# jameshball/kidney-diffusion

Measured on AMD Instinct MI355X. Metric: denoising-steps/sec (64->256 SR UNet, bs16), higher is better.
Workload: dtype f32

## Files before the change

### include/kd_engine.h

```cpp
#ifndef KD_ENGINE_H
#define KD_ENGINE_H

#include <stddef.h>
#include <stdint.h>

#ifdef __cplusplus
extern "C" {
#endif

#define KD_MAX_LEVELS 8

const char* kd_last_error(void);
#define KD_ENGINE_ABI_VERSION 2
int kd_version(void);
const char* kd_build_id(void);

typedef struct kd_unet_config {
  int dim;
  int num_levels;
  int dim_mults[KD_MAX_LEVELS];
  int num_resnet_blocks[KD_MAX_LEVELS];
  int layer_attns[KD_MAX_LEVELS];
  int layer_cross_attns[KD_MAX_LEVELS];
  int cond_dim;
  int channels;
  int cond_images_channels;
  int lowres_cond;
  int memory_efficient;
  int init_conv_to_final_conv_residual;
  int cond_on_text;
  int text_tokens;
  int attn_heads;
  int attn_dim_head;
  int ff_mult_x2;
  int num_time_tokens;
  int sinu_dim;
  int resnet_groups;
  int attend_at_middle;
  int use_gca;
  int batch;
  int image_size;
  int conv_algo;
  int attn_qk_norm;
  int downsample_conv4;
  int mid_attn_plain;
  int wino_slice_mb;
  int wino43_min_cin;
  int gemm_bf16x3;
  int x3_linear;
  int wino4_max_images;
} kd_unet_config_t;

typedef struct kd_param {
  const char* name;
  const float* d_data;
  int64_t numel;
} kd_param_t;

typedef struct kd_unet kd_unet_t;

int kd_unet_create(const kd_unet_config_t* cfg, const kd_param_t* params, int n_params,
                   kd_unet_t** out);
int kd_unet_create_shared(const kd_unet_config_t* cfg, const kd_param_t* params, int n_params,
                          const kd_unet_t* share_with, kd_unet_t** out);
int kd_unet_create_self_cond(const kd_unet_config_t* cfg, const kd_param_t* params, int n_params,
                             const kd_unet_t* share_with, int self_cond, kd_unet_t** out);
typedef struct kd_unet_ext {
  int self_cond;
  int use_linear_attn[KD_MAX_LEVELS];
  int use_linear_cross_attn[KD_MAX_LEVELS];
  int cross_embed_downsample;
  int upsample_nearest;
} kd_unet_ext_t;
int kd_unet_create_ext(const kd_unet_config_t* cfg, const kd_param_t* params, int n_params, const kd_unet_t* share_with,
                       const kd_unet_ext_t* ext, kd_unet_t** out);
typedef struct kd_unet_ext2 {
  int combine_upsample_fmaps;
} kd_unet_ext2_t;
int kd_unet_create_ext2(const kd_unet_config_t* cfg, const kd_param_t* params, int n_params, const kd_unet_t* share_with,
                        const kd_unet_ext_t* ext, const kd_unet_ext2_t* ext2, kd_unet_t** out);
typedef struct kd_unet_ext3 {
  int layer_attns_depth[KD_MAX_LEVELS];
} kd_unet_ext3_t;
int kd_unet_create_ext3(const kd_unet_config_t* cfg, const kd_param_t* params, int n_params, const kd_unet_t* share_with,
                        const kd_unet_ext_t* ext, const kd_unet_ext2_t* ext2, const kd_unet_ext3_t* ext3, kd_unet_t** out);
void kd_unet_destroy(kd_unet_t* u);
int64_t kd_unet_hbm_bytes(const kd_unet_t* u);
int64_t kd_unet_weight_bytes(const kd_unet_t* u);
int64_t kd_unet_macs(const kd_unet_t* u);
int64_t kd_unet_mfma_macs(const kd_unet_t* u);
int64_t kd_unet_mfma_bf16_macs(const kd_unet_t* u);
int kd_unet_num_launches(const kd_unet_t* u);
int kd_unet_num_cond_launches(const kd_unet_t* u);
float kd_unet_cond_table_build_ms(kd_unet_t* u, int* rows, int* runs);
int64_t kd_unet_cond_table_refused_bytes(const kd_unet_t* u);

int kd_unet_text_cond(kd_unet_t* u, const float* d_text_embeds, const float* d_text_mask, int L, int drop,
                      float* d_text_tokens, float* d_text_hiddens, void* stream);

int kd_unet_profile(kd_unet_t* u, int iters, char* buf, size_t buflen, void* stream);

int kd_unet_forward(kd_unet_t* u, const float* d_x, const float* d_lowres,
                    const float* d_cond_images, const float* d_log_snr,
                    const float* d_lowres_log_snr, const float* d_text_tokens,
                    const float* d_text_hiddens, float* d_out, void* stream);
int kd_unet_forward_self_cond(kd_unet_t* u, const float* d_x, const float* d_self_cond, const float* d_lowres,
                              const float* d_cond_images, const float* d_log_snr, const float* d_lowres_log_snr,
                              const float* d_text_tokens, const float* d_text_hiddens, float* d_out, void* stream);

int kd_cfg_combine(const float* d_cond, const float* d_null, float* d_out, float cond_scale, int64_t n,
                   void* stream);

enum { KD_OBJ_NOISE = 0, KD_OBJ_V = 1, KD_OBJ_X_START = 2 };

typedef struct kd_schedule {
  int T;
  const float* log_snr;
  const float* alpha;
  const float* sigma;
  const float* alpha_next;
  const float* sigma_next;
  const float* c;
  const float* noise_scale;
  const float* rn_a;
  const float* rn_b;
} kd_schedule_t;

typedef struct kd_sample_args {
  int objective;
  int dynamic_threshold;
  float percentile;
  int resample_times;
  const float* d_lowres;
  const float* d_lowres_log_snr;
  const float* d_cond_images;
  const float* d_text_tokens;
  const float* d_text_hiddens;
  const float* d_inpaint_images;
  const float* d_inpaint_masks;
  const float* d_noise_step;
  const float* d_noise_inpaint;
  const float* d_noise_renoise;
  uint64_t seed;
  int use_graph;
  float cond_scale;
  const float* d_null_text_tokens;
  const float* d_null_text_hiddens;
  int lowres_log_snr_uniform;
  float lowres_log_snr_value;
  int cond_table;
  int cond_table_max_mb;
} kd_sample_args_t;

int kd_sample_loop(kd_unet_t* u, const kd_schedule_t* sched, const kd_sample_args_t* args,
                   float* d_img, void* stream);
int kd_sample_steps(kd_unet_t* u, const kd_schedule_t* sched, const kd_sample_args_t* args,
                    float* d_img, int k_begin, int k_end, void* stream);
int kd_sample_build_cond_table(kd_unet_t* u, const kd_schedule_t* sched, const kd_sample_args_t* args, int k_begin,
                               int k_end, int force, int* built, void* stream);
int kd_sample_finalize(kd_unet_t* u, const kd_sample_args_t* args, float* d_img, void* stream);
int kd_sample_last(kd_unet_t* u, int which, float* d_out, void* stream);
int kd_sample_set_self_cond(kd_unet_t* u, const float* d_x_start, void* stream);

typedef struct kd_edm_schedule {
  int N;
  float S_noise;
  const float* sigma;
  const float* sigma_hat;
  const float* sigma_next;
  const float* churn;
  const float* euler_step;
  const float* heun_step;
  const float* renoise;
  const float* c_in_hat;
  const float* c_skip_hat;
  const float* c_out_hat;
  const float* c_noise_hat;
  const float* c_in_next;
  const float* c_skip_next;
  const float* c_out_next;
  const float* c_noise_next;
} kd_edm_schedule_t;

int kd_edm_sample_loop(kd_unet_t* u, const kd_edm_schedule_t* sched, const kd_sample_args_t* args, float* d_img,
                       void* stream);
int kd_edm_sample_steps(kd_unet_t* u, const kd_edm_schedule_t* sched, const kd_sample_args_t* args, float* d_img,
                        int k_begin, int k_end, void* stream);


int kd_conv2d_nhwc(const float* d_x, const float* d_w_oihw, const float* d_bias, float* d_y,
                   int B, int Hi, int Wi, int Cin, int Cout, int KH, int KW, int stride, int pad,
                   int act, void* stream);
int kd_upsample_nearest_conv3x3_nhwc(const float* d_x, const float* d_w_oihw, const float* d_bias, float* d_y, int ldy, int yoff,
                                     int B, int H, int W, int Cin, int Cout, void* stream);
int kd_upsample_nearest_gn_conv3x3_nhwc(const float* d_x, int ldx, const float* d_ab, const float* d_w_oihw, const float* d_bias,
                                        float* d_y, int ldy, int yoff, int B, int H, int W, int Cin, int Cout, int scale,
                                        void* stream);
int kd_conv3x3_winograd_nhwc(const float* d_x, const float* d_w_oihw, const float* d_bias, float* d_y,
                             int B, int H, int W, int Cin, int Cout, void* stream);
int kd_conv3x3_winograd4_nhwc(const float* d_x, const float* d_w_oihw, const float* d_bias, const float* d_res,
                              float* d_y, int B, int H, int W, int Cin, int Cout, int G, float eps,
                              float* d_out_stats, int gemm_bf16x3, void* stream);
int kd_gemm_bf16x3(const float* d_a, const float* d_b, float* d_c, int G, int M, int N, int K, int a_planes, void* stream);
int kd_linear_bf16x3(const float* d_x, int ldx, const float* d_w, const float* d_bias, const float* d_res, int ldres,
                     const float* d_gate_src, int ldgs, const float* d_gate, int hw, float* d_y, int ldy, int M, int N, int K,
                     int act, int pixshuf_wo, double* d_seg, void* stream);
int kd_linear_bf16x3_seg_rows(int M, int N, int K);
int kd_downsample_bf16x3(const float* d_x, int ldx, const float* d_w, const float* d_bias, float* d_y, int B, int H, int W, int C,
                         int O, double* d_seg, void* stream);
int kd_gn_conv3x3_winograd_fused_nhwc(const float* d_x, const float* d_gamma, const float* d_beta,
                                      const float* d_scale_shift, const float* d_w_oihw,
                                      const float* d_bias, const float* d_res, float* d_y, int B, int H,
                                      int W, int Cin, int Cout, int G, float eps, float* d_out_stats,
                                      int ldx, void* stream);

int kd_linear_skinny(const float* d_x, int ldx, const float* d_w, const float* d_bias, float* d_y, int ldy, int M, int K,
                     int N, int in_act, int act, void* stream);
int kd_global_context_gate(const float* d_x, int B, int HW, int C, const float* d_wk, const float* d_bk, const float* d_w0,
                           const float* d_b0, int hid, const float* d_w2, const float* d_b2, float* d_gate, float* d_pooled,
                           int path, void* stream);
int kd_gate_add_nhwc(const float* d_a, const float* d_gate, const float* d_r, int ldr, float* d_y, int ldy, double* d_seg,
                     int B, int HW, int C, void* stream);
int kd_gate_add_chunks(int B, int HW);
int kd_linattn_chunk_tokens(void);
int kd_linattn_dwconv_nhwc(const float* d_x, const float* d_wq, const float* d_wk, const float* d_wv, float* d_y,
                           float* d_part, int B, int H, int W, int heads, void* stream);
int kd_linattn_context(const float* d_k, const float* d_v, int ld, const float* d_part, int HW, const float* d_ck,
                       const float* d_cv, int ldc, int m, const float* d_null_k, const float* d_null_v, float* d_ctx, int B,
                       int heads, void* stream);
int kd_linattn_apply(const float* d_q, int ldq, const float* d_ctx, float* d_out, int ldo, int B, int N, int heads,
                     float scale, int silu, void* stream);
int kd_gn_fold_seg(const double* d_seg0, int nseg0, int nchunk0, float scale0, float ab_mul0, const double* d_seg1, int nseg1,
                   int nchunk1, float scale1, float ab_mul1, const float* d_gamma, const float* d_beta,
                   const float* d_scale_shift, int ld_ss, float* d_ab, float* d_stats, int B, int HW, int C, int G, float eps,
                   void* stream);
float kd_wf_ab_scale(void);
int kd_gn_conv3x3_winograd4_nhwc(const float* d_x, int ldx, const float* d_stats, const float* d_gamma, const float* d_beta,
                                 const float* d_scale_shift, int ld_ss, int skip_c0, float skip_scale, const float* d_w_oihw,
                                 const float* d_bias, const float* d_res, int ldres, float* d_y, double* d_out_seg, int B,
                                 int H, int W, int Cin, int Cout, int G, int gemm_mode, int images_per_set, void* stream);

int kd_init_conv_nchw(const float* d_x, const float* d_w3, const float* d_w7, const float* d_w15,
                      const float* d_bias, float* d_y, int B, int S, int n3, int n7, int n15, void* stream);
int kd_init_conv_planes_nchw(const float* d_x, const float* d_self_cond, const float* d_w3, const float* d_w7,
                             const float* d_w15, int Itot, int c0, const float* d_bias, const float* d_res, float* d_y, int B,
                             int S, int n3, int n7, int n15, int iters, float* ms, void* stream);
int kd_init_conv_planes_c_nchw(const float* d_x, const float* d_self_cond, const float* d_w3, const float* d_w7,
                               const float* d_w15, int Itot, int c0, const float* d_bias, const float* d_res, float* d_y, int B,
                               int S, int n3, int n7, int n15, int iters, float* ms, int channels, void* stream);
int kd_final_conv_nchw(const float* d_feat, const float* d_w_oihw, const float* d_bias, const float* d_lowres, float* d_out,
                       int B, int H, int W, int Cfeat, int channels, void* stream);
int kd_groupnorm_silu_nhwc(const float* d_x, const float* d_gamma, const float* d_beta,
                           const float* d_scale_shift, float* d_y, int B, int HW, int C, int G,
                           float eps, void* stream);
int kd_layernorm(const float* d_x, const float* d_g, const float* d_beta, float* d_y,
                 int rows, int C, float eps, void* stream);
int kd_layernorm_ex(const float* d_x, const float* d_g, const float* d_beta, const float* d_res, float* d_y, int rows, int C,
                    float eps, int in_act, const float* d_g2, float* d_y2, void* stream);
int kd_layernorm_linear_bf16x3(const float* d_x, const float* d_g, const float* d_beta, int rows, int C, float eps, int in_act,
                               const float* d_w, const float* d_bias, const float* d_res, int ldres, float* d_y, int ldy,
                               int N, void* d_planes, void* stream);
int kd_attention(const float* d_q, const float* d_k, const float* d_v, float* d_out,
                 int B, int Nq, int Nk, int H, int Hkv, int D, void* stream);
int kd_attention_ex(const float* d_q, int ldq, const float* d_null_kv, const float* d_k0, const float* d_v0, int ld0, int n0,
                    const float* d_k1, const float* d_v1, int ld1, int n1, float* d_out, int ldo, int B, int Nq, int H, int Hkv,
                    float scale, void* stream);
int kd_attention_ex_d(const float* d_q, int ldq, const float* d_null_kv, const float* d_k0, const float* d_v0, int ld0, int n0,
                      const float* d_k1, const float* d_v1, int ld1, int n1, float* d_out, int ldo, int B, int Nq, int H, int Hkv,
                      int D, float scale, void* stream);
int kd_attention_key_tile(int D);
int kd_l2norm_heads(float* d_x, int ld, int64_t rows, int heads, const float* d_scale_vec, void* stream);
int kd_l2norm_heads_d(float* d_x, int ld, int64_t rows, int heads, int D, const float* d_scale_vec, void* stream);
int kd_text_select(const float* d_tok, const float* d_mask, const float* d_null_embed, float* d_out, int B, int L, int P, int C,
                   int drop, void* stream);
int kd_add_rows_bcast(const float* d_x, const float* d_add, float* d_y, int B, int R, int C, void* stream);
int kd_mean_rows(const float* d_x, float* d_y, int B, int R, int C, void* stream);
int kd_copy_rows(const float* d_src, int64_t src_bstride, int ld_src, float* d_dst, int64_t dst_bstride, int ld_dst, int rows,
                 int C, int B, void* stream);
int kd_quantile_abs(const float* d_x, float* d_out, int B, int64_t n, float q, void* d_workspace,
                    size_t workspace_bytes, void* stream);
size_t kd_quantile_workspace_bytes(int B);
int kd_philox_normal(float* d_out, int64_t n, uint64_t seed, uint64_t stream_id, void* stream);

#ifdef __cplusplus
}
#endif
#endif
```

### kidney-diffusion_amd/csrc/api.inc

```
extern "C" {

const char* kd_last_error(void) { return kd::g_err.c_str(); }
int kd_version(void) { return KD_ENGINE_ABI_VERSION; }

int kd_unet_create(const kd_unet_config_t* cfg, const kd_param_t* params, int n_params, kd_unet_t** out) {
  return kd_unet_create_shared(cfg, params, n_params, nullptr, out);
}

int kd_unet_create_shared(const kd_unet_config_t* cfg, const kd_param_t* params, int n_params,
                          const kd_unet_t* share_with, kd_unet_t** out) {
  return kd_unet_create_self_cond(cfg, params, n_params, share_with, 0, out);
}

int kd_unet_create_self_cond(const kd_unet_config_t* cfg, const kd_param_t* params, int n_params,
                             const kd_unet_t* share_with, int self_cond, kd_unet_t** out) {
  kd_unet_ext_t ext;
  memset(&ext, 0, sizeof ext);
  ext.self_cond = self_cond;
  return kd_unet_create_ext(cfg, params, n_params, share_with, &ext, out);
}

int kd_unet_create_ext(const kd_unet_config_t* cfg, const kd_param_t* params, int n_params, const kd_unet_t* share_with,
                       const kd_unet_ext_t* ext, kd_unet_t** out) {
  return kd_unet_create_ext2(cfg, params, n_params, share_with, ext, nullptr, out);
// ... 363 lines not shown
  KD_REQUIRE(d_x && d_w_oihw && d_y, "kd_upsample_nearest_gn_conv3x3_nhwc: null argument");
  if (const char* why = upsample_scale_refusal(ldx, ldy, yoff, B, H, W, Cin, Cout, scale)) {
    set_error(why);
    return 1;
  }
  EntryBufs bufs;
  float* wp = nullptr;
  if (bufs.get(&wp, upsample_scale_weight_floats(Cin, Cout) * sizeof(float))) return 1;
  int rc = launch_upsample_scale_pack(d_w_oihw, wp, Cout, Cin, s);
  if (!rc) rc = launch_upsample_scale_conv3x3(d_x, ldx, d_ab, wp, d_bias, d_y, ldy, yoff, B, H, W, Cin, Cout, scale, s);
  return entry_finish(rc, s);
}

int kd_conv3x3_winograd_nhwc(const float* d_x, const float* d_w_oihw, const float* d_bias, float* d_y, int B, int H,
                             int W, int Cin, int Cout, void* stream) {
  hipStream_t s = (hipStream_t)stream;
  KD_REQUIRE(H % 2 == 0 && W % 2 == 0, "Winograd path needs even H and W");
  const int64_t Mt = (int64_t)B * (H / 2) * (W / 2);
  KD_REQUIRE(Mt % 256 == 0 && Cin % 32 == 0 && Cout > 32 && Cout % 4 == 0,
             "Winograd path needs B*H*W/4 % 256 == 0, Cin % 32 == 0, Cout > 32");
  EntryBufs bufs;
  float *U = nullptr, *V = nullptr, *D = nullptr;
  if (bufs.get(&U, (size_t)16 * Cout * Cin * sizeof(float))) return 1;
  if (bufs.get(&V, (size_t)16 * Mt * Cin * sizeof(float))) return 1;
  if (bufs.get(&D, (size_t)16 * Mt * Cout * sizeof(float))) return 1;
  int rc = launch_wino_pack(d_w_oihw, U, Cout, Cin, s);
  if (!rc) rc = launch_wino_in(d_x, Cin, nullptr, nullptr, nullptr, nullptr, 0, V, B, H, W, Cin, 1, 0, Mt, s);
  if (!rc) {
    ConvParams p{};
    p.x = V; p.w = U; p.y = D;
    p.B = 1; p.Hi = 1; p.Wi = (int)(16 * Mt); p.Cin = Cin; p.ldx = Cin;
    p.Ho = 1; p.Wo = (int)(16 * Mt); p.Cout = Cout;
    p.KH = 1; p.KW = 1; p.stride = 1; p.pad = 0;
    p.out_mode = OUT_NHWC; p.ldy = Cout;
    p.wz_rows = (int)Mt; p.wz_count = 16;
    rc = launch_conv_igemm(p, s);
  }
  if (!rc) rc = launch_wino_out(D, d_bias, nullptr, 0, d_y, B, H, W, Cout, 0, Mt, s);
  return entry_finish(rc, s);
}

int kd_conv3x3_winograd4_nhwc(const float* d_x, const float* d_w_oihw, const float* d_bias, const float* d_res, float* d_y,
                              int B, int H, int W, int Cin, int Cout, int G, float eps, float* d_out_stats, int gemm_bf16x3,
                              void* stream) {
  hipStream_t s = (hipStream_t)stream;
  KD_REQUIRE(H % 4 == 0 && W % 4 == 0, "Winograd F(4x4,3x3) path needs H % 4 == 0 and W % 4 == 0");
  const int64_t Mt = (int64_t)B * (H / 4) * (W / 4);
  KD_REQUIRE(!gemm_bf16x3 || gemm_bf16x3_ok(36, Mt, Cout, Cin),
             "bf16x3 position GEMMs need B*H*W/16 % 256 == 0, Cout % 128 == 0, Cin % 32 == 0");
  KD_REQUIRE(Mt % 128 == 0 && Cin % 32 == 0 && Cout % 64 == 0,
             "Winograd F(4x4,3x3) path needs B*H*W/16 % 128 == 0, Cin % 32 == 0, Cout % 64 == 0");
  KD_REQUIRE(!d_out_stats || (G > 0 && Cout % G == 0 && (Cout / G) % 16 == 0), "output statistics need (Cout / G) % 16 == 0");
  EntryBufs bufs;
  float *U = nullptr, *V = nullptr, *D = nullptr;
  double* seg = nullptr;
  void *U3 = nullptr, *x3ws = nullptr;
  const int nchunk = (H / 4) * (W / 4);
  if (bufs.get(&U, (size_t)36 * Cout * Cin * sizeof(float))) return 1;
  if (bufs.get(&V, (size_t)36 * Mt * Cin * (gemm_bf16x3 == 1 ? 6 : sizeof(float)))) return 1;
  if (bufs.get(&D, (size_t)36 * Mt * Cout * sizeof(float))) return 1;
  if (gemm_bf16x3 && bufs.get(&U3, (size_t)36 * Cout * Cin * 6)) return 1;
  if (gemm_bf16x3 && bufs.get(&x3ws, gemm_bf16x3_workspace_bytes())) return 1;
  if (d_out_stats && bufs.get(&seg, (size_t)B * (Cout / 16) * nchunk * 2 * sizeof(double))) return 1;
  if (gemm_bf16x3) KD_HIP_CHECK(hipMemsetAsync(x3ws, 0, gemm_bf16x3_workspace_bytes(), s));
  int rc = launch_wino4_pack(d_w_oihw, U, Cout, Cin, s);
  if (!rc && gemm_bf16x3) {
    rc = launch_split3(U, U3, 36, Cout, Cin, s);
    if (!rc && gemm_bf16x3 == 1) rc = launch_wino4_in3(d_x, Cin, nullptr, nullptr, nullptr, nullptr, 0, V, B, H, W, Cin, 1, s);
    if (!rc && gemm_bf16x3 != 1) rc = launch_wino4_in(d_x, Cin, nullptr, nullptr, nullptr, nullptr, 0, V, B, H, W, Cin, 1, s);
    if (!rc) rc = launch_gemm_bf16x3(V, U3, D, 36, (int)Mt, Cout, Cin, entry_x3_shape(36, Mt, Cout, Cin), x3ws, s, gemm_bf16x3 != 1);
  }
  if (!rc && !gemm_bf16x3) rc = launch_wino4_in(d_x, Cin, nullptr, nullptr, nullptr, nullptr, 0, V, B, H, W, Cin, 1, s);
  if (!rc && !gemm_bf16x3) {
    ConvParams p{};
    p.x = V; p.w = U; p.y = D;
    p.B = 1; p.Hi = 1; p.Wi = (int)(36 * Mt); p.Cin = Cin; p.ldx = Cin;
    p.Ho = 1; p.Wo = (int)(36 * Mt); p.Cout = Cout;
    p.KH = 1; p.KW = 1; p.stride = 1; p.pad = 0;
    p.out_mode = OUT_NHWC; p.ldy = Cout;
    p.wz_rows = (int)Mt; p.wz_count = 36;
    rc = launch_conv_igemm(p, s);
  }
  if (!rc) rc = launch_wino4_out(D, d_bias, d_res, Cout, d_y, Cout, seg, B, H, W, Cout, s);
  if (!rc && seg)
    rc = launch_gn_finalize(seg, d_out_stats, (Cout / G / 16) * nchunk, B, G, (double)H * W * (Cout / G), eps, s);
  return entry_finish(rc, s);
}

int kd_gemm_bf16x3(const float* d_a, const float* d_b, float* d_c, int G, int M, int N, int K, int a_planes, void* stream) {
  hipStream_t s = (hipStream_t)stream;
  KD_REQUIRE(gemm_bf16x3_ok(G, M, N, K), "kd_gemm_bf16x3 needs M % 256 == 0, N % 128 == 0, K % 32 == 0, operand planes < 4 GB");
  EntryBufs bufs;
  void *A3 = nullptr, *B3 = nullptr, *ws = nullptr;
  if (bufs.get(&B3, (size_t)G * N * K * 6)) return 1;
  if (a_planes && bufs.get(&A3, (size_t)G * M * K * 6)) return 1;
  if (bufs.get(&ws, gemm_bf16x3_workspace_bytes())) return 1;
  int rc = a_planes ? launch_split3(d_a, A3, G, M, K, s) : 0;
  if (!rc) rc = launch_split3(d_b, B3, G, N, K, s);
  if (!rc) rc = launch_gemm_bf16x3(a_planes ? A3 : (const void*)d_a, B3, d_c, G, M, N, K, entry_x3_shape(G, M, N, K), ws, s, !a_planes);
  return entry_finish(rc, s);
}

int kd_downsample_bf16x3(const float* d_x, int ldx, const float* d_w, const float* d_bias, float* d_y, int B, int H, int W, int C,
                         int O, double* d_seg, void* stream) {
  hipStream_t s = (hipStream_t)stream;
  const int K = 4 * C;
  const int64_t M = (int64_t)B * (H / 2) * (W / 2);
  X3Epi e;
  e.bias = d_bias;
  e.lda = ldx > 0 ? ldx : C;
  e.ldy = O;
  e.a_tap_c = C;
  e.a_wi = W;
  e.a_hi = H;
  e.hw = (H / 2) * (W / 2);
  e.seg = d_seg;
  e.seg_nseg = d_seg ? O / 16 : 0;
  const X3Shape sh = entry_x3_shape(1, M, O, K);
  KD_REQUIRE(H > 0 && W > 0 && !(H & 1) && !(W & 1) && M < 0x7fffffff && gemm_bf16x3_epi_ok(M, O, K, e, sh),
             "kd_downsample_bf16x3 needs even map sides, C % 16 == 0, B (H/2) (W/2) % 256 == 0, O % 128 == 0");
  EntryBufs bufs;
  float *wt = nullptr, *wk = nullptr;
  void *W3 = nullptr, *ws = nullptr;
  if (bufs.get(&wt, (size_t)O * K * 4) || bufs.get(&wk, (size_t)O * K * 4) || bufs.get(&W3, (size_t)O * K * 6) ||
      bufs.get(&ws, gemm_bf16x3_workspace_bytes()))
    return 1;
  int rc = launch_pack_unshuffle(d_w, wt, O, C, s);
  for (int t = 0; t < 4 && !rc; ++t) rc = launch_copy_scale_rows(wt + (size_t)t * O * C, C, wk + (size_t)t * C, K, C, 1.0f, O, s);
  if (!rc) rc = launch_split3(wk, W3, 1, O, K, s);
  if (!rc) rc = launch_gemm_bf16x3(d_x, W3, d_y, 1, (int)M, O, K, sh, ws, s, true, true, &e);
  return entry_finish(rc, s);
}

int kd_linear_bf16x3_seg_rows(int M, int N, int K) { return gemm_bf16x3_ok(1, M, N, K) ? entry_x3_shape(1, M, N, K).seg_rows() : 0; }

int kd_linear_bf16x3(const float* d_x, int ldx, const float* d_w, const float* d_bias, const float* d_res, int ldres,
                     const float* d_gate_src, int ldgs, const float* d_gate, int hw, float* d_y, int ldy, int M, int N, int K,
                     int act, int pixshuf_wo, double* d_seg, void* stream) {
  hipStream_t s = (hipStream_t)stream;
  X3Epi e;
  e.seg = d_seg;
  e.seg_nseg = d_seg ? (pixshuf_wo ? N / 4 : N) / 16 : 0;
  e.act = act;
  e.pixshuf_wo = pixshuf_wo;
  e.bias = d_bias;
  e.res = d_res;
  e.ldres = ldres;
  e.gate_src = d_gate_src;
  e.ldgs = ldgs;
  e.gate = d_gate;
  e.hw = hw;
  e.ldy = ldy > 0 ? ldy : (pixshuf_wo ? N / 4 : N);
  e.lda = ldx > 0 ? ldx : K;
  const X3Shape sh = entry_x3_shape(1, M, N, K);
  KD_REQUIRE(gemm_bf16x3_epi_ok(M, N, K, e, sh), "kd_linear_bf16x3 needs M % 256 == 0, N % 128 == 0, K % 32 == 0, row strides >= the "
                                             "rows, hw % 256 == 0 under a gate");
  EntryBufs bufs;
  void *W3 = nullptr, *ws = nullptr;
  if (bufs.get(&W3, (size_t)N * K * 6) || bufs.get(&ws, gemm_bf16x3_workspace_bytes())) return 1;
  int rc = launch_split3(d_w, W3, 1, N, K, s);
  if (!rc) rc = launch_gemm_bf16x3(d_x, W3, d_y, 1, M, N, K, sh, ws, s, true, true, &e);
  return entry_finish(rc, s);
}

int kd_gn_conv3x3_winograd_fused_nhwc(const float* d_x, const float* d_gamma, const float* d_beta,
                                      const float* d_scale_shift, const float* d_w_oihw, const float* d_bias,
                                      const float* d_res, float* d_y, int B, int H, int W, int Cin, int Cout, int G,
                                      float eps, float* d_out_stats, int ldx, void* stream) {
  hipStream_t s = (hipStream_t)stream;
  if (ldx <= 0) ldx = Cin;
  KD_REQUIRE(wino_fused128_ok(B, H, W, Cin, Cout) && G > 0 && Cin % G == 0,
             "GroupNorm-fused Winograd path needs H % 8 == 0, W % 16 == 0, Cin % 4 == 0, Cin <= 2048, Cout % 128 == 0");
  KD_REQUIRE(ldx >= Cin && ldx % 4 == 0, "GroupNorm-fused Winograd path: input row stride must be >= Cin and a multiple of 4");
  KD_REQUIRE(!d_out_stats || (Cout % G == 0 && (Cout / G) % 16 == 0), "output statistics need (Cout / G) % 16 == 0");
  EntryBufs bufs;
  float *U = nullptr, *stats = nullptr, *ab = nullptr;
  double *partial = nullptr, *opart = nullptr;
  void* items = nullptr;
  if (bufs.get(&U, (size_t)16 * Cout * Cin * sizeof(float))) return 1;
  if (bufs.get(&stats, (size_t)B * G * 2 * sizeof(float))) return 1;
  if (bufs.get(&ab, (size_t)B * Cin * 2 * sizeof(float))) return 1;
  if (bufs.get(&partial, gn_partial_bytes(B, H * W, Cin, G))) return 1;
  if (d_out_stats && bufs.get(&opart, (size_t)B * G * wino_fused_out_stats_chunks(H, W, Cout, G) * 2 * sizeof(double))) return 1;
  if (bufs.get(&items, wino_fused128_items_count(B, H, W, Cout) * 16)) return 1;
  int rc = launch_wino_fused128_pack(d_w_oihw, U, Cout, Cin, s, WF_U_SCALE);
  if (!rc) rc = launch_gn_stats(d_x, ldx, stats, partial, B, H * W, Cin, G, eps, s);
  if (!rc) rc = launch_gn_fold(stats, d_gamma, d_beta, d_scale_shift, 2 * Cin, ab, B, Cin, G, s);
  if (!rc) rc = launch_wino_fused128_items(items, B, H, W, Cout, s);
  if (!rc)
    rc = launch_wino_fused_gn128(d_x, ldx, ab, U, d_bias, d_res, Cout, d_y, B, H, W, Cin, Cout, opart, opart ? G : 0, items, s);
  if (!rc && opart)
    rc = launch_gn_finalize(opart, d_out_stats, (int)wino_fused_out_stats_chunks(H, W, Cout, G), B, G,
                            (double)H * W * (Cout / G), eps, s);
  return entry_finish(rc, s);
}


int kd_linear_skinny(const float* d_x, int ldx, const float* d_w, const float* d_bias, float* d_y, int ldy, int M, int K,
                     int N, int in_act, int act, void* stream) {
  hipStream_t s = (hipStream_t)stream;
  KD_REQUIRE(d_x && d_w && d_y, "kd_linear_skinny: null argument");
  KD_REQUIRE(M > 0 && K > 0 && N > 0 && ldx >= K && ldy >= N, "kd_linear_skinny needs M, K, N > 0, ldx >= K, ldy >= N");
  KD_REQUIRE(in_act >= ACT_NONE && in_act <= ACT_SIGMOID && act >= ACT_NONE && act <= ACT_SIGMOID,
             "kd_linear_skinny: unknown activation");
  return entry_finish(launch_linear_skinny(d_x, ldx, d_w, d_bias, d_y, ldy, M, K, N, in_act, act, s), s);
}

int kd_linattn_chunk_tokens(void) { return LA_CHUNK; }

int kd_linattn_dwconv_nhwc(const float* d_x, const float* d_wq, const float* d_wk, const float* d_wv, float* d_y,
                           float* d_part, int B, int H, int W, int heads, void* stream) {
  hipStream_t s = (hipStream_t)stream;
  KD_REQUIRE(d_x && d_wq && d_wk && d_wv && d_y && d_part, "kd_linattn_dwconv_nhwc: null argument");
  KD_REQUIRE(B > 0 && H > 0 && W > 0 && heads > 0, "kd_linattn_dwconv_nhwc needs B, H, W, heads > 0");
  const int inner = heads * 64;
  EntryBufs bufs;
  float* w = nullptr;
  if (bufs.get((void**)&w, (size_t)27 * inner * sizeof(float))) return 1;
  int rc = launch_linattn_pack_dw(d_wq, d_wk, d_wv, w, inner, s);
  if (!rc) rc = launch_linattn_dwconv(d_x, w, d_y, d_part, B, H, W, inner, s);
  return entry_finish(rc, s);
}

int kd_linattn_context(const float* d_k, const float* d_v, int ld, const float* d_part, int HW, const float* d_ck,
                       const float* d_cv, int ldc, int m, const float* d_null_k, const float* d_null_v, float* d_ctx, int B,
                       int heads, void* stream) {
  hipStream_t s = (hipStream_t)stream;
  KD_REQUIRE(d_ctx && B > 0 && heads > 0 && HW >= 0 && m >= 0, "kd_linattn_context: null output or bad sizes");
  EntryBufs bufs;
  float* ws = nullptr;
  if (HW > 0 && bufs.get((void**)&ws, linattn_ws_floats(B, heads, HW) * sizeof(float))) return 1;
  return entry_finish(launch_linattn_context(d_k, d_v, ld, d_part, HW, d_ck, d_cv, ldc, m, d_null_k, d_null_v, ws, d_ctx, B,
                                             heads, s), s);
}

int kd_linattn_apply(const float* d_q, int ldq, const float* d_ctx, float* d_out, int ldo, int B, int N, int heads,
                     float scale, int silu, void* stream) {
  hipStream_t s = (hipStream_t)stream;
  KD_REQUIRE(d_q && d_ctx && d_out, "kd_linattn_apply: null argument");
  return entry_finish(launch_linattn_apply(d_q, ldq, d_ctx, d_out, ldo, B, N, heads, scale, silu, s), s);
}

int kd_global_context_gate(const float* d_x, int B, int HW, int C, const float* d_wk, const float* d_bk, const float* d_w0,
                           const float* d_b0, int hid, const float* d_w2, const float* d_b2, float* d_gate, float* d_pooled,
                           int path, void* stream) {
  hipStream_t s = (hipStream_t)stream;
  KD_REQUIRE(d_x && d_wk && d_bk && d_w0 && d_b0 && d_w2 && d_b2 && d_gate, "kd_global_context_gate: null argument");
  KD_REQUIRE(B > 0 && HW > 0 && hid > 0 && C % 4 == 0 && C > 0 && C <= 2048,
             "kd_global_context_gate needs B, HW, hid > 0 and C % 4 == 0, C <= 2048");
  KD_REQUIRE(path >= 0 && path <= 2, "kd_global_context_gate: path 0 (the plan's choice), 1 (pool + two linears), 2 (fused)");
  const bool fused_ok = gca_gate_fused_ok(C, hid) && (((uintptr_t)d_w0 | (uintptr_t)d_w2) & 15) == 0;
  KD_REQUIRE(path != 2 || fused_ok, "kd_global_context_gate: the fused gate needs C <= 512, hid <= 256, 16-byte aligned weights");
  const bool fused = path == 2 || (path == 0 && gca_gate_fused_ok(C, hid) && B > 1);
  KD_REQUIRE(!(fused && d_pooled), "kd_global_context_gate: the fused gate does not leave the pooled vector");
  EntryBufs bufs;
  float *scratch = nullptr, *pooled = d_pooled, *hidden = nullptr;
  if (bufs.get((void**)&scratch, gca_scratch_floats(B, HW, C) * sizeof(float))) return 1;
  if (fused) return entry_finish(launch_gca_gate(d_x, d_wk, d_bk, scratch, d_w0, d_b0, hid, d_w2, d_b2, d_gate, B, HW, C, s), s);
  if (!pooled && bufs.get((void**)&pooled, (size_t)B * C * sizeof(float))) return 1;
  if (bufs.get((void**)&hidden, (size_t)B * hid * sizeof(float))) return 1;
  int rc = launch_gca_pool(d_x, d_wk, d_bk, nullptr, pooled, scratch, B, HW, C, s);
  if (!rc) rc = launch_linear_skinny(pooled, C, d_w0, d_b0, hidden, hid, B, C, hid, ACT_NONE, ACT_SILU, s);
  if (!rc) rc = launch_linear_skinny(hidden, hid, d_w2, d_b2, d_gate, C, B, hid, C, ACT_NONE, ACT_SIGMOID, s);
  return entry_finish(rc, s);
}

int kd_gate_add_chunks(int B, int HW) { return B > 0 && HW > 0 ? gate_add_chunks(B, HW) : 0; }

int kd_gate_add_nhwc(const float* d_a, const float* d_gate, const float* d_r, int ldr, float* d_y, int ldy, double* d_seg,
                     int B, int HW, int C, void* stream) {
  hipStream_t s = (hipStream_t)stream;
  if (ldr <= 0) ldr = C;
  if (ldy <= 0) ldy = C;
  KD_REQUIRE(d_a && d_r && d_y, "kd_gate_add_nhwc: null argument");
  KD_REQUIRE(B > 0 && HW > 0 && C > 0 && C % 4 == 0 && ldr >= C && ldy >= C && ldr % 4 == 0 && ldy % 4 == 0,
             "kd_gate_add_nhwc needs C % 4 == 0 and row strides >= C, multiples of 4");
  KD_REQUIRE((((uintptr_t)d_a | (uintptr_t)d_gate | (uintptr_t)d_r | (uintptr_t)d_y) & 15) == 0,
             "kd_gate_add_nhwc: 16-byte aligned maps and gate");
  KD_REQUIRE(!d_seg || C % 16 == 0, "kd_gate_add_nhwc: segment partials need C % 16 == 0");
  return entry_finish(launch_gate_add(d_a, d_gate, d_r, ldr, d_y, ldy, d_seg, B, HW, C, s), s);
}

float kd_wf_ab_scale(void) { return WF_AB_SCALE; }

int kd_gn_fold_seg(const double* d_seg0, int nseg0, int nchunk0, float scale0, float ab_mul0, const double* d_seg1, int nseg1,
                   int nchunk1, float scale1, float ab_mul1, const float* d_gamma, const float* d_beta,
                   const float* d_scale_shift, int ld_ss, float* d_ab, float* d_stats, int B, int HW, int C, int G, float eps,
                   void* stream) {
  hipStream_t s = (hipStream_t)stream;
  KD_REQUIRE(d_seg0 && (d_ab || d_stats), "kd_gn_fold_seg: null argument");
  KD_REQUIRE(B > 0 && HW > 0 && G > 0 && C % G == 0 && (C / G) % 16 == 0, "kd_gn_fold_seg needs groups of 16 n channels");
  KD_REQUIRE(nseg0 > 0 && nchunk0 > 0 && (!d_seg1 || (nseg1 > 0 && nchunk1 > 0)) &&
                 16 * (nseg0 + (d_seg1 ? nseg1 : 0)) == C,
             "kd_gn_fold_seg: the sources' 16-channel segments must tile the C channels");
  KD_REQUIRE(!d_ab || (d_gamma && d_beta), "kd_gn_fold_seg: the affine needs gamma and beta");
  KD_REQUIRE(!d_scale_shift || ld_ss >= 2 * C, "kd_gn_fold_seg: FiLM rows [scale | shift] need ld_ss >= 2 C");
  SegSrc s0{d_seg0, nseg0, nchunk0, 0, scale0, ab_mul0};
  SegSrc s1{d_seg1, d_seg1 ? nseg1 : 0, d_seg1 ? nchunk1 : 0, 16 * nseg0, scale1, ab_mul1};
  return entry_finish(launch_gn_fold_seg(s0, s1, d_gamma, d_beta, d_scale_shift, ld_ss, d_ab, d_stats, B, C, G,
                                         (double)HW * (C / G), eps, s),
                      s);
}

int kd_gn_conv3x3_winograd4_nhwc(const float* d_x, int ldx, const float* d_stats, const float* d_gamma, const float* d_beta,
                                 const float* d_scale_shift, int ld_ss, int skip_c0, float skip_scale, const float* d_w_oihw,
                                 const float* d_bias, const float* d_res, int ldres, float* d_y, double* d_out_seg, int B,
                                 int H, int W, int Cin, int Cout, int G, int gemm_mode, int images_per_set, void* stream) {
  hipStream_t s = (hipStream_t)stream;
  if (ldx <= 0) ldx = Cin;
  if (ldres <= 0) ldres = Cout;
  const int Bx = images_per_set > 0 ? images_per_set : B;
  KD_REQUIRE(d_x && d_stats && d_gamma && d_beta && d_w_oihw && d_bias && d_y, "kd_gn_conv3x3_winograd4_nhwc: null argument");
  KD_REQUIRE(B > 0 && Bx > 0 && B % Bx == 0, "kd_gn_conv3x3_winograd4_nhwc: images_per_set must divide B");
  KD_REQUIRE(H > 0 && W > 0 && H % 4 == 0 && W % 4 == 0, "Winograd F(4x4,3x3) path needs H % 4 == 0 and W % 4 == 0");
  const int64_t Mt = (int64_t)Bx * (H / 4) * (W / 4);
  KD_REQUIRE(Mt % 128 == 0 && Cin % 32 == 0 && Cout % 64 == 0 && 36 * Mt < 0x7fffffff &&
                 (int64_t)36 * Cout * Cin * 4 < 0x7fffffff,
             "Winograd F(4x4,3x3) path needs images_per_set*H*W/16 % 128 == 0, Cin % 32 == 0, Cout % 64 == 0");
  KD_REQUIRE(gemm_mode == -1 || gemm_mode == 1 || gemm_mode == 2, "kd_gn_conv3x3_winograd4_nhwc: gemm_mode -1, 1 or 2");
  KD_REQUIRE(gemm_mode < 0 || gemm_bf16x3_ok(36, Mt, Cout, Cin),
             "bf16x3 position GEMMs need images_per_set*H*W/16 % 256 == 0, Cout % 128 == 0, Cin % 32 == 0");
  KD_REQUIRE(G > 0 && Cin % G == 0, "kd_gn_conv3x3_winograd4_nhwc: Cin % G == 0");
  KD_REQUIRE(ldx >= Cin && ldx % 2 == 0 && ((uintptr_t)d_x & 7) == 0 && (int64_t)Bx * H * W * ldx * 4 < ((int64_t)1 << 32),
             "kd_gn_conv3x3_winograd4_nhwc: x rows of stride >= Cin, even, 8-byte aligned, one set's map below 4 GB");
  KD_REQUIRE(skip_c0 < 0 || (skip_c0 <= Cin && skip_c0 % 2 == 0), "kd_gn_conv3x3_winograd4_nhwc: skip_c0 in [0, Cin], even");
  KD_REQUIRE(!d_scale_shift || ld_ss >= 2 * Cin, "kd_gn_conv3x3_winograd4_nhwc: FiLM rows [scale | shift] need ld_ss >= 2 Cin");
  KD_REQUIRE(!d_res || (ldres >= Cout && ldres % 2 == 0), "kd_gn_conv3x3_winograd4_nhwc: residual row stride >= Cout, even");
  KD_REQUIRE((((uintptr_t)d_y | (uintptr_t)d_res | (uintptr_t)d_bias) & 7) == 0,
             "kd_gn_conv3x3_winograd4_nhwc: 8-byte aligned y, residual and bias");
  const bool planes = gemm_mode == 1, x3 = gemm_mode > 0;
  const X3Shape sh = entry_x3_shape(36, Mt, Cout, Cin);
  EntryBufs bufs;
  float *U = nullptr, *D = nullptr;
  void *V = nullptr, *U3 = nullptr, *ws = nullptr;
  if (bufs.get((void**)&U, (size_t)36 * Cout * Cin * sizeof(float))) return 1;
  if (bufs.get(&V, planes ? (size_t)36 * Mt * Cin * 6 : (size_t)36 * Mt * Cin * sizeof(float))) return 1;
  if (bufs.get((void**)&D, (size_t)36 * Mt * Cout * sizeof(float))) return 1;
  if (x3 && bufs.get(&U3, ((size_t)36 * Cout * Cin * 3 + 1) / 2 * sizeof(float))) return 1;
  if (x3 && bufs.get(&ws, gemm_bf16x3_workspace_bytes())) return 1;
  int rc = launch_wino4_pack(d_w_oihw, U, Cout, Cin, s);
  if (!rc && x3) rc = launch_split3(U, U3, 36, Cout, Cin, s);
  const int64_t HW = (int64_t)H * W, nchunk = (H / 4) * (W / 4);
  for (int st = 0; st < B / Bx && !rc; ++st) {
    const int b0 = st * Bx;
    const float* xs = d_x + (size_t)b0 * HW * ldx;
    const float* ss = d_stats + (size_t)b0 * G * 2;
    const float* ssp = d_scale_shift ? d_scale_shift + (size_t)b0 * ld_ss : nullptr;
    if (planes)
      rc = launch_wino4_in3(xs, ldx, ss, d_gamma, d_beta, ssp, ld_ss, V, Bx, H, W, Cin, G, s, skip_c0, skip_scale);
    else
      rc = launch_wino4_in(xs, ldx, ss, d_gamma, d_beta, ssp, ld_ss, (float*)V, Bx, H, W, Cin, G, s, skip_c0, skip_scale);
    if (!rc && x3) {
      rc = launch_gemm_bf16x3(V, U3, D, 36, (int)Mt, Cout, Cin, sh, ws, s, !planes);
    } else if (!rc) {
      ConvParams p{};
      p.x = (const float*)V; p.w = U; p.y = D;
      p.B = 1; p.Hi = 1; p.Wi = (int)(36 * Mt); p.Cin = Cin; p.ldx = Cin;
      p.Ho = 1; p.Wo = (int)(36 * Mt); p.Cout = Cout;
      p.KH = 1; p.KW = 1; p.stride = 1; p.pad = 0;
      p.out_mode = OUT_NHWC; p.ldy = Cout;
      p.wz_rows = (int)Mt; p.wz_count = 36;
      rc = launch_conv_igemm(p, s);
    }
    if (!rc)
      rc = launch_wino4_out(D, d_bias, d_res ? d_res + (size_t)b0 * HW * ldres : nullptr, ldres, d_y + (size_t)b0 * HW * Cout,
                            Cout, d_out_seg ? d_out_seg + (size_t)b0 * (Cout / 16) * nchunk * 2 : nullptr, Bx, H, W, Cout, s);
  }
  return entry_finish(rc, s);
}

int kd_init_conv_nchw(const float* d_x, const float* d_w3, const float* d_w7, const float* d_w15, const float* d_bias,
                      float* d_y, int B, int S, int n3, int n7, int n15, void* stream) {
  return kd_init_conv_planes_nchw(d_x, nullptr, d_w3, d_w7, d_w15, 3, 0, d_bias, nullptr, d_y, B, S, n3, n7, n15, 1, nullptr,
                                  stream);
}

int kd_init_conv_planes_nchw(const float* d_x, const float* d_self_cond, const float* d_w3, const float* d_w7,
                             const float* d_w15, int Itot, int c0, const float* d_bias, const float* d_res, float* d_y, int B,
                             int S, int n3, int n7, int n15, int iters, float* ms, void* stream) {
  return kd_init_conv_planes_c_nchw(d_x, d_self_cond, d_w3, d_w7, d_w15, Itot, c0, d_bias, d_res, d_y, B, S, n3, n7, n15, iters,
                                    ms, 3, stream);
}

int kd_init_conv_planes_c_nchw(const float* d_x, const float* d_self_cond, const float* d_w3, const float* d_w7,
                               const float* d_w15, int Itot, int c0, const float* d_bias, const float* d_res, float* d_y, int B,
                               int S, int n3, int n7, int n15, int iters, float* ms, int channels, void* stream) {
  hipStream_t s = (hipStream_t)stream;
  KD_REQUIRE(channels >= 1 && channels <= 4, "kd_init_conv_planes_c_nchw: 1 to 4 image channels");
  const int np = d_self_cond ? 2 * channels : channels;
  KD_REQUIRE(d_x && d_w3 && d_w7 && d_w15 && d_y && iters >= 1, "kd_init_conv_planes_nchw: null argument or iters < 1");
  KD_REQUIRE(B >= 1 && S >= 1, "kd_init_conv_planes_nchw: empty shape");
  KD_REQUIRE(c0 >= 0 && c0 + np <= Itot, "kd_init_conv_planes_nchw: input channels c0 .. c0 + planes - 1 out of range");
  KD_REQUIRE(init_conv_fused_ok(S, n3, n7, n15, np), "init conv kernel: S % 32 == 0 and the weights must fit LDS");
  EntryBufs bufs;
  float* wp = nullptr;
  hipEvent_t e0 = nullptr, e1 = nullptr;
  if (bufs.get(&wp, init_conv_weight_floats(n3, n7, n15, np) * sizeof(float))) return 1;
  int rc = launch_init_conv_pack(d_w3, d_w7, d_w15, wp, n3, n7, n15, Itot, c0, np, s);
  if (!rc && ms) {
    rc = hipEventCreate(&e0) != hipSuccess || hipEventCreate(&e1) != hipSuccess || hipEventRecord(e0, s) != hipSuccess;
    if (rc) set_error("kd_init_conv_planes_nchw: event setup failed");
  }
  for (int i = 0; i < iters && !rc; ++i)
    rc = launch_init_conv(d_x, d_self_cond, channels, np, wp, d_bias, d_res, d_y, n3 + n7 + n15, nullptr, B, S, n3, n7, n15, s);
  if (!rc && ms && hipEventRecord(e1, s) != hipSuccess) {
    set_error("kd_init_conv_planes_nchw: event record failed");
    rc = 1;
  }
  hipError_t e = hipStreamSynchronize(s);
  if (!rc && ms && e == hipSuccess) {
    float t = 0.f;
    e = hipEventElapsedTime(&t, e0, e1);
    *ms = t / iters;
  }
  if (e0) (void)hipEventDestroy(e0);
  if (e1) (void)hipEventDestroy(e1);
  if (rc) return rc;
  KD_HIP_CHECK(e);
  return 0;
}

int kd_final_conv_nchw(const float* d_feat, const float* d_w_oihw, const float* d_bias, const float* d_lowres, float* d_out,
                       int B, int H, int W, int Cfeat, int channels, void* stream) {
  hipStream_t s = (hipStream_t)stream;
  KD_REQUIRE(d_feat && d_w_oihw && d_bias && d_out, "kd_final_conv_nchw: null argument");
  KD_REQUIRE(channels >= 1 && channels <= 4, "kd_final_conv_nchw: 1 to 4 image channels");
  KD_REQUIRE(B >= 1 && H >= 1 && W >= 1 && Cfeat >= 4 && Cfeat % 4 == 0 && (int64_t)B * H * W < 0x7fffffff / 48,
             "kd_final_conv_nchw needs a non-empty map below 2^31 / 48 pixels and Cfeat % 4 == 0");
  const int Ctot = Cfeat + (d_lowres ? channels : 0), nf = final_gemm_cols(channels);
  EntryBufs bufs;
  float *wp = nullptr, *pm = nullptr, *stat = nullptr;
  if (bufs.get(&wp, (size_t)nf * Cfeat * sizeof(float)) || bufs.get(&pm, (size_t)B * H * W * nf * sizeof(float))) return 1;
  if (d_lowres && bufs.get(&stat, (size_t)B * channels * H * W * sizeof(float))) return 1;
  int rc = launch_pack_final(d_w_oihw, wp, Ctot, Cfeat, channels, s);
  if (!rc && d_lowres) rc = launch_final_static(d_lowres, d_w_oihw, d_bias, stat, Ctot, Cfeat, channels, B, H, W, s);
  if (!rc) {
    ConvParams p{};
    p.x = d_feat; p.w = wp; p.y = pm;
    p.B = B; p.Hi = H; p.Wi = W; p.Cin = Cfeat; p.ldx = Cfeat;
    p.Ho = H; p.Wo = W; p.Cout = nf;
    p.KH = 1; p.KW = 1; p.stride = 1; p.pad = 0;
    p.out_mode = OUT_NHWC; p.ldy = nf;
    rc = launch_conv_igemm(p, s);
  }
  if (!rc) rc = launch_final_gather(pm, stat, d_bias, d_out, channels, B, H, W, s);
  return entry_finish(rc, s);
}

int kd_groupnorm_silu_nhwc(const float* d_x, const float* d_gamma, const float* d_beta, const float* d_scale_shift,
                           float* d_y, int B, int HW, int C, int G, float eps, void* stream) {
  hipStream_t s = (hipStream_t)stream;
  EntryBufs bufs;
  float* stats = nullptr;
  double* partial = nullptr;
  if (bufs.get(&stats, (size_t)B * G * 2 * sizeof(float)) || bufs.get(&partial, gn_partial_bytes(B, HW, C, G))) return 1;
  int rc = launch_gn_stats(d_x, C, stats, partial, B, HW, C, G, eps, s);
  if (!rc) rc = launch_gn_apply_silu(d_x, C, stats, d_gamma, d_beta, d_scale_shift, 2 * C, d_y, B, HW, C, G, s);
  return entry_finish(rc, s);
}

int kd_layernorm(const float* d_x, const float* d_g, const float* d_beta, float* d_y, int rows, int C, float eps,
                 void* stream) {
  return launch_layernorm(d_x, C, d_g, d_beta, nullptr, 0, d_y, rows, C, eps, (hipStream_t)stream);
}

int kd_layernorm_ex(const float* d_x, const float* d_g, const float* d_beta, const float* d_res, float* d_y, int rows, int C,
                    float eps, int in_act, const float* d_g2, float* d_y2, void* stream) {
  KD_REQUIRE(in_act >= ACT_NONE && in_act <= ACT_SIGMOID, "kd_layernorm_ex: unknown activation");
  return launch_layernorm(d_x, C, d_g, d_beta, d_res, C, d_y, rows, C, eps, (hipStream_t)stream, in_act, d_g2, d_y2);
}

int kd_layernorm_linear_bf16x3(const float* d_x, const float* d_g, const float* d_beta, int rows, int C, float eps, int in_act,
                               const float* d_w, const float* d_bias, const float* d_res, int ldres, float* d_y, int ldy,
                               int N, void* d_planes, void* stream) {
  hipStream_t s = (hipStream_t)stream;
  KD_REQUIRE(in_act >= ACT_NONE && in_act <= ACT_SIGMOID, "kd_layernorm_linear_bf16x3: unknown activation");
  KD_REQUIRE(d_planes && C % 16 == 0 && C <= 4096, "kd_layernorm_linear_bf16x3 needs C % 16 == 0, C <= 4096 and the plane buffer");
  X3Epi e;
  e.bias = d_bias;
  e.res = d_res;
  e.ldres = ldres;
  e.hw = rows;
  e.ldy = ldy > 0 ? ldy : N;
  e.lda = C;
  const X3Shape sh = entry_x3_shape(1, rows, N, C);
  KD_REQUIRE(gemm_bf16x3_epi_ok(rows, N, C, e, sh), "kd_layernorm_linear_bf16x3 needs rows % 256 == 0, N % 128 == 0, C % 32 == 0");
  EntryBufs bufs;
  void *W3 = nullptr, *ws = nullptr;
  if (bufs.get(&W3, (size_t)N * C * 6) || bufs.get(&ws, gemm_bf16x3_workspace_bytes())) return 1;
  int rc = launch_split3(d_w, W3, 1, N, C, s);
  if (!rc) rc = launch_layernorm(d_x, C, d_g, d_beta, nullptr, 0, (float*)d_planes, rows, C, eps, s, in_act, nullptr, nullptr, nullptr, 0, 1);
  if (!rc) rc = launch_gemm_bf16x3(d_planes, W3, d_y, 1, rows, N, C, sh, ws, s, false, true, &e);
  return entry_finish(rc, s);
}

int kd_attention(const float* d_q, const float* d_k, const float* d_v, float* d_out, int B, int Nq, int Nk, int H,
                 int Hkv, int D, void* stream) {
  KD_REQUIRE(D == 32 || D == 64 || D == 128, "kd_attention is built for D = 32, 64 and 128");
  KVSeg s0{d_k, d_v, Hkv * D, Nk};
  KVSeg s1{nullptr, nullptr, 0, 0};
  return launch_attention(d_q, H * D, nullptr, nullptr, s0, s1, d_out, H * D, B, Nq, H, Hkv, D, 1.0f,
                          (hipStream_t)stream);
}

int kd_attention_ex(const float* d_q, int ldq, const float* d_null_kv, const float* d_k0, const float* d_v0, int ld0, int n0,
                    const float* d_k1, const float* d_v1, int ld1, int n1, float* d_out, int ldo, int B, int Nq, int H, int Hkv,
                    float scale, void* stream) {
  return kd_attention_ex_d(d_q, ldq, d_null_kv, d_k0, d_v0, ld0, n0, d_k1, d_v1, ld1, n1, d_out, ldo, B, Nq, H, Hkv, 64, scale,
                           stream);
}

int kd_attention_ex_d(const float* d_q, int ldq, const float* d_null_kv, const float* d_k0, const float* d_v0, int ld0, int n0,
                      const float* d_k1, const float* d_v1, int ld1, int n1, float* d_out, int ldo, int B, int Nq, int H, int Hkv,
                      int D, float scale, void* stream) {
  hipStream_t s = (hipStream_t)stream;
  KD_REQUIRE(d_q && d_out && B > 0 && H > 0 && n0 >= 0 && n1 >= 0, "kd_attention_ex: null argument or bad sizes");
  KD_REQUIRE((n0 == 0 || (d_k0 && d_v0)) && (n1 == 0 || (d_k1 && d_v1)), "kd_attention_ex: a segment with keys needs k and v");
  KD_REQUIRE((((uintptr_t)d_q | (uintptr_t)d_null_kv | (uintptr_t)d_k0 | (uintptr_t)d_v0 | (uintptr_t)d_k1 | (uintptr_t)d_v1 |
               (uintptr_t)d_out) & 15) == 0, "kd_attention_ex: 16-byte aligned pointers");
  KD_REQUIRE(D == 32 || D == 64 || D == 128, "kd_attention_ex_d: D must be 32, 64 or 128");
  KD_REQUIRE(ldq >= H * D && ldo >= H * D && (n0 == 0 || ld0 >= Hkv * D) && (n1 == 0 || ld1 >= Hkv * D),
             "kd_attention_ex: a row stride is shorter than its heads");
  KVSeg s0{d_k0, d_v0, ld0, n0};
  KVSeg s1{d_k1, d_v1, ld1, n1};
  return entry_finish(launch_attention(d_q, ldq, d_null_kv, d_null_kv ? d_null_kv + D : nullptr, s0, s1, d_out, ldo, B,
                                       Nq, H, Hkv, D, scale, s), s);
}

int kd_attention_key_tile(int D) { return attention_key_tile(D); }

int kd_l2norm_heads(float* d_x, int ld, int64_t rows, int heads, const float* d_scale_vec, void* stream) {
  return kd_l2norm_heads_d(d_x, ld, rows, heads, 64, d_scale_vec, stream);
}

int kd_l2norm_heads_d(float* d_x, int ld, int64_t rows, int heads, int D, const float* d_scale_vec, void* stream) {
  hipStream_t s = (hipStream_t)stream;
  KD_REQUIRE(D == 32 || D == 64 || D == 128, "kd_l2norm_heads_d: D must be 32, 64 or 128");
  KD_REQUIRE(d_x && rows >= 0 && heads > 0 && ld >= heads * D, "kd_l2norm_heads: null argument or ld < heads * D");
  return entry_finish(launch_l2norm_heads(d_x, ld, rows, heads, D, d_scale_vec, s), s);
}

int kd_text_select(const float* d_tok, const float* d_mask, const float* d_null_embed, float* d_out, int B, int L, int P, int C,
                   int drop, void* stream) {
  hipStream_t s = (hipStream_t)stream;
  KD_REQUIRE(d_tok && d_null_embed && d_out, "kd_text_select: null argument");
  KD_REQUIRE(B > 0 && C > 0 && L >= 1 && L <= P, "kd_text_select needs B, C > 0 and 1 <= L <= P");
  return entry_finish(launch_text_select(d_tok, d_mask, d_null_embed, d_out, B, L, P, C, drop != 0, s), s);
}

int kd_add_rows_bcast(const float* d_x, const float* d_add, float* d_y, int B, int R, int C, void* stream) {
  hipStream_t s = (hipStream_t)stream;
  KD_REQUIRE(d_x && d_add && d_y && B > 0 && R > 0 && C > 0, "kd_add_rows_bcast: null argument or empty shape");
  return entry_finish(launch_add_rows_bcast(d_x, d_add, d_y, B, R, C, s), s);
}

int kd_mean_rows(const float* d_x, float* d_y, int B, int R, int C, void* stream) {
  hipStream_t s = (hipStream_t)stream;
  KD_REQUIRE(d_x && d_y && B > 0 && R > 0 && C > 0, "kd_mean_rows: null argument or empty shape");
  KD_REQUIRE((int64_t)B * C < 0x7fffffff, "kd_mean_rows: B * C must stay below 2^31 (one thread per output, int index)");
  return entry_finish(launch_mean_rows(d_x, d_y, B, R, C, s), s);
}

int kd_copy_rows(const float* d_src, int64_t src_bstride, int ld_src, float* d_dst, int64_t dst_bstride, int ld_dst, int rows,
                 int C, int B, void* stream) {
  hipStream_t s = (hipStream_t)stream;
  KD_REQUIRE(d_src && d_dst && rows >= 0 && C >= 0 && B >= 0, "kd_copy_rows: null argument or negative size");
  KD_REQUIRE(ld_src >= C && ld_dst >= C && src_bstride >= 0 && dst_bstride >= 0, "kd_copy_rows needs row strides >= C, batch strides >= 0");
  return entry_finish(launch_copy_rows(d_src, src_bstride, ld_src, d_dst, dst_bstride, ld_dst, rows, C, B, s), s);
}

size_t kd_quantile_workspace_bytes(int B) { return quantile_ws_bytes(B); }
int kd_quantile_abs(const float* d_x, float* d_out, int B, int64_t n, float q, void* d_workspace,
                    size_t workspace_bytes, void* stream) {
  KD_REQUIRE(workspace_bytes >= quantile_ws_bytes(B), "quantile workspace too small");
  return launch_quantile_abs(d_x, d_out, B, n, q, d_workspace, (hipStream_t)stream);
}

int kd_cfg_combine(const float* d_cond, const float* d_null, float* d_out, float cond_scale, int64_t n,
                   void* stream) {
  KD_REQUIRE(d_cond && d_null && d_out && n >= 0, "kd_cfg_combine: null argument");
  return launch_cfg_combine(d_cond, d_null, d_out, cond_scale, n, (hipStream_t)stream);
}

int kd_philox_normal(float* d_out, int64_t n, uint64_t seed, uint64_t stream_id, void* stream) {
  return launch_philox_normal(d_out, n, seed, stream_id, (hipStream_t)stream);
}

}
```

### kidney-diffusion_amd/csrc/common.h

```cpp
#pragma once
#include <hip/hip_runtime.h>
#include <stdint.h>
#include <stdio.h>
#include <algorithm>
#include <string>

#ifdef KD_EXPERIMENT
#include "../../scratch/experiment_switch.h"
#else
constexpr int kd_switch(const char*, int dflt) { return dflt; }
#endif

namespace kd {

void set_error(const std::string& msg);

#define KD_HIP_CHECK(expr)                                                               \
  do {                                                                                   \
    hipError_t _e = (expr);                                                              \
    if (_e != hipSuccess) {                                                              \
      ::kd::set_error(std::string(#expr) + " failed: " + hipGetErrorString(_e) + " at " + \
                      __FILE__ + ":" + std::to_string(__LINE__));                        \
      return 1;                                                                          \
    }                                                                                    \
  } while (0)

#define KD_REQUIRE(cond, msg)                                                             \
  do {                                                                                    \
    if (!(cond)) {                                                                        \
      ::kd::set_error(std::string("requirement failed: ") + #cond + " — " + (msg) + " at " + \
                      __FILE__ + ":" + std::to_string(__LINE__));                         \
      return 1;                                                                           \
    }                                                                                     \
  } while (0)

enum Act { ACT_NONE = 0, ACT_SILU = 1, ACT_GELU = 2, ACT_SIGMOID = 3 };
enum OutMode { OUT_NHWC = 0, OUT_PIXSHUF = 1, OUT_NCHW = 2 };

struct ConvParams {
  const float* x;
  const float* w;
  const float* bias;
  float* y;
  int B, Hi, Wi, Cin, ldx;
  int Ho, Wo, Cout;
  int KH, KW, stride, pad;
  int rr_cin;
  int act;
  const float* res;
  int ldres;
  const float* gate_src;
  const float* gate;
  int ldgs;
  int out_mode;
  int ldy, yoff;
  int wz_rows, wz_count;
  float* partial;
  int ksplit;
  double* seg_partial;
  int seg_nseg;
  int seg_c0;
  int wide_epilogue;
};

int launch_conv_igemm(const ConvParams& p, hipStream_t s);
int conv_ksplit(const ConvParams& p);
int conv_seg_chunks(const ConvParams& p);
int64_t conv_macs(const ConvParams& p);

int launch_pack_oihw(const float* w_oihw, float* w_packed, int O, int I, int Ipad, int KH, int KW, hipStream_t s);
int launch_pack_oihw_rowrun(const float* w_oihw, float* w_packed, int O, int I, int Ipad, int KH, int KW, hipStream_t s);
int launch_pack_oihw_rowrun_sub(const float* w_oihw, float* w_packed, int O, int Itot, int a0, int na, int b0, int nb,
                                int Ipad, int KH, int KW, hipStream_t s);
int launch_pack_unshuffle(const float* w, float* w_packed, int O, int C, hipStream_t s);
int launch_pack_shuffle(const float* w, const float* b, float* w_packed, float* b_packed, int Co, int I,
                        hipStream_t s);

int launch_wino_pack(const float* w_oihw, float* U, int O, int I, hipStream_t s);
int launch_wino_in(const float* x, int ldx, const float* stats, const float* gamma, const float* beta,
                   const float* scale_shift, int ld_ss, float* V, int B, int H, int W, int C, int G, int64_t t0,
                   int64_t nt, hipStream_t s);
int launch_wino_out(const float* D, const float* bias, const float* res, int ldres, float* y, int B, int H, int W,
                    int C, int64_t t0, int64_t nt, hipStream_t s, double* seg_partial = nullptr);

int launch_wino4_pack(const float* w_oihw, float* U, int O, int I, hipStream_t s);
int launch_wino4_in(const float* x, int ldx, const float* stats, const float* gamma, const float* beta,
                    const float* scale_shift, int ld_ss, float* V, int B, int H, int W, int C, int G, hipStream_t s,
                    int mul_c0 = -1, float mul = 1.0f);
int launch_wino4_out(const float* D, const float* bias, const float* res, int ldres, float* y, int ldy, double* seg_partial,
                     int B, int H, int W, int C, hipStream_t s);

constexpr int X3_BK = 16;
__device__ __forceinline__ void x3_split(const float __attribute__((ext_vector_type(2))) a, uint32_t& h, uint32_t& m,
                                         uint32_t& l) {
  typedef float f2 __attribute__((ext_vector_type(2)));
  typedef __bf16 b2 __attribute__((ext_vector_type(2)));
  const b2 hb = __builtin_convertvector(a, b2);
  const f2 r1 = a - __builtin_convertvector(hb, f2);
  const b2 mb = __builtin_convertvector(r1, b2);
  const f2 r2 = r1 - __builtin_convertvector(mb, f2);
  const b2 lb = __builtin_convertvector(r2, b2);
  h = __builtin_bit_cast(uint32_t, hb);
  m = __builtin_bit_cast(uint32_t, mb);
  l = __builtin_bit_cast(uint32_t, lb);
}
bool gemm_bf16x3_ok(int G, int64_t M, int N, int K);
int launch_split3(const float* x, void* planes, int G, int R, int K, hipStream_t s);
size_t gemm_bf16x3_workspace_bytes();
struct X3Epi {
  const float* bias = nullptr;
  const float* res = nullptr;
  const float* gate_src = nullptr;
  const float* gate = nullptr;
  int ldres = 0, ldgs = 0;
  int hw = 0;
  int ldy = 0;
  int lda = 0;
  int a_tap_c = 0, a_wi = 0, a_hi = 0;
  double* seg = nullptr;
  int seg_nseg = 0, seg_coff = 0;
  int seg_rows8 = 0;
  int wide = 0;
  int act = ACT_NONE;
  int pixshuf_wo = 0;
};
struct X3Shape {
  int P, R, S, first;
  bool needs_sum() const { return R && S > 1; }
  int seg_rows() const { return needs_sum() ? 8 : 32; }
};
X3Shape gemm_bf16x3_shape(int G, int M, int N, int K, int cus);
int gemm_bf16x3_device_cus();
bool gemm_bf16x3_epi_ok(int64_t M, int N, int K, const X3Epi& e, const X3Shape& sh);
int launch_gemm_bf16x3(const void* A3, const void* B3, float* C, int G, int M, int N, int K, const X3Shape& sh, void* ws, hipStream_t s,
                       bool a_f32 = false, bool with_sum = true, const X3Epi* epi = nullptr);
int launch_gemm_bf16x3_sum(float* C, int G, int M, int N, int K, const X3Shape& sh, const void* ws, hipStream_t s, const X3Epi* epi = nullptr);
int launch_wino4_in3(const float* x, int ldx, const float* stats, const float* gamma, const float* beta,
                     const float* scale_shift, int ld_ss, void* V3, int B, int H, int W, int C, int G, hipStream_t s,
                     int mul_c0 = -1, float mul = 1.0f);

constexpr float WF_AB_SCALE = -1.4426950408889634f;
constexpr float WF_U_SCALE = -0.6931471805599453f;
int launch_gn_fold(const float* stats, const float* gamma, const float* beta, const float* scale_shift, int ld_ss,
                   float* ab, int B, int C, int G, hipStream_t s);
bool wino_fused128_ok(int B, int H, int W, int C, int N);
int launch_wino_fused128_pack(const float* w_oihw, float* U, int O, int I, hipStream_t s, float scale);
size_t wino_fused128_items_count(int B, int H, int W, int N);
int launch_wino_fused128_items(void* items, int B, int H, int W, int N, hipStream_t s);
size_t wino_fused_out_stats_chunks(int H, int W, int N, int G);
int launch_wino_fused_gn128(const float* x, int ldx, const float* ab, const float* U, const float* bias, const float* res,
                            int ldres, float* y, int B, int H, int W, int C, int N, double* out_partial, int out_groups,
                            const void* items, hipStream_t s);
int wino_fused_gn_max_cin();
int launch_gn_finalize(const double* partial, float* stats, int chunks, int B, int G, double count, float eps,
                       hipStream_t s);

int launch_gn_stats(const float* x, int ldx, float* stats , double* partial,
                    int B, int HW, int C, int G, float eps, hipStream_t s);
size_t gn_partial_bytes(int B, int HW, int C, int G);
int launch_gn_apply_silu(const float* x, int ldx, const float* stats, const float* gamma, const float* beta,
                         const float* scale_shift ,
                         int ld_ss, float* y, int B, int HW, int C, int G, hipStream_t s);
int launch_layernorm(const float* x, int ldx, const float* g, const float* beta, const float* res, int ldres, float* y,
                     int rows, int C, float eps, hipStream_t s, int in_act = ACT_NONE, const float* g2 = nullptr,
                     float* y2 = nullptr, double* seg = nullptr, int seg_hw = 0, int planes = 0);
int launch_copy_scale_rows(const float* src, int ld_src, float* dst, int ld_dst, int C, float scale, int64_t rows,
                           hipStream_t s);
int launch_gate_add(const float* a, const float* gate, const float* r, int ldr, float* y, int ldy, double* seg, int B,
                    int HW, int C, hipStream_t s);
int gate_add_chunks(int B, int HW);

struct SegSrc {
  const double* partial;
  int nseg, nchunk;
  int c0;
  float scale;
  float ab_mul;
};
int launch_gn_fold_seg(SegSrc s0, SegSrc s1, const float* gamma, const float* beta, const float* scale_shift, int ld_ss,
                       float* ab, float* stats, int B, int C, int G, double count, float eps, hipStream_t s);
int launch_add(const float* a, const float* b, float* y, int64_t n, hipStream_t s);
int launch_act(const float* a, float* y, int64_t n, int act, hipStream_t s);
int launch_pack_init(const float* cond, int Cc, const float* x, int Cx, const float* lowres, int Cl, float* y, int Cpad,
                     int B, int HW, hipStream_t s);
int launch_copy_rows(const float* src, int64_t src_bstride, int ld_src, float* dst, int64_t dst_bstride,
                     int ld_dst, int rows, int C, int B, hipStream_t s);
int launch_bcast_row(const float* src, float* dst, int64_t dst_bstride, int C, int B, hipStream_t s);

struct KVSeg {
  const float* k;
  const float* v;
  int ld;
  int n;
};
int launch_attention(const float* q, int ldq, const float* null_k, const float* null_v, KVSeg s0, KVSeg s1,
                     float* out, int ldo, int B, int Nq, int H, int Hkv, int D, float scale, hipStream_t s);
int attention_key_tile(int D);
int launch_linear_gemv(const float* x, const float* w, const float* bias, float* y, int K, int N, int in_act, int act,
                       hipStream_t s);
int launch_linear_skinny(const float* x, int ldx, const float* w, const float* bias, float* y, int ldy, int M,
                         int K, int N, int in_act, int act, hipStream_t s);
int launch_linear_skinny_valu(const float* x, int ldx, const float* w, const float* bias, float* y, int ldy, int M,
                              int K, int N, int in_act, int act, hipStream_t s);
int launch_gca_pool(const float* x, const float* wk, const float* bk, float* logits, float* pooled,
                    float* scratch, int B, int HW, int C, hipStream_t s);
size_t gca_scratch_floats(int B, int HW, int C);
bool gca_gate_fused_ok(int C, int hid);
int launch_gca_gate(const float* x, const float* wk, const float* bk, float* scratch, const float* w0, const float* b0, int hid,
                    const float* w2, const float* b2, float* gate, int B, int HW, int C, hipStream_t s);
int launch_sinu_emb(const float* t, const float* w, float* out, int B, int half, hipStream_t s);

bool init_conv_fused_ok(int S, int n3, int n7, int n15, int np);
size_t init_conv_weight_floats(int n3, int n7, int n15, int np);
int launch_init_conv_pack(const float* w3, const float* w7, const float* w15, float* out, int n3, int n7, int n15, int Itot,
                          int c0, int np, hipStream_t s);
int launch_init_conv(const float* x_nchw, const float* sc_nchw, int cx, int np, const float* wp, const float* bias, const float* res,
                     float* y, int ldy, double* seg, int B, int S, int n3, int n7, int n15, hipStream_t s);

constexpr int LA_CHUNK = 64;
int linattn_chunks(int HW);
int linattn_splits(int B, int heads, int HW);
size_t linattn_ws_floats(int B, int heads, int HW);
int launch_linattn_pack_dw(const float* wq, const float* wk, const float* wv, float* dst, int inner, hipStream_t s);
int launch_linattn_dwconv(const float* x, const float* w, float* y, float* part, int B, int H, int W, int inner,
                          hipStream_t s);
int launch_linattn_context(const float* k, const float* v, int ld, const float* part, int HW, const float* ck,
                           const float* cv, int ldc, int m, const float* nk, const float* nv, float* ws, float* ctx, int B,
                           int heads, hipStream_t s);
int launch_linattn_apply(const float* q, int ldq, const float* ctx, float* out, int ldo, int B, int N, int heads,
                         float scale, int silu, hipStream_t s);

const char* upsample_nearest_refusal(int ldx, int ldy, int yoff, int B, int H, int W, int Cin, int Cout);
size_t upsample_nearest_weight_floats(int Cin, int Cout);
int launch_upsample_nearest_pack(const float* w_oihw, float* wp, int O, int I, hipStream_t s);
int launch_upsample_nearest_conv3x3(const float* x, int ldx, const float* wp, const float* bias, float* y, int ldy, int yoff, int B,
                                    int H, int W, int Cin, int Cout, hipStream_t s);
const char* upsample_scale_refusal(int ldx, int ldy, int yoff, int B, int H, int W, int Cin, int Cout, int s);
size_t upsample_scale_weight_floats(int Cin, int Cout);
int launch_upsample_scale_pack(const float* w_oihw, float* wp, int O, int I, hipStream_t s);
int launch_upsample_scale_conv3x3(const float* x, int ldx, const float* ab, const float* wp, const float* bias, float* y, int ldy,
                                  int yoff, int B, int H, int W, int Cin, int Cout, int scale, hipStream_t s);

int final_gemm_cols(int ch);
int launch_pack_final(const float* w_oihw, float* w_packed, int Ctot, int C, int ch, hipStream_t s);
int launch_final_static(const float* lowres, const float* w_oihw, const float* bias, float* stat, int Ctot, int c0,
                        int ch, int B, int H, int W, hipStream_t s);
int launch_final_gather(const float* P, const float* stat, const float* bias, float* out, int ch, int B, int H, int W,
                        hipStream_t s);

int launch_text_select(const float* tok, const float* mask, const float* null_embed, float* out, int B, int L, int P,
                       int C, int drop, hipStream_t s);
int launch_add_rows_bcast(const float* x, const float* add, float* y, int B, int R, int C, hipStream_t s);
int launch_mean_rows(const float* x, float* y, int B, int R, int C, hipStream_t s);
int launch_l2norm_heads(float* x, int ld, int64_t rows, int heads, int D, const float* scale_vec, hipStream_t s);
int launch_cfg_combine(const float* cond, const float* nul, float* out, float scale, int64_t n, hipStream_t s);

struct StepTables {
  const float *log_snr, *alpha, *sigma, *alpha_next, *sigma_next, *c, *noise_scale, *rn_a, *rn_b;
};
int launch_fill_time(const float* table, const int* d_iter, int R, float* out, int B, hipStream_t s);
int launch_x0(const float* x, const float* pred, float* x0, const StepTables& tb, const int* d_iter, int R,
              int objective, int64_t n, hipStream_t s);
int launch_quantile_abs(const float* x, float* out, int B, int64_t n, float q, void* ws, hipStream_t s);
size_t quantile_ws_bytes(int B);
int launch_ddpm_update(float* x, const float* x0, const float* s_thresh, const float* noise, int64_t noise_stride,
                       const uint64_t* d_seed, const StepTables& tb, const int* d_iter, int R, int dynamic_threshold,
                       int B, int64_t per, hipStream_t s, float* sc_out = nullptr);
int launch_inpaint_mix(float* x, const float* inp, const float* mask, const float* noise, int64_t noise_stride,
                       const uint64_t* d_seed, const StepTables& tb, const int* d_iter, int R, int B, int C, int64_t hw,
                       hipStream_t s);
int launch_seed_set(uint64_t* d_seed, uint64_t value, hipStream_t s);
int launch_renoise(float* x, const float* noise, int64_t noise_stride, const uint64_t* d_seed, const StepTables& tb,
                   const int* d_iter, int R, int T, int B, int64_t per, hipStream_t s);
int launch_iter_set(int* d_iter, int value, hipStream_t s);
int launch_cond_gather(const void* tab, void* dst, size_t bytes, const int* d_iter, int R, hipStream_t s);
struct CondSeg { uint32_t off4, row4, start; };
int launch_fill_time_rows(const float* table, int k0, int T, float* out, int B, hipStream_t s);
int launch_cond_scatter(const float* ws, float* tab, const CondSeg* d_segs, int nseg, uint32_t row_total, int B, int k0, int T,
                        int64_t cond_floats, hipStream_t s);
int launch_finalize(float* x, const float* inp, const float* mask, int B, int C, int64_t hw, hipStream_t s);
struct EdmTables {
  const float *sigma, *sigma_hat, *sigma_next, *churn, *euler_step, *heun_step, *renoise, *c_in_hat, *c_skip_hat,
      *c_out_hat, *c_in_next, *c_skip_next, *c_out_next, *c_noise_hat, *c_noise_next;
};
int launch_edm_churn(const float* x, float* xh, float* net_in, const float* inp, const float* mask, const float* noise,
                     int64_t noise_stride, const uint64_t* d_seed, const EdmTables& tb, float s_noise, const int* d_iter,
                     int R, int B, int C, int64_t hw, hipStream_t s);
int launch_edm_precond_out(const float* x, const float* net, float* den, const float* c_skip_tab, const float* c_out_tab,
                           const int* d_iter, int R, int64_t n, hipStream_t s);
int launch_edm_euler(const float* xh, const float* den, const float* s_thresh, float* d_out, float* x, float* net_in,
                     const EdmTables& tb, const int* d_iter, int R, int dynamic_threshold, int B, int64_t per,
                     hipStream_t s, float* sc_out = nullptr);
int launch_edm_heun(float* x, const float* xh, const float* d_in, const float* den, const float* s_thresh,
                    const float* noise, int64_t noise_stride, const uint64_t* d_seed, const EdmTables& tb,
                    const int* d_iter, int R, int N, int renoise, int dynamic_threshold, int B, int64_t per,
                    hipStream_t s, float* sc_out = nullptr);

int launch_iter_inc(int* d_iter, hipStream_t s);
int launch_philox_normal(float* out, int64_t n, uint64_t seed, uint64_t stream_id, hipStream_t s);

}
```

### kidney-diffusion_amd/csrc/engine.hip

```cpp
#include <stdlib.h>
#include <string.h>

#include <algorithm>
#include <cstddef>
#include <functional>
#include <map>
#include <memory>
#include <stdexcept>
#include <string>
#include <type_traits>
#include <unordered_map>
#include <unordered_set>
#include <vector>

#include "../../include/kd_engine.h"
#include "common.h"

namespace kd {

static thread_local std::string g_err;
void set_error(const std::string& msg) { g_err = msg; }

#define KD_THROW_IF(expr)                                          \
  do {                                                             \
// ... 687 lines not shown
    last_seg_nchunk = seg_nseg ? seg_nchunk : 0;
    if (Bset > 0) {
      const int64_t M = (int64_t)Bset * Ho * Wo;
      const int Cin = x.C;
      const float* W3 = cached("x3lin:" + std::to_string((uintptr_t)w) + ":" + std::to_string(Cout) + "x" + std::to_string(Cin),
                               ((size_t)Cout * Cin * 3 + 1) / 2,
                               [&](float* dst) { KD_THROW_IF(launch_split3(w, dst, 1, Cout, Cin, 0)); });
      X3Epi base;
      base.bias = bias;
      base.ldres = p.ldres;
      base.ldgs = p.ldgs;
      base.hw = Ho * Wo;
      base.ldy = p.ldy;
      base.lda = p.ldx;
      base.act = o.act;
      base.pixshuf_wo = o.out_mode == OUT_PIXSHUF ? Wo : 0;
      const int seg_coff = o_yoff - seg_c0;
      for (int b0 = 0; b0 < x.B; b0 += Bset) {
        const Ref res = image(o.res, b0).floats(res_coff), gs = image(o.gate_src, b0), gate = image(o.gate, b0);
        const Ref seg = seg_nseg ? seg_at(sego, seg_nseg, seg_nchunk, b0) : Ref();
        auto epi_of = [=]() {
          X3Epi e = base;
          e.res = res.f();
          e.gate_src = gs.f();
          e.gate = gate.f();
          if (seg) {
            e.seg = seg.d();
            e.seg_nseg = seg_nseg;
            e.seg_coff = seg_coff;
          }
          return e;
        };
        const std::string shape = " M" + std::to_string(M) + " Cin" + std::to_string(Cin) + " Cout" + std::to_string(Cout);
        const int64_t m = o.macs_override >= 0 ? o.macs_override : M * Cout * Cin;
        emit_x3_gemm(image(x, b0), W3, image(y, b0).floats(o_yoff), 1, M, Cout, Cin, !x.x3p, epi_of, "conv k1", shape, m);
      }
      if (ks > 1) free(part);
      return y;
    }
    const Ref xr = at(x), yr = base(y), res = at(o.res).floats(res_coff), gs = at(o.gate_src), gate = at(o.gate);
    const Ref seg = seg_nseg ? seg_at(sego) : Ref();
    const kd_unet* io = u;
    emit([=](hipStream_t s) {
      ConvParams q = p;
      q.x = xr.f();
      q.y = ext ? io->out : yr.f();
      q.res = res.f();
      q.gate_src = gs.f();
      q.gate = gate.f();
      q.partial = partial.f();
      if (seg) {
        q.seg_partial = seg.d();
        q.seg_nseg = seg_nseg;
        q.seg_c0 = p.yoff - o_yoff + seg_c0;
      }
      return launch_conv_igemm(q, s);
    });
    if (ks > 1) free(part);
    int cin = o.cin_logical > 0 ? o.cin_logical : x.C;
    int64_t m = o.macs_override >= 0 ? o.macs_override : (int64_t)x.B * Ho * Wo * Cout * cin * K * K;
    if (recorded()) {
      u->op_label.back() = "conv k" + std::to_string(K) + " s" + std::to_string(stride) + " M" +
                           std::to_string((int64_t)x.B * Ho * Wo) + " Cin" + std::to_string(x.C) + " Cout" +
                           std::to_string(Cout);
      u->op_macs.back() = m;
    }
    count_macs(m, (int64_t)x.B * Ho * Wo * Cout * p.Cin * p.KH * p.KW);
    return y;
  }
  struct FlatLinear {
    T x, res, dst;
    ConvOpt o;
    static T flat(const T& t) {
      T f = t;
      f.B = 1; f.H = 1; f.W = (int)t.rows();
      return f;
    }
    FlatLinear(const T& x_, const T* res_, const T* dst_, int act) : x(flat(x_)) {
      o.act = act;
      if (res_) {
        res = flat(*res_);
        o.res = &res;
      }
      if (dst_) {
        dst = flat(*dst_);
        o.dst = &dst;
      }
    }
    FlatLinear(const FlatLinear&) = delete;
  };
  T linear(const T& x, const float* w, const float* bias, int N, int act = ACT_NONE, const T* res = nullptr,
           const T* dst = nullptr) {
    const FlatLinear f(x, res, dst, act);
    T y = conv(f.x, w, bias, N, 1, 1, 0, f.o);
    y.B = x.B; y.H = x.H; y.W = x.W;
    return y;
  }
  void skinny(Ref x, int ldx, const float* w, const float* bias, Ref y, int ldy, int M, int K, int N, int in_act, int act) {
    emit([=](hipStream_t s) {
      return launch_linear_skinny(x.f(), ldx, w, bias, y.f(), ldy, M, K, N, in_act, act, s);
    }, "skinny M" + std::to_string(M) + " K" + std::to_string(K) + " N" + std::to_string(N), (int64_t)M * K * N);
    if (phase != Phase::Text) u->macs += (int64_t)M * K * N;
  }

  T layernorm(const T& x, const float* g, const float* beta, const T* res = nullptr, int in_act = ACT_NONE,
              const float* g2 = nullptr, T* y2 = nullptr, bool want_seg = false, int planes = 0) {
    if (!x3_planes_on || x.C % 16 || x.C > 4096 || !step_op()) planes = 0;
    auto alloc_out = [&](bool pl) {
      if (!pl) return alloc(x.B, x.H, x.W, x.C);
      T t = alloc_bytes((size_t)x.rows() * x.C * 6);
      t.B = x.B; t.H = x.H; t.W = x.W; t.C = x.C;
      t.x3p = true;
      return t;
    };
    if ((planes & 1) && want_seg) throw std::runtime_error("plan: GroupNorm partials of a LayerNorm output in plane form");
    T y = alloc_out(planes & 1);
    if (g2) *y2 = alloc_out(planes & 2);
    int rows = (int)x.rows(), C = x.C, ldx = x.LD(), ldres = res ? res->LD() : 0;
    const int hw = x.HW();
    const bool sg = want_seg && step_op() && C % 16 == 0 && C <= 4096 && x.B * hw == rows;
    const Ref seg = sg ? seg_at(add_seg(y, 0, C / 16, hw)) : Ref();
    const Ref xr = at(x), yr = at(y), rr = at(res), y2r = g2 ? at(*y2) : Ref();
    emit([=](hipStream_t s) {
      return launch_layernorm(xr.f(), ldx, g, beta, rr.f(), ldres, yr.f(), rows, C, 1e-5f, s, in_act, g2, y2r.f(), seg.d(), hw, planes);
    }, std::string(g2 ? "ln x2 rows" : "ln rows") + std::to_string(rows) + " C" + std::to_string(C) + (planes ? " planes" : ""));
    return y;
  }
  bool linear_is_x3(const T& x, int N, const T* res = nullptr, const T* dst = nullptr) const {
    FlatLinear f(x, res, dst, ACT_NONE);
    f.x.ld = 0; f.x.coff = 0;
    return x3_linear_ok(f.x, N, 1, 1, 0, f.o);
  }

  T gn_silu(const T& x, const std::string& prefix, int ss_col) {
    const float* gamma = P(prefix + ".weight", x.C);
    const float* beta = P(prefix + ".bias", x.C);
    int G = cfg.resnet_groups;
    T y = alloc(x.B, x.H, x.W, x.C);
    emit_gn_stats(x, gamma, beta, ss_col, nullptr);
    const Ref xr = at(x), yr = at(y), st = at(gn_stats_t);
    const Film ss = film(ss_col);
    int Bx = x.B, HW = x.HW(), C = x.C, ldx = x.LD();
    emit([=](hipStream_t s) {
      return launch_gn_apply_silu(xr.f(), ldx, st.f(), gamma, beta, ss.row.f(), ss.ld, yr.f(), Bx, HW, C, G, s);
    }, "gn apply HW" + std::to_string(HW) + " C" + std::to_string(C));
    return y;
  }

  float attn_scale(int D = 0) const {
    return cfg.attn_qk_norm == 1 ? 16.0f : cfg.attn_qk_norm == 2 ? 8.0f : 1.0f / sqrtf((float)(D ? D : cfg.attn_dim_head));
  }
  void qk_norm(const T& t, int ld, int heads, const float* scale_vec, int D = 0) {
    const Ref tr = at(t);
    int64_t rows = t.rows();
    if (!D) D = cfg.attn_dim_head;
    emit([=](hipStream_t s) { return launch_l2norm_heads(tr.f(), ld, rows, heads, D, scale_vec, s); },
         "qk l2norm rows" + std::to_string(rows) + " heads" + std::to_string(heads));
  }
  const float* q_scale_of(const std::string& pre, int D = 0) { return cfg.attn_qk_norm == 2 ? P(pre + ".q_scale", D ? D : cfg.attn_dim_head) : nullptr; }
  const float* k_scale_of(const std::string& pre, int D = 0) { return cfg.attn_qk_norm == 2 ? P(pre + ".k_scale", D ? D : cfg.attn_dim_head) : nullptr; }
  const float* null_kv_of(const std::string& pre, int D = 0) {
    if (!D) D = cfg.attn_dim_head;
    const float* raw_nkv = P(pre + ".null_kv", 2 * D);
    if (!cfg.attn_qk_norm) return raw_nkv;
    const float* ks = k_scale_of(pre, D);
    return cached("null_kv_qknorm" + std::to_string(cfg.attn_qk_norm) + ":" + pre, (size_t)2 * D, [&](float* dst) {
      KD_HIP_THROW(hipMemcpyAsync(dst, raw_nkv, (size_t)2 * D * sizeof(float), hipMemcpyDeviceToDevice, 0));
      KD_THROW_IF(launch_l2norm_heads(dst, 2 * D, 1, 1, D, ks, 0));
    });
  }

  T cross_attn(const T& x, const std::string& pre, const T& c) {
    const int dim = x.C, D = (int)(numel(pre + ".null_kv") / 2), inner = (int)(numel(pre + ".to_q.weight") / dim);
    if (D != 32 && D != 64 && D != 128)
      throw std::runtime_error("'" + pre + "': the attention kernels are built for dim_head 32, 64 and 128");
    const int H = inner / D;
    if (H < 1 || H * D != inner) throw std::runtime_error("'" + pre + ".to_q.weight' is no whole number of heads");
    T xn = layernorm(x, P(pre + ".norm.g", dim), nullptr);
    T q = linear(xn, P(pre + ".to_q.weight", (int64_t)inner * dim), nullptr, inner);
    free(xn);
    T kv;
    {
      auto ph = cond_scope();
      kv = linear(c, P(pre + ".to_kv.weight", (int64_t)2 * inner * c.C), nullptr, 2 * inner);
      if (cfg.attn_qk_norm) qk_norm(kv, 2 * inner, H, k_scale_of(pre, D), D);
    }
    const float* nkv = null_kv_of(pre, D);
    if (cfg.attn_qk_norm) qk_norm(q, inner, H, q_scale_of(pre, D), D);
    T o = alloc(x.B, x.H, x.W, inner);
    {
      const Ref qr = at(q), kr = at(kv), vr = kr.floats(inner), outr = at(o);
      int Bx = x.B, Nq = x.HW(), Nc = c.HW();
      float scale = attn_scale(D);
      emit([=](hipStream_t s) {
        KVSeg s0{kr.f(), vr.f(), 2 * inner, Nc};
        KVSeg s1{nullptr, nullptr, 0, 0};
        return launch_attention(qr.f(), inner, nkv, nkv + D, s0, s1, outr.f(), inner, Bx, Nq, H, H, D, scale, s);
      }, "xattn Nq" + std::to_string(Nq) + " Nk" + std::to_string(Nc + 1));
      u->macs += (int64_t)Bx * H * Nq * (Nc + 1) * D * 2;
    }
    free(q);
    free(kv);
    T proj = linear(o, P(pre + ".to_out.0.weight", (int64_t)dim * inner), nullptr, dim);
    free(o);
    T y = layernorm(proj, P(pre + ".to_out.1.g", dim), nullptr, &x, ACT_NONE, nullptr, nullptr, true);
    free(proj);
    return y;
  }

  T transformer(const T& x, const std::string& pre, const T* ctx, const T* dst = nullptr, bool plain = false, int depth = 1) {
    if (plain) return transformer_layer(x, pre + ".fn.fn", std::string(), ctx, dst, true);
    if (depth < 1) throw std::runtime_error("plan: TransformerBlock depth must be at least 1");
    T cur = x;
    for (int i = 0; i < depth; ++i) {
      const std::string l = pre + ".layers." + std::to_string(i);
      T y = transformer_layer(cur, l + ".0", l + ".1", ctx, i == depth - 1 ? dst : nullptr, false);
      if (i > 0) free(cur);
      cur = y;
    }
    return cur;
  }
  T transformer_layer(const T& x, const std::string& a, const std::string& f, const T* ctx, const T* dst, bool plain) {
    int H = cfg.attn_heads, D = cfg.attn_dim_head, inner = H * D, dim = x.C;
    const bool qkv1 = cfg.conv_algo == 0 && kd_switch("KD_QKV_FUSED", 1) != 0;
    T xn = layernorm(x, P(a + ".norm.g", dim), nullptr, nullptr, ACT_NONE, nullptr, nullptr, false,
                     qkv1 && linear_is_x3(x, inner + 2 * D) ? 1 : 0);
    const float* wq = P(a + ".to_q.weight", (int64_t)inner * dim);
    const float* wkv = P(a + ".to_kv.weight", (int64_t)2 * D * dim);
    T q, kv, qkv;
    if (qkv1) {
      const float* wqkv = cached("qkv:" + a, (size_t)(inner + 2 * D) * dim, [&](float* dst) {
        KD_HIP_THROW(hipMemcpyAsync(dst, wq, (size_t)inner * dim * sizeof(float), hipMemcpyDeviceToDevice, 0));
        KD_HIP_THROW(hipMemcpyAsync(dst + (size_t)inner * dim, wkv, (size_t)2 * D * dim * sizeof(float), hipMemcpyDeviceToDevice, 0));
      });
      qkv = linear(xn, wqkv, nullptr, inner + 2 * D);
      q = qkv;
      q.C = inner; q.ld = inner + 2 * D; q.coff = 0;
      kv = qkv;
      kv.C = 2 * D; kv.ld = inner + 2 * D; kv.coff = inner;
    } else {
      q = linear(xn, wq, nullptr, inner);
      kv = linear(xn, wkv, nullptr, 2 * D);
    }
    free(xn);
    T ckv;
    bool has_ctx = ctx != nullptr;
    if (has_ctx) {
      auto ph = cond_scope();
      T cn = layernorm(*ctx, P(a + ".to_context.0.weight", ctx->C), P(a + ".to_context.0.bias", ctx->C));
      ckv = linear(cn, P(a + ".to_context.1.weight", (int64_t)2 * D * ctx->C), P(a + ".to_context.1.bias", 2 * D),
                   2 * D);
      free(cn);
      if (cfg.attn_qk_norm) qk_norm(ckv, 2 * D, 1, k_scale_of(a));
    }
    const float* nkv = null_kv_of(a);
    if (cfg.attn_qk_norm) {
      qk_norm(q, q.LD(), H, q_scale_of(a));
      qk_norm(kv, kv.LD(), 1, k_scale_of(a));
    }
    T o = alloc(x.B, x.H, x.W, inner);
    {
      const Ref qr = at(q), kr = at(kv), outr = at(o), ck = has_ctx ? at(ckv) : Ref();
      int Bx = x.B, N = x.HW(), Nc = has_ctx ? ctx->HW() : 0;
      const int ldq = q.LD(), ldkv = kv.LD();
      float scale = attn_scale();
      emit([=](hipStream_t s) {
        KVSeg s0{nullptr, nullptr, 0, 0};
        if (ck) s0 = KVSeg{ck.f(), ck.floats(D).f(), 2 * D, Nc};
        KVSeg s1{kr.f(), kr.floats(D).f(), ldkv, N};
        return launch_attention(qr.f(), ldq, nkv, nkv + D, s0, s1, outr.f(), inner, Bx, N, H, 1, D, scale, s);
      }, "attn N" + std::to_string(N));
      u->macs += (int64_t)Bx * H * N * (N + Nc + 1) * D * 2;
    }
    if (qkv1) {
      free(qkv);
    } else {
      free(q);
      free(kv);
    }
    if (has_ctx) free(ckv);
    T proj = linear(o, P(a + ".to_out.0.weight", (int64_t)dim * inner), nullptr, dim);
    free(o);
    if (plain) {
      T x1 = layernorm(proj, P(a + ".to_out.1.g", dim), nullptr, &x);
      free(proj);
      return x1;
    }
    T h0;
    int hidden = dim * cfg.ff_mult_x2 / 2;
    const bool gelu_late = linear_is_x3(proj, hidden);
    T x1 = layernorm(proj, P(a + ".to_out.1.g", dim), nullptr, &x, ACT_NONE, P(f + ".0.g", dim), &h0, false, gelu_late ? 2 : 0);
    free(proj);
    T h1 = linear(h0, P(f + ".1.weight", (int64_t)hidden * dim), nullptr, hidden, gelu_late ? ACT_NONE : ACT_GELU);
    free(h0);
    T h2 = layernorm(h1, P(f + ".3.g", hidden), nullptr, nullptr, gelu_late ? ACT_GELU : ACT_NONE, nullptr, nullptr, false,
                     linear_is_x3(h1, dim, &x1, dst) ? 1 : 0);
    free(h1);
    T y = linear(h2, P(f + ".4.weight", (int64_t)dim * hidden), nullptr, dim, ACT_NONE, &x1, dst);
    free(h2);
    free(x1);
    return y;
  }

  T gca(const T& h, const std::string& pre) {
    int C = h.C, hid = std::max(3, C / 2);
    const float* wk = P(pre + ".to_k.weight", C);
    const float* bk = P(pre + ".to_k.bias", 1);
    const float* w0 = P(pre + ".net.0.weight", (int64_t)hid * C);
    const float* b0 = P(pre + ".net.0.bias", hid);
    const float* w2 = P(pre + ".net.2.weight", (int64_t)C * hid);
    const float* b2 = P(pre + ".net.2.bias", C);
    int Bx = h.B, HW = h.HW();
    const Ref hr = at(h);
    if (gca_gate_fused_ok(C, hid) && h.B > 1 && kd_switch("KD_GCA_FUSED", 1)) {
      T scratch = alloc_bytes(gca_scratch_floats(h.B, h.HW(), C) * sizeof(float));
      T gate = alloc(h.B, 1, 1, C);
      const Ref sr = at(scratch), gr = at(gate);
      emit([=](hipStream_t s) {
        return launch_gca_gate(hr.f(), wk, bk, sr.f(), w0, b0, hid, w2, b2, gr.f(), Bx, HW, C, s);
      }, "gca_gate HW" + std::to_string(HW) + " C" + std::to_string(C));
      u->macs += (int64_t)Bx * HW * C * 2 + (int64_t)Bx * C * hid * 2;
      free(scratch);
      return gate;
    }
    T logits = alloc(h.B, h.H, h.W, 1);
    T pooled = alloc(h.B, 1, 1, C);
    T scratch = alloc_bytes(gca_scratch_floats(h.B, h.HW(), C) * sizeof(float));
    const Ref lr = at(logits), pr = at(pooled), sr = at(scratch);
    emit([=](hipStream_t s) {
      return launch_gca_pool(hr.f(), wk, bk, lr.f(), pr.f(), sr.f(), Bx, HW, C, s);
    }, "gca_pool HW" + std::to_string(HW) + " C" + std::to_string(C));
    u->macs += (int64_t)Bx * HW * C * 2;
    free(logits);
    free(scratch);
    T hidden = alloc(h.B, 1, 1, hid);
    skinny(at(pooled), C, w0, b0, at(hidden), hid, h.B, C, hid, ACT_NONE, ACT_SILU);
    free(pooled);
    T gate = alloc(h.B, 1, 1, C);
    skinny(at(hidden), hid, w2, b2, at(gate), C, h.B, hid, C, ACT_NONE, ACT_SIGMOID);
    free(hidden);
    return gate;
  }

  enum class Conv3x3 { Wino4, WinoGemm, WinoFused, Direct };
  struct Conv3x3Choice { Conv3x3 algo; int images; };
  Conv3x3Choice conv3x3_choice(const T& x, int cout) const {
    const int images = wino4_images(x, cout);
    if (images > 0) return {Conv3x3::Wino4, images};
    const bool fused = fwino_ok(x, cout);
    auto gemm_ok = [&] {
      if (cfg.conv_algo == 1 || cfg.conv_algo == 4) return false;
      const int min_cin = cfg.conv_algo >= 32 ? cfg.conv_algo : 256;
      if (cfg.conv_algo < 32 && fused) return false;
      if ((x.H & 1) || (x.W & 1) || x.C < min_cin || x.C % 32 || cout <= 32 || cout % 4) return false;
      const int64_t Mt = (int64_t)x.B * (x.H / 2) * (x.W / 2);
      return Mt % 256 == 0 && 16 * Mt < 0x7fffffff && (int64_t)16 * cout * x.C * 4 < 0x7fffffff;
    };
    if (gemm_ok()) return {Conv3x3::WinoGemm, 0};
    if (fused && x.C <= wino_fused_gn_max_cin() && x.C % cfg.resnet_groups == 0 && (int64_t)x.H * x.W * x.LD() * 4 < 0x7fffffff)
      return {Conv3x3::WinoFused, 0};
    return {Conv3x3::Direct, 0};
  }
  bool fwino_ok(const T& x, int cout) const {
    if (cfg.conv_algo == 1 || cfg.conv_algo == 2) return false;
    if (x.C < 32 || !wino_fused128_ok(x.B, x.H, x.W, x.C, cout)) return false;
    if (cfg.conv_algo == 3) return true;
    return (int64_t)x.B * (x.H / 16) * (x.W / 16) * (cout / 64) >= 256;
  }
  int wino4_images(const T& x, int cout) const {
    const int cap = cfg.wino4_max_images > 0 ? cfg.wino4_max_images : x.B;
    if (cap >= x.B && wino4_whole_ok(x, cout)) return x.B;
    if (cap >= x.B && (cfg.conv_algo != 0 || cfg.wino43_min_cin != 0 || cfg.gemm_bf16x3 < 0 || !recorded())) return 0;
    if (cap < x.B && !wino4_whole_ok(x, cout)) return 0;
    for (int ns = 2; ns <= x.B; ++ns) {
      if (x.B % ns) continue;
      T xs = x;
      xs.B = x.B / ns;
      if (xs.B > cap || (int64_t)xs.B * x.H * x.W * x.LD() * 4 >= ((int64_t)1 << 32)) continue;
      const int64_t Mt = (int64_t)xs.B * (x.H / 4) * (x.W / 4);
      if (cap >= x.B && ((x.H & 3) || (x.W & 3) || !gemm_bf16x3_ok(36, Mt, cout, x.C))) continue;
      if (wino4_whole_ok(xs, cout)) return xs.B;
    }
    return 0;
  }
  bool wino4_whole_ok(const T& x, int cout) const {
    if (cfg.conv_algo != 0 && cfg.conv_algo != 4) return false;
    if (cfg.wino43_min_cin < 0 && cfg.conv_algo == 0) return false;
    if ((x.H & 3) || (x.W & 3) || x.C % 32 || cout % 64 || cout < 64) return false;
    const int64_t Mt = (int64_t)x.B * (x.H / 4) * (x.W / 4);
    if (Mt % 128 || 36 * Mt >= 0x7fffffff || (int64_t)36 * cout * x.C * 4 >= 0x7fffffff) return false;
    if (cfg.conv_algo == 4) return true;
    if ((36 * Mt / 128) * (cout / 64) < 512) return false;
    int thr = cfg.wino43_min_cin > 0 ? cfg.wino43_min_cin : 512;
    if (cfg.wino43_min_cin == 0 && cfg.gemm_bf16x3 >= 0 && gemm_bf16x3_ok(36, Mt, cout, x.C)) thr = 128;
    return x.C >= thr;
  }
  T wino4_block(const T& x, int Bx, const std::string& gn_prefix, int ss_col, const std::string& conv_prefix, int Cout,
                const T* res, int skip_c0, float skip_scale) {
    const int Cin = x.C, G = cfg.resnet_groups, H = x.H, W = x.W, HW = x.HW(), nset = x.B / Bx;
    const int64_t Mt = (int64_t)Bx * (H / 4) * (W / 4);
    const float* gamma = P(gn_prefix + ".weight", Cin);
    const float* beta = P(gn_prefix + ".bias", Cin);
    const float* bias = P(conv_prefix + ".bias", Cout);
    const float* wsrc = raw(conv_prefix + ".weight", (int64_t)Cout * Cin * 9);
    float* U = cached("wino4:" + conv_prefix, (size_t)36 * Cout * Cin,
                      [&](float* dst) { KD_THROW_IF(launch_wino4_pack(wsrc, dst, Cout, Cin, 0)); });
    emit_gn_stats(x, gamma, beta, ss_col, nullptr);
    const bool x3 = cfg.gemm_bf16x3 >= 0 && recorded() && gemm_bf16x3_ok(36, Mt, Cout, Cin);
    const bool v_f32 = cfg.gemm_bf16x3 == 2 || (cfg.gemm_bf16x3 == 0 && (int64_t)Cin * Cout < 40 * (6 * (int64_t)Cin + 4 * Cout));
    const bool x3_planes = x3 && !v_f32;
    T V = x3_planes ? alloc_bytes((size_t)36 * Mt * Cin * 6) : alloc(1, 1, (int)(36 * Mt), Cin);
    T D = alloc(1, 1, (int)(36 * Mt), Cout);
    T y = alloc(x.B, H, W, Cout);
    const std::string shape = " M" + std::to_string((int64_t)Bx * HW) + " Cin" + std::to_string(Cin) + " Cout" +
                              std::to_string(Cout);
    const bool sg = Cout % 64 == 0;
    const int seg_nchunk = (H / 4) * (W / 4);
    const size_t sgo_all = sg ? add_seg(y, 0, Cout / 16, seg_nchunk) : 0;
    const Ref vr = at(V), dr = at(D);
    for (int st = 0; st < nset; ++st) {
      const int b0 = st * Bx;
      {
        const Ref xr = image(x, b0), sr = at(gn_stats_t).floats((int64_t)b0 * G * 2);
        const Film ss = film(ss_col, b0);
        const int ldx = x.LD();
        emit([=](hipStream_t s) {
          if (x3_planes)
            return launch_wino4_in3(xr.f(), ldx, sr.f(), gamma, beta, ss.row.f(), ss.ld, vr.f(), Bx, H, W, Cin, G, s, skip_c0, skip_scale);
          return launch_wino4_in(xr.f(), ldx, sr.f(), gamma, beta, ss.row.f(), ss.ld, vr.f(), Bx, H, W, Cin, G, s, skip_c0, skip_scale);
        }, (x3_planes ? "wino4_in3" : "wino4_in") + shape);
      }
      if (x3) {
        const float* U3 = cached("wino4x3:" + conv_prefix, ((size_t)36 * Cout * Cin * 3 + 1) / 2,
                                 [&](float* dst) { KD_THROW_IF(launch_split3(U, dst, 36, Cout, Cin, 0)); });
        emit_x3_gemm(vr, U3, dr, 36, Mt, Cout, Cin, !x3_planes, nullptr, "wino4", shape, (int64_t)Bx * HW * Cout * Cin * 9);
      } else {
        ConvOpt o;
        o.wz_rows = (int)Mt;
        o.wz_count = 36;
        o.dst = &D;
        o.macs_override = (int64_t)Bx * HW * Cout * Cin * 9;
        conv(V, U, nullptr, Cout, 1, 1, 0, o);
        if (recorded()) u->op_label.back() = "wino4 gemm" + shape;
      }
      {
        const Ref seg = sg ? seg_at(sgo_all, Cout / 16, seg_nchunk, b0) : Ref(), yr = image(y, b0), rr = image(res, b0);
        const int ldres = res ? res->LD() : 0;
        emit([=](hipStream_t s) {
          return launch_wino4_out(dr.f(), bias, rr.f(), ldres, yr.f(), Cout, seg.d(), Bx, H, W, Cout, s);
        }, "wino4_out" + shape);
      }
    }
    free(V);
    free(D);
    return y;
  }

  T wino_block(const T& x, const std::string& gn_prefix, int ss_col, const std::string& conv_prefix, int Cout,
               const T* res) {
    const int Cin = x.C, G = cfg.resnet_groups, Bx = x.B, H = x.H, W = x.W, HW = x.HW();
    const int64_t Mt = (int64_t)Bx * (H / 2) * (W / 2);
    const float* gamma = P(gn_prefix + ".weight", Cin);
    const float* beta = P(gn_prefix + ".bias", Cin);
    const float* bias = P(conv_prefix + ".bias", Cout);
    const float* wsrc = raw(conv_prefix + ".weight", (int64_t)Cout * Cin * 9);
    float* U = cached("wino:" + conv_prefix, (size_t)16 * Cout * Cin,
                      [&](float* dst) { KD_THROW_IF(launch_wino_pack(wsrc, dst, Cout, Cin, 0)); });
    const int64_t slice_mb = cfg.wino_slice_mb;
    int64_t nt_slice = Mt;
    if (slice_mb > 0) {
      nt_slice = (slice_mb << 20) / (64 * (int64_t)(Cin + Cout)) / 256 * 256;
      nt_slice = std::min(Mt, std::max<int64_t>(nt_slice, 256));
    }
    emit_gn_stats(x, gamma, beta, ss_col, nullptr);
    T V = alloc(1, 1, (int)(16 * nt_slice), Cin);
    T D = alloc(1, 1, (int)(16 * nt_slice), Cout);
    T y = alloc(Bx, H, W, Cout);
    const bool sg = Cout % 16 == 0;
    const Ref seg = sg ? seg_at(add_seg(y, 0, Cout / 16, (H / 2) * (W / 2))) : Ref();
    const std::string shape = " M" + std::to_string((int64_t)Bx * HW) + " Cin" + std::to_string(Cin) + " Cout" +
                              std::to_string(Cout);
    const Ref xr = at(x), vr = at(V), dr = at(D), yr = at(y), rr = at(res), st = at(gn_stats_t);
    const Film ss = film(ss_col);
    const int ldx = x.LD(), ldres = res ? res->LD() : 0;
    for (int64_t t0 = 0; t0 < Mt; t0 += nt_slice) {
      const int64_t nt = std::min(nt_slice, Mt - t0);
      emit([=](hipStream_t s) {
        return launch_wino_in(xr.f(), ldx, st.f(), gamma, beta, ss.row.f(), ss.ld, vr.f(), Bx, H, W, Cin, G, t0, nt, s);
      }, "wino_in" + shape);
      T Vs = V, Ds = D;
      Vs.W = (int)(16 * nt);
      Ds.W = (int)(16 * nt);
      ConvOpt o;
      o.wz_rows = (int)nt;
      o.dst = &Ds;
      o.macs_override = nt * 4 * Cout * Cin * 9;
      conv(Vs, U, nullptr, Cout, 1, 1, 0, o);
      if (recorded()) u->op_label.back() = "wino gemm" + shape;
      emit([=](hipStream_t s) {
        return launch_wino_out(dr.f(), bias, rr.f(), ldres, yr.f(), Bx, H, W, Cout, t0, nt, s, seg.d());
      }, "wino_out" + shape);
    }
    free(V);
    free(D);
    return y;
  }

  T fwino_gn_conv(const T& x, const std::string& gn_prefix, int ss_col, const std::string& conv_prefix, int Cout,
                  const T* res) {
    const int Cin = x.C, G = cfg.resnet_groups, Bx = x.B, H = x.H, W = x.W;
    const float* gamma = P(gn_prefix + ".weight", Cin);
    const float* beta = P(gn_prefix + ".bias", Cin);
    const float* bias = P(conv_prefix + ".bias", Cout);
    const float* wsrc = raw(conv_prefix + ".weight", (int64_t)Cout * Cin * 9);
    float* U = cached("winof_gn128:" + conv_prefix, (size_t)16 * Cout * Cin,
                      [&](float* dst) { KD_THROW_IF(launch_wino_fused128_pack(wsrc, dst, Cout, Cin, 0, WF_U_SCALE)); });
    T ab = alloc_bytes((size_t)Bx * Cin * 2 * sizeof(float));
    T y = alloc(Bx, H, W, Cout);
    const Ref abr = at(ab);
    if (!emit_gn_stats(x, gamma, beta, ss_col, &ab)) {
      const Ref st = at(gn_stats_t);
      const Film ss = film(ss_col);
      emit([=](hipStream_t s) { return launch_gn_fold(st.f(), gamma, beta, ss.row.f(), ss.ld, abr.f(), Bx, Cin, G, s); },
           "gn fold C" + std::to_string(Cin));
    }
    const bool so_ = Cout % 16 == 0;
    const Ref seg = so_ ? seg_at(add_seg(y, 0, Cout / 16, (int)wino_fused_out_stats_chunks(H, W, Cout, Cout / 16))) : Ref();
    const Ref xr = at(x), yr = at(y), rr = at(res);
    const int ldres = res ? res->LD() : 0, ldx = x.LD();
    const int64_t m = (int64_t)Bx * H * W * Cout * Cin * 9;
    const std::string shape_key = std::to_string(Bx) + "x" + std::to_string(H) + "x" + std::to_string(W) + "x" + std::to_string(Cout);
    const float* items = cached("winof128_items:" + shape_key, wino_fused128_items_count(Bx, H, W, Cout) * 4,
                                [&](float* dst) { KD_THROW_IF(launch_wino_fused128_items(dst, Bx, H, W, Cout, 0)); });
    emit([=](hipStream_t s) {
      return launch_wino_fused_gn128(xr.f(), ldx, abr.f(), U, bias, rr.f(), ldres, yr.f(), Bx, H, W, Cin, Cout, seg.d(),
                                     so_ ? Cout / 16 : 0, items, s);
    }, "wino fused M" + std::to_string((int64_t)Bx * H * W) + " Cin" + std::to_string(Cin) + " Cout" +
           std::to_string(Cout), m);
    free(ab);
    count_macs(m, (int64_t)Bx * H * W * 4 * Cout * ((Cin / 4 + 3) / 4 * 16));
    return y;
  }

  T gn_conv3x3(const T& x, bool free_x, const std::string& pre, int ss_col, int Cout, const T* res, int skip_c0 = -1,
               float skip_scale = 1.0f) {
    const Conv3x3Choice c = conv3x3_choice(x, Cout);
    if (skip_c0 >= 0 && c.algo != Conv3x3::Wino4 && c.algo != Conv3x3::WinoFused)
      throw std::runtime_error("plan: folded skip scale on a conv path that cannot apply it: " + pre);
    const std::string gn = pre + ".groupnorm", cv = pre + ".project";
    T y;
    switch (c.algo) {
      case Conv3x3::Wino4: y = wino4_block(x, c.images, gn, ss_col, cv, Cout, res, skip_c0, skip_scale); break;
      case Conv3x3::WinoGemm: y = wino_block(x, gn, ss_col, cv, Cout, res); break;
      case Conv3x3::WinoFused: y = fwino_gn_conv(x, gn, ss_col, cv, Cout, res); break;
      case Conv3x3::Direct: {
        T a = gn_silu(x, gn, ss_col);
        if (free_x) free(x);
        ConvOpt o;
        o.res = res;
        o.want_seg = true;
        y = conv(a, pack_conv(cv + ".weight", Cout, a.C, a.C, 3), P(cv + ".bias", Cout), Cout, 3, 1, 1, o);
        free(a);
        return y;
      }
    }
    if (free_x) free(x);
    return y;
  }

  T resnet(const T& x, const std::string& pre, int dim_out, const T* ctx, bool use_gca, const T* ct = nullptr,
           const T* out_slot = nullptr, int skip_c0 = -1, float skip_scale = 1.0f) {
    bool has_cross = has(pre + ".cross_attn.to_q.weight");
    if (has_cross && !ctx) throw std::runtime_error("cross-attention block without conditioning tokens: " + pre);
    int dim_in = x.C;
    T h = gn_conv3x3(x, false, pre + ".block1", -1, dim_out, nullptr, skip_c0, skip_scale);
    if (has_cross) {
      T h2 = lin_cross_pre.count(pre) ? linear_cross_attn(h, pre + ".cross_attn", *ctx) : cross_attn(h, pre + ".cross_attn", *ctx);
      free(h);
      h = h2;
    }
    auto it = tmlp_off.find(pre);
    int ss_col = it != tmlp_off.end() ? it->second : -1;
    bool has_res_conv = has(pre + ".res_conv.weight");
    T h2 = gn_conv3x3(h, true, pre + ".block2", ss_col, dim_out, (!use_gca && !has_res_conv) ? &x : nullptr);
    if (!use_gca && !has_res_conv) return h2;
    if (skip_c0 >= 0 && !has_res_conv) throw std::runtime_error("plan: folded skip scale without a skip conv: " + pre);
    const float* w_res = nullptr;
    if (has_res_conv) {
      w_res = P(pre + ".res_conv.weight", (int64_t)dim_out * dim_in);
      if (skip_c0 >= 0) {
        const float* src = w_res;
        w_res = cached("res_conv_skipscaled:" + pre + ":" + std::to_string(skip_c0), (size_t)dim_out * dim_in, [&](float* dst) {
          KD_THROW_IF(launch_copy_scale_rows(src, dim_in, dst, dim_in, dim_in, 1.0f, dim_out, 0));
          KD_THROW_IF(launch_copy_scale_rows(dst + skip_c0, dim_in, dst + skip_c0, dim_in, dim_in - skip_c0, skip_scale,
                                             dim_out, 0));
        });
      }
    }
    T out;
    if (use_gca) {
      T gate = gca(h2, pre + ".gca");
      if (has_res_conv) {
        ConvOpt o;
        o.gate_src = &h2;
        o.gate = &gate;
        o.want_seg = true;
        if (ct) o.dst = ct;
        out = conv(x, w_res, P(pre + ".res_conv.bias", dim_out), dim_out, 1, 1, 0, o);
      } else {
        out = out_slot ? *out_slot : alloc(x.B, x.H, x.W, dim_out);
        if (out.C != dim_out) throw std::runtime_error("plan: output slot of the wrong width: " + pre);
        const Ref ar = at(h2), gr = at(gate), rr = at(x), yr = at(out);
        int Bx = x.B, HW = x.HW(), ldr = x.LD(), ldy = out.LD();
        const bool sg = dim_out % 16 == 0;
        const Ref seg = sg ? seg_at(add_seg(out, 0, dim_out / 16, gate_add_chunks(Bx, HW))) : Ref();
        emit([=](hipStream_t s) {
          return launch_gate_add(ar.f(), gr.f(), rr.f(), ldr, yr.f(), ldy, seg.d(), Bx, HW, dim_out, s);
        }, "gate_add HW" + std::to_string(HW) + " C" + std::to_string(dim_out));
      }
      free(gate);
    } else {
      ConvOpt o;
      o.res = &h2;
      o.want_seg = true;
      if (ct) o.dst = ct;
      out = conv(x, w_res, P(pre + ".res_conv.bias", dim_out), dim_out, 1, 1, 0, o);
    }
    free(h2);
    return out;
  }

  X3Epi downsample_x3_epi(const T& x, int ldy) const {
    X3Epi e;
    e.lda = x.LD();
    e.ldy = ldy;
    e.a_tap_c = x.C;
    e.a_wi = x.W;
    e.a_hi = x.H;
    e.hw = (x.H / 2) * (x.W / 2);
    return e;
  }
  bool downsample_x3_ok(const T& x, int Cout, int ldy = 0) const {
    if ((x.H & 1) || (x.W & 1) || x.C % 16) return false;
    return x3_epi_layer_ok((int64_t)x.B * (x.H / 2) * (x.W / 2), Cout, 4 * x.C, 256, downsample_x3_epi(x, ldy ? ldy : Cout));
  }
  T downsample_x3(const T& x, const std::string& pre, const float* w_taps , const float* bias, int Cout,
                  const T* dst = nullptr) {
    const int C = x.C, K = 4 * C, Ho = x.H / 2, Wo = x.W / 2;
    const int64_t M = (int64_t)x.B * Ho * Wo;
    const float* W3 = cached("x3down:" + pre, ((size_t)Cout * K * 3 + 1) / 2, [&](float* dst) {
      float* wk = nullptr;
      KD_HIP_THROW(hipMalloc((void**)&wk, (size_t)Cout * K * sizeof(float)));
      int rc = 0;
      for (int t = 0; t < 4 && !rc; ++t)
        rc = launch_copy_scale_rows(w_taps + (size_t)t * Cout * C, C, wk + (size_t)t * C, K, C, 1.0f, Cout, 0);
      if (!rc) rc = launch_split3(wk, dst, 1, Cout, K, 0);
      hipError_t er = hipDeviceSynchronize();
      (void)hipFree(wk);
      KD_THROW_IF(rc);
      KD_HIP_THROW(er);
    });
    T y = dst ? *dst : alloc(x.B, Ho, Wo, Cout);
    const X3Epi base = downsample_x3_epi(x, y.LD());
    const int span = y.C;
    const bool sg = Cout % 16 == 0 && span % 16 == 0 && (Ho * Wo) % 32 == 0;
    last_seg_nchunk = sg ? Ho * Wo / gemm_bf16x3_shape(1, (int)M, Cout, K, u->cus).seg_rows() : 0;
    const Ref seg = sg ? seg_at(add_seg(y, 0, span / 16, last_seg_nchunk)) : Ref();
    auto epi_of = [=]() {
      X3Epi e = base;
      e.bias = bias;
      if (seg) {
        e.seg = seg.d();
        e.seg_nseg = span / 16;
      }
      return e;
    };
    const std::string shape = " M" + std::to_string(M) + " Cin" + std::to_string(C) + " Cout" + std::to_string(Cout);
    emit_x3_gemm(at(x), W3, at(y), 1, M, Cout, K, true, epi_of, "conv k2", shape, M * Cout * K);
    return y;
  }
  T downsample(const T& x, const std::string& pre, int dim_out) {
    if (u->cross_embed_downsample) return cross_embed_downsample(x, pre, dim_out);
    if (cfg.downsample_conv4) {
      ConvOpt o4;
      o4.want_seg = true;
      return conv(x, pack_conv(pre + ".weight", dim_out, x.C, x.C, 4), P(pre + ".bias", dim_out), dim_out, 4, 2, 1, o4);
    }
    const float* src = raw(pre + ".1.weight", (int64_t)dim_out * 4 * x.C);
    const int C = x.C;
    float* w = cached("unshuffle:" + pre, (size_t)dim_out * 4 * C,
                      [&](float* dst) { KD_THROW_IF(launch_pack_unshuffle(src, dst, dim_out, C, 0)); });
    if (downsample_x3_ok(x, dim_out)) return downsample_x3(x, pre, w, P(pre + ".1.bias", dim_out), dim_out);
    ConvOpt o;
    o.want_seg = true;
    return conv(x, w, P(pre + ".1.bias", dim_out), dim_out, 2, 2, 0, o);
  }
  T cross_embed_downsample(const T& x, const std::string& pre, int dim_out) {
    if (dim_out & 1) throw std::runtime_error("cross_embed_downsample: odd dim_out " + std::to_string(dim_out) + " at " + pre);
    if ((x.H & 1) || (x.W & 1)) throw std::runtime_error("cross_embed_downsample: odd map at " + pre);
    const int d2 = dim_out / 2, d4 = dim_out - d2, C = x.C;
    const float* w2 = pack_conv(pre + ".convs.0.weight", d2, C, C, 2);
    const float* b2 = P(pre + ".convs.0.bias", d2);
    T y = alloc(x.B, x.H / 2, x.W / 2, dim_out);
    if (downsample_x3_ok(x, d2, dim_out)) {
      downsample_x3(x, pre + ".convs.0", w2, b2, d2, &y);
    } else {
      ConvOpt o2;
      o2.dst = &y;
      o2.want_seg = true;
      o2.seg_c0 = 0;
      o2.seg_cn = dim_out;
      conv(x, w2, b2, d2, 2, 2, 0, o2);
    }
    const int chunks2 = last_seg_nchunk;
    ConvOpt o4;
    o4.dst = &y;
    o4.yoff = d2;
    o4.want_seg = true;
    o4.seg_c0 = 0;
    o4.seg_cn = dim_out;
    conv(x, pack_conv(pre + ".convs.1.weight", d4, C, C, 4), P(pre + ".convs.1.bias", d4), d4, 4, 2, 1, o4);
    auto it = seg_of.find(y.at());
    if (it != seg_of.end() && (it->second.parts.size() != 1 || chunks2 == 0 || chunks2 != last_seg_nchunk)) {
      for (auto& sp : it->second.parts)
        if (sp.owned) arena.release(sp.off);
      seg_of.erase(it);
    }
    return y;
  }
  T upsample_nearest(const T& x, const std::string& pre, int dim_out, const T* ct = nullptr) {
    const int C = x.C;
    const float* wsrc = raw(pre + ".1.weight", (int64_t)dim_out * C * 9);
    const float* b = P(pre + ".1.bias", dim_out);
    T y = ct ? *ct : alloc(x.B, 2 * x.H, 2 * x.W, dim_out);
    if (y.B != x.B || y.H != 2 * x.H || y.W != 2 * x.W) throw std::runtime_error("plan: upsample target of the wrong shape");
    if (const char* why = upsample_nearest_refusal(x.LD(), y.LD(), y.coff, x.B, x.H, x.W, C, dim_out))
      throw std::runtime_error(std::string(why) + " (" + pre + ": Cin " + std::to_string(C) + ", Cout " + std::to_string(dim_out) + ")");
    if ((x.coff & 3)) throw std::runtime_error("upsample_nearest_conv3x3: input channel offset must be a multiple of 4 (" + pre + ")");
    const float* wp = cached("upnearest_w:" + pre, upsample_nearest_weight_floats(C, dim_out),
                             [&](float* dst) { KD_THROW_IF(launch_upsample_nearest_pack(wsrc, dst, dim_out, C, 0)); });
    const Ref xr = at(x), yr = base(y);
    const int ldx = x.LD(), ldy = y.LD(), yoff = y.coff, Bx = x.B, H = x.H, W = x.W;
    const int64_t M = (int64_t)Bx * H * W;
    const int64_t m = 4 * M * dim_out * C * 9;
    emit([=](hipStream_t s) {
      return launch_upsample_nearest_conv3x3(xr.f(), ldx, wp, b, yr.f(), ldy, yoff, Bx, H, W, C, dim_out, s);
    }, "upsample nearest conv3 M" + std::to_string(M) + " Cin" + std::to_string(C) + " Cout" + std::to_string(dim_out), m);
    count_macs(m, 4 * M * dim_out * 4 * C);
    return y;
  }
  T upsample(const T& x, const std::string& pre, int dim_out, const T* ct = nullptr) {
    if (u->upsample_nearest) return upsample_nearest(x, pre, dim_out, ct);
    const float* wsrc = raw(pre + ".net.0.weight", (int64_t)4 * dim_out * x.C);
    const float* bsrc = raw(pre + ".net.0.bias", 4 * dim_out);
    const int C = x.C;
    float* b = nullptr;
    float* w = cached("shuffle_w:" + pre, (size_t)4 * dim_out * C, [&](float* dst) {
      b = cached("shuffle_b:" + pre, (size_t)4 * dim_out, [](float*) {});
      KD_THROW_IF(launch_pack_shuffle(wsrc, bsrc, dst, b, dim_out, C, 0));
    });
    if (!b) b = cached("shuffle_b:" + pre, (size_t)4 * dim_out, [](float*) {});
    ConvOpt o;
    o.act = ACT_SILU;
    o.out_mode = OUT_PIXSHUF;
    o.want_seg = true;
    if (ct) o.dst = ct;
    return conv(x, w, b, 4 * dim_out, 1, 1, 0, o);
  }
  static constexpr int COMBINE_GROUPS = 8;
  T gn_silu_plain(const T& x, const float* gamma, const float* beta, int G) {
    const int Bx = x.B, HW = x.HW(), C = x.C, ldx = x.LD();
    if (C % G || (C / G) % 4) throw std::runtime_error("upsample_combiner: GroupNorm(" + std::to_string(G) + ") needs groups of 4 n channels, C = " + std::to_string(C));
    T st = alloc_bytes((size_t)Bx * G * 2 * sizeof(float)), part = alloc_bytes(gn_partial_bytes(Bx, HW, C, G));
    T y = alloc(x.B, x.H, x.W, C);
    const Ref xr = at(x), yr = at(y), sr = at(st), pr = at(part);
    emit([=](hipStream_t s) { return launch_gn_stats(xr.f(), ldx, sr.f(), pr.d(), Bx, HW, C, G, 1e-5f, s); },
         "gn stats HW" + std::to_string(HW) + " C" + std::to_string(C));
    emit([=](hipStream_t s) { return launch_gn_apply_silu(xr.f(), ldx, sr.f(), gamma, beta, nullptr, 0, yr.f(), Bx, HW, C, G, s); },
         "gn apply HW" + std::to_string(HW) + " C" + std::to_string(C));
    free(st);
    free(part);
    return y;
  }
  void combine_fmap(const T& f, int i, int scale, const T& cat, int yoff) {
    const int G = COMBINE_GROUPS, dim = cfg.dim, Cin = f.C, Bx = f.B, H = f.H, W = f.W;
    const std::string pre = "upsample_combiner.fmap_convs." + std::to_string(i);
    const float* gamma = P(pre + ".groupnorm.weight", Cin);
    const float* beta = P(pre + ".groupnorm.bias", Cin);
    const float* bias = P(pre + ".project.bias", dim);
    if (cat.B != Bx || cat.H != scale * H || cat.W != scale * W || scale < 1)
      throw std::runtime_error("plan: " + pre + ": the map is no integer fraction of the full resolution");
    if (scale == 1) {
      T a = gn_silu_plain(f, gamma, beta, G);
      ConvOpt o;
      o.dst = &cat;
      o.yoff = yoff;
      conv(a, pack_conv(pre + ".project.weight", dim, Cin, Cin, 3), bias, dim, 3, 1, 1, o);
      free(a);
      return;
    }
    if (const char* why = upsample_scale_refusal(f.LD(), cat.LD(), cat.coff + yoff, Bx, H, W, Cin, dim, scale))
      throw std::runtime_error(std::string(why) + " (" + pre + ": Cin " + std::to_string(Cin) + ", Cout " + std::to_string(dim) + ")");
    if ((f.coff & 3)) throw std::runtime_error("upsample_nearest_gn_conv3x3: input channel offset must be a multiple of 4 (" + pre + ")");
    const float* wsrc = raw(pre + ".project.weight", (int64_t)dim * Cin * 9);
    const float* wp = cached("upcombine_w:" + pre, upsample_scale_weight_floats(Cin, dim),
                             [&](float* dst) { KD_THROW_IF(launch_upsample_scale_pack(wsrc, dst, dim, Cin, 0)); });
    SegPart sp[2];
    int nsp = 0;
    bool fold = Cin % G == 0 && (Cin / G) % 16 == 0 && seg_sources(f, sp, nsp, G);
    for (int k = 0; k < nsp; ++k) fold = fold && sp[k].scale == 1.0f && sp[k].ab_mul == 1.0f;
    T src = f, ab;
    if (fold) {
      ab = alloc_bytes((size_t)Bx * Cin * 2 * sizeof(float));
      const SegPart a = sp[0], b2 = nsp > 1 ? sp[1] : SegPart();
      const Ref pa = seg_at(a.off), pb = nsp > 1 ? seg_at(b2.off) : Ref(), abr = at(ab);
      const int HW = f.HW();
      emit([=](hipStream_t s) {
        SegSrc s0{pa.d(), a.nseg, a.nchunk, a.c0, a.scale, a.ab_mul};
        SegSrc s1{pb.d(), b2.nseg, b2.nchunk, b2.c0, b2.scale, b2.ab_mul};
        return launch_gn_fold_seg(s0, s1, gamma, beta, nullptr, 0, abr.f(), nullptr, Bx, Cin, G, (double)HW * (Cin / G), 1e-5f, s);
      }, "gn fold seg HW" + std::to_string(HW) + " C" + std::to_string(Cin));
    } else {
      src = gn_silu_plain(f, gamma, beta, G);
    }
    const Ref xr = at(src), abr = fold ? at(ab) : Ref(), yr = base(cat);
    const int ldx = src.LD(), ldy = cat.LD(), yo = cat.coff + yoff;
    const int64_t M = (int64_t)Bx * H * W;
    const int64_t m = M * scale * scale * dim * Cin * 9;
    emit([=](hipStream_t s) {
      return launch_upsample_scale_conv3x3(xr.f(), ldx, abr.f(), wp, bias, yr.f(), ldy, yo, Bx, H, W, Cin, dim, scale, s);
    }, "upsample combine s=" + std::to_string(scale) + " M" + std::to_string(M) + " Cin" + std::to_string(Cin) + " Cout" +
           std::to_string(dim) + (fold ? " affine" : ""), m);
    count_macs(m, M * dim * Cin * (scale == 2 ? 16 : 25));
    free(fold ? ab : src);
  }
  T concat_skip(const T& x, const T& skip, float scale) {
    T y = alloc(x.B, x.H, x.W, x.C + skip.C);
    int Ca = x.C, Cb = skip.C, lda = x.LD(), ldb = skip.LD();
    int64_t rows = x.rows();
    const Ref ar = at(x), br = at(skip), ya = at(y), yb = ya.floats(Ca);
    emit([=](hipStream_t s) {
      if (launch_copy_scale_rows(ar.f(), lda, ya.f(), Ca + Cb, Ca, 1.0f, rows, s)) return 1;
      return launch_copy_scale_rows(br.f(), ldb, yb.f(), Ca + Cb, Cb, scale, rows, s);
    }, "concat rows" + std::to_string(rows) + " C" + std::to_string(Ca + Cb));
    return y;
  }
  void concat_skip_tail(const T& y, int Ca, const T& skip, float scale) {
    const Ref br = at(skip), yb = at(y).floats(Ca);
    int Cb = skip.C, ldb = skip.LD(), ldy = y.LD();
    int64_t rows = y.rows();
    emit([=](hipStream_t s) {
      return launch_copy_scale_rows(br.f(), ldb, yb.f(), ldy, Cb, scale, rows, s);
    }, "concat tail rows" + std::to_string(rows) + " C" + std::to_string(Ca + Cb));
  }
  void concat_head(const T& ct, const T& x, const char* what = "concat head") {
    const Ref ar = at(x), yr = at(ct);
    int Ca = x.C, lda = x.LD(), ldy = ct.LD();
    int64_t rows = x.rows();
    emit([=](hipStream_t s) { return launch_copy_scale_rows(ar.f(), lda, yr.f(), ldy, Ca, 1.0f, rows, s); },
         std::string(what) + " rows" + std::to_string(rows) + " C" + std::to_string(Ca));
  }
  void scale_slice(const T& t, int c0, int n, float scale) {
    const Ref tr = at(t).floats(c0);
    int ld = t.LD();
    int64_t rows = t.rows();
    emit([=](hipStream_t s) {
      return launch_copy_scale_rows(tr.f(), ld, tr.f(), ld, n, scale, rows, s);
    }, "scale slice rows" + std::to_string(rows) + " C" + std::to_string(n));
  }

  void collect_time_mlps() {
    std::vector<std::string> names;
    const std::string suffix = ".time_mlp.1.weight";
    for (auto& kv : params) {
      const std::string& n = kv.first;
      if (n.size() > suffix.size() && n.compare(n.size() - suffix.size(), suffix.size(), suffix) == 0)
        names.push_back(n.substr(0, n.size() - suffix.size()));
    }
    std::sort(names.begin(), names.end());
    int tcd = u->time_cond_dim;
    int total = 0;
    for (auto& pre : names) {
      int64_t ne = numel(pre + suffix);
      if (ne % tcd) throw std::runtime_error("time_mlp weight of unexpected shape: " + pre);
      tmlp_off[pre] = total;
      total += (int)(ne / tcd);
    }
    tmlp_total = total;
    tmlp_prefixes = names;
    if (total == 0) return;
    tmlp_w = cached("time_mlps_w", (size_t)total * tcd, [&](float* dst) {
      for (auto& pre : names) {
        int64_t ne = numel(pre + suffix);
        KD_HIP_THROW(hipMemcpyAsync(dst + (size_t)tmlp_off[pre] * tcd, raw(pre + suffix), (size_t)ne * 4,
                                    hipMemcpyDeviceToDevice, 0));
      }
    });
    tmlp_b = cached("time_mlps_b", (size_t)total, [&](float* dst) {
      for (auto& pre : names) {
        int64_t ne = numel(pre + suffix);
        KD_HIP_THROW(hipMemcpyAsync(dst + tmlp_off[pre], raw(pre + ".time_mlp.1.bias", ne / tcd),
                                    (size_t)(ne / tcd) * 4, hipMemcpyDeviceToDevice, 0));
      }
    });
// ... 43 lines not shown
```

### kidney-diffusion_amd/csrc/kernels_small.hip

```cpp
#include "common.h"

namespace kd {

typedef float f32x16 __attribute__((ext_vector_type(16)));
typedef float f32x4 __attribute__((ext_vector_type(4)));

__device__ __forceinline__ float act_s(float v, int act) {
  if (act == ACT_SILU) return v / (1.0f + expf(-v));
  if (act == ACT_GELU) return 0.5f * v * (1.0f + erff(v * 0.70710678118654752440f));
  if (act == ACT_SIGMOID) return 1.0f / (1.0f + expf(-v));
  return v;
}
__device__ __forceinline__ float wave_sum(float v) {
#pragma unroll
  for (int off = 32; off > 0; off >>= 1) v += __shfl_xor(v, off, 64);
  return v;
}

constexpr int SKM_UNROLL = 8;

template <int KW>
__global__ __launch_bounds__(64 * KW) void linear_skinny_mfma_kernel(const float* __restrict__ x, int ldx,
                                                                    const float* __restrict__ w,
                                                                    const float* __restrict__ bias,
                                                                    float* __restrict__ y, int ldy, int M, int K, int N,
                                                                    int in_act, int act) {
  __shared__ float part[KW > 1 ? (KW - 1) * 16 * 64 : 1];
  const int lane = threadIdx.x & 63, i = lane & 31, h = lane >> 5;
  const int kw = threadIdx.x >> 6;
  const int n0 = blockIdx.x * 32, m0 = blockIdx.y * 32;
  const int n = min(n0 + i, N - 1);
  const int m = m0 + i;
  const bool m_ok = m < M;
  const float* wp = w + (int64_t)n * K + 4 * h;
  const float* xp = x + (int64_t)(m_ok ? m : 0) * ldx + 4 * h;
  f32x16 acc;
#pragma unroll
  for (int r = 0; r < 16; ++r) acc[r] = 0.f;
  const f32x4 z = {0.f, 0.f, 0.f, 0.f};
  const int kper = KW > 1 ? ((K + KW * 8 * SKM_UNROLL - 1) / (KW * 8 * SKM_UNROLL)) * (8 * SKM_UNROLL) : K;
  const int k_lo = kw * kper, k_hi = min(K, k_lo + kper);
  for (int k0 = k_lo; k0 < k_hi; k0 += 8 * SKM_UNROLL) {
    f32x4 a[SKM_UNROLL], b[SKM_UNROLL];
#pragma unroll
    for (int u = 0; u < SKM_UNROLL; ++u) {
      int k = k0 + 8 * u + 4 * h;
      bool ok = k < k_hi;
      a[u] = ok ? *(const f32x4*)(wp + k0 + 8 * u) : z;
      b[u] = (ok && m_ok) ? *(const f32x4*)(xp + k0 + 8 * u) : z;
    }
#pragma unroll
    for (int u = 0; u < SKM_UNROLL; ++u) {
      if (in_act != ACT_NONE) {
#pragma unroll
        for (int e = 0; e < 4; ++e) b[u][e] = act_s(b[u][e], in_act);
      }
#pragma unroll
      for (int s = 0; s < 4; ++s) acc = __builtin_amdgcn_mfma_f32_32x32x2f32(a[u][s], b[u][s], acc, 0, 0, 0);
    }
  }
  if (KW > 1) {
    if (kw > 0) {
#pragma unroll
      for (int r = 0; r < 16; ++r) part[((kw - 1) * 16 + r) * 64 + lane] = acc[r];
    }
    __syncthreads();
    if (kw > 0) return;
#pragma unroll
    for (int q = 0; q < KW - 1; ++q)
#pragma unroll
      for (int r = 0; r < 16; ++r) acc[r] += part[(q * 16 + r) * 64 + lane];
  }
  if (!m_ok) return;
  float* yr = y + (int64_t)m * ldy;
  const bool vec = (ldy & 3) == 0 && (((uintptr_t)y) & 15) == 0;
#pragma unroll
  for (int g = 0; g < 4; ++g) {
    const int nb = n0 + 8 * g + 4 * h;
    float v[4];
#pragma unroll
    for (int e = 0; e < 4; ++e) {
      int nn = nb + e;
      v[e] = act_s(acc[4 * g + e] + ((bias && nn < N) ? bias[nn] : 0.f), act);
    }
    if (vec && nb + 3 < N) {
      f32x4 o = {v[0], v[1], v[2], v[3]};
      *(f32x4*)(yr + nb) = o;
    } else {
#pragma unroll
      for (int e = 0; e < 4; ++e)
        if (nb + e < N) yr[nb + e] = v[e];
    }
  }
}

int launch_linear_skinny(const float* x, int ldx, const float* w, const float* bias, float* y, int ldy, int M,
                         int K, int N, int in_act, int act, hipStream_t s) {
  KD_REQUIRE(M > 0 && N > 0 && K > 0, "skinny linear: empty");
  const bool mfma_ok = (K & 3) == 0 && (ldx & 3) == 0 && (((uintptr_t)x) & 15) == 0 && (((uintptr_t)w) & 15) == 0;
  if (!mfma_ok) return launch_linear_skinny_valu(x, ldx, w, bias, y, ldy, M, K, N, in_act, act, s);
  if (M == 1 && K <= 16384) return launch_linear_gemv(x, w, bias, y, K, N, in_act, act, s);
  dim3 grid((N + 31) / 32, (M + 31) / 32);
  if (K >= 512)
    hipLaunchKernelGGL(linear_skinny_mfma_kernel<4>, grid, dim3(256), 0, s, x, ldx, w, bias, y, ldy, M, K, N, in_act, act);
  else
    hipLaunchKernelGGL(linear_skinny_mfma_kernel<1>, grid, dim3(64), 0, s, x, ldx, w, bias, y, ldy, M, K, N, in_act, act);
  KD_HIP_CHECK(hipGetLastError());
  return 0;
}

constexpr int GCA_ROWS = 256;
static inline int gca_rows(int HW, int B) {
  int r = GCA_ROWS;
  while ((HW + r - 1) / r > 1024) r *= 2;
  while (r > 32 && (int64_t)((HW + r - 1) / r) * B < 1024 && (HW + r / 2 - 1) / (r / 2) <= 1024) r /= 2;
  return r;
}
constexpr int GCA_MAXT = 8;
constexpr int GCA_U = 4;

template <int T, int RPW>
__global__ __launch_bounds__(256) void gca_partial_kernel(const float* __restrict__ x, const float* __restrict__ wk,
                                                          const float* __restrict__ bk, float* __restrict__ part,
                                                          int HW, int C, int rows) {
  extern __shared__ float sm[];
  const int b = blockIdx.y, chunk = blockIdx.x, nchunks = gridDim.x;
  const int lane = threadIdx.x & 63, wave = threadIdx.x >> 6;
  constexpr int LPR = 64 / RPW;
  const int sub = RPW == 2 ? (lane >> 5) : 0;
  const int li = RPW == 2 ? (lane & 31) : lane;
  const int C4 = C >> 2;
  const int p0 = chunk * rows, p1 = min(HW, p0 + rows);
  f32x4 wv[T], acc[T];
  const f32x4 z = {0.f, 0.f, 0.f, 0.f};
#pragma unroll
  for (int t = 0; t < T; ++t) {
    int c4 = li + LPR * t;
    wv[t] = c4 < C4 ? *(const f32x4*)(wk + c4 * 4) : z;
    acc[t] = z;
  }
  const float bias = bk[0];
  float mrun = -INFINITY, lrun = 0.f;
  const int stride = 4 * RPW;
  for (int pb = p0 + wave * RPW + sub; pb < p1; pb += stride * GCA_U) {
    f32x4 xv[GCA_U][T];
#pragma unroll
    for (int u = 0; u < GCA_U; ++u) {
      const int p = pb + u * stride;
      const float* xr = x + ((int64_t)b * HW + (p < p1 ? p : p0)) * C;
#pragma unroll
      for (int t = 0; t < T; ++t) {
        int c4 = li + LPR * t;
        xv[u][t] = c4 < C4 ? *(const f32x4*)(xr + c4 * 4) : z;
      }
    }
#pragma unroll
    for (int u = 0; u < GCA_U; ++u) {
      float d = 0.f;
#pragma unroll
      for (int t = 0; t < T; ++t)
        d += (xv[u][t][0] * wv[t][0] + xv[u][t][1] * wv[t][1]) + (xv[u][t][2] * wv[t][2] + xv[u][t][3] * wv[t][3]);
#pragma unroll
      for (int off = LPR / 2; off > 0; off >>= 1) d += __shfl_xor(d, off, 64);
      if (pb + u * stride < p1) {
        const float logit = d + bias;
        const float mnew = fmaxf(mrun, logit);
        const float corr = expf(mrun - mnew), pw = expf(logit - mnew);
        lrun = lrun * corr + pw;
#pragma unroll
        for (int t = 0; t < T; ++t) acc[t] = acc[t] * corr + xv[u][t] * pw;
        mrun = mnew;
      }
    }
  }
  if (RPW == 2) {
    const float mo = __shfl_xor(mrun, 32, 64), lo = __shfl_xor(lrun, 32, 64);
    const float mn = fmaxf(mrun, mo);
    const float e1 = mrun == -INFINITY ? 0.f : expf(mrun - mn), e2 = mo == -INFINITY ? 0.f : expf(mo - mn);
#pragma unroll
    for (int t = 0; t < T; ++t) {
      f32x4 ao;
#pragma unroll
      for (int e = 0; e < 4; ++e) ao[e] = __shfl_xor(acc[t][e], 32, 64);
      acc[t] = acc[t] * e1 + ao * e2;
    }
    lrun = lrun * e1 + lo * e2;
    mrun = mn;
  }
  float* sacc = sm;
  float* sml = sm + 4 * C;
  if (lane == 0) {
    sml[wave * 2] = mrun;
    sml[wave * 2 + 1] = lrun;
  }
  if (sub == 0) {
#pragma unroll
    for (int t = 0; t < T; ++t) {
      int c4 = li + LPR * t;
      if (c4 < C4) *(f32x4*)(sacc + wave * C + c4 * 4) = acc[t];
    }
  }
  __syncthreads();
  float mb = fmaxf(fmaxf(sml[0], sml[2]), fmaxf(sml[4], sml[6]));
  float sc[4], lb = 0.f;
#pragma unroll
  for (int wv_ = 0; wv_ < 4; ++wv_) {
    sc[wv_] = sml[wv_ * 2] == -INFINITY ? 0.f : expf(sml[wv_ * 2] - mb);
    lb += sml[wv_ * 2 + 1] * sc[wv_];
  }
  float* out = part + ((int64_t)b * nchunks + chunk) * (C + 2);
  for (int c = threadIdx.x; c < C; c += 256)
    out[2 + c] = (sacc[c] * sc[0] + sacc[C + c] * sc[1]) + (sacc[2 * C + c] * sc[2] + sacc[3 * C + c] * sc[3]);
  if (threadIdx.x == 0) {
    out[0] = mb;
    out[1] = lb;
  }
}

__global__ __launch_bounds__(256) void gca_combine_kernel(const float* __restrict__ part, float* __restrict__ pooled,
                                                          int nchunks, int C) {
  __shared__ float se[1024];
  __shared__ float red[8];
  __shared__ float sacc[16][16];
  const int b = blockIdx.x, lane = threadIdx.x & 63, wave = threadIdx.x >> 6;
  const int cl = threadIdx.x & 15, sub = threadIdx.x >> 4;
  const int c = blockIdx.y * 16 + cl;
  const float* pb = part + (int64_t)b * nchunks * (C + 2);
  float m = -INFINITY;
  for (int i = threadIdx.x; i < nchunks; i += 256) m = fmaxf(m, pb[(int64_t)i * (C + 2)]);
#pragma unroll
  for (int off = 32; off > 0; off >>= 1) m = fmaxf(m, __shfl_xor(m, off, 64));
  if (lane == 0) red[wave] = m;
  __syncthreads();
  const float mg = fmaxf(fmaxf(red[0], red[1]), fmaxf(red[2], red[3]));
  float l = 0.f;
  for (int i = threadIdx.x; i < nchunks; i += 256) {
    float e = expf(pb[(int64_t)i * (C + 2)] - mg);
    se[i] = e;
    l += pb[(int64_t)i * (C + 2) + 1] * e;
  }
  l = wave_sum(l);
  if (lane == 0) red[4 + wave] = l;
  __syncthreads();
  const float inv = 1.0f / ((red[4] + red[5]) + (red[6] + red[7]));
  float s = 0.f;
  if (c < C)
    for (int i = sub; i < nchunks; i += 16) s += pb[(int64_t)i * (C + 2) + 2 + c] * se[i];
  sacc[sub][cl] = s;
  __syncthreads();
  if (sub == 0 && c < C) {
    float t = 0.f;
#pragma unroll
    for (int k = 0; k < 16; ++k) t += sacc[k][cl];
    pooled[(int64_t)b * C + c] = t * inv;
  }
}

constexpr int GCAG_MAXC = 512;
__global__ __launch_bounds__(256) void gca_gate_kernel(const float* __restrict__ part, int nchunks, int C,
                                                       const float* __restrict__ w0, const float* __restrict__ b0, int hid,
                                                       const float* __restrict__ w2, const float* __restrict__ b2,
                                                       float* __restrict__ gate) {
  __shared__ float se[1024];
  __shared__ float red[8];
  __shared__ __attribute__((aligned(16))) float pooled[GCAG_MAXC];
  __shared__ __attribute__((aligned(16))) float hidden[GCAG_MAXC / 2];
  const int b = blockIdx.x, lane = threadIdx.x & 63, wave = threadIdx.x >> 6;
  const float* pb = part + (int64_t)b * nchunks * (C + 2);
  float m = -INFINITY;
  for (int i = threadIdx.x; i < nchunks; i += 256) m = fmaxf(m, pb[(int64_t)i * (C + 2)]);
#pragma unroll
  for (int off = 32; off > 0; off >>= 1) m = fmaxf(m, __shfl_xor(m, off, 64));
  if (lane == 0) red[wave] = m;
  __syncthreads();
  const float mg = fmaxf(fmaxf(red[0], red[1]), fmaxf(red[2], red[3]));
  float l = 0.f;
  for (int i = threadIdx.x; i < nchunks; i += 256) {
    const float e = expf(pb[(int64_t)i * (C + 2)] - mg);
    se[i] = e;
    l += pb[(int64_t)i * (C + 2) + 1] * e;
  }
  l = wave_sum(l);
  if (lane == 0) red[4 + wave] = l;
  __syncthreads();
  const float inv = 1.0f / ((red[4] + red[5]) + (red[6] + red[7]));
  for (int c = threadIdx.x; c < C; c += 256) {
    float s0 = 0.f, s1 = 0.f, s2 = 0.f, s3 = 0.f;
    int i = 0;
    for (; i + 3 < nchunks; i += 4) {
      s0 = fmaf(pb[(int64_t)i * (C + 2) + 2 + c], se[i], s0);
      s1 = fmaf(pb[(int64_t)(i + 1) * (C + 2) + 2 + c], se[i + 1], s1);
      s2 = fmaf(pb[(int64_t)(i + 2) * (C + 2) + 2 + c], se[i + 2], s2);
      s3 = fmaf(pb[(int64_t)(i + 3) * (C + 2) + 2 + c], se[i + 3], s3);
    }
    for (; i < nchunks; ++i) s0 = fmaf(pb[(int64_t)i * (C + 2) + 2 + c], se[i], s0);
    pooled[c] = ((s0 + s1) + (s2 + s3)) * inv;
  }
  __syncthreads();
  typedef float f32x4g __attribute__((ext_vector_type(4)));
  for (int h = threadIdx.x; h < hid; h += 256) {
    const f32x4g* wr = (const f32x4g*)(w0 + (int64_t)h * C);
    float a0 = 0.f, a1 = 0.f, a2 = 0.f, a3 = 0.f;
    for (int c4 = 0; c4 < C / 4; ++c4) {
      const f32x4g wv = wr[c4], pv = *(const f32x4g*)(pooled + 4 * c4);
      a0 = fmaf(wv[0], pv[0], a0);
      a1 = fmaf(wv[1], pv[1], a1);
      a2 = fmaf(wv[2], pv[2], a2);
      a3 = fmaf(wv[3], pv[3], a3);
    }
    const float v = ((a0 + a1) + (a2 + a3)) + b0[h];
    hidden[h] = v / (1.0f + expf(-v));
  }
  __syncthreads();
  for (int n = threadIdx.x; n < C; n += 256) {
    const float* wr = w2 + (int64_t)n * hid;
    float a0 = 0.f, a1 = 0.f;
    int h = 0;
    if ((hid & 3) == 0) {
      float a2 = 0.f, a3 = 0.f;
      for (; h < hid; h += 4) {
        const f32x4g wv = *(const f32x4g*)(wr + h), hv = *(const f32x4g*)(hidden + h);
        a0 = fmaf(wv[0], hv[0], a0);
        a1 = fmaf(wv[1], hv[1], a1);
        a2 = fmaf(wv[2], hv[2], a2);
        a3 = fmaf(wv[3], hv[3], a3);
      }
      a0 += a2;
      a1 += a3;
    } else {
      for (; h < hid; ++h) a0 = fmaf(wr[h], hidden[h], a0);
    }
    const float v = (a0 + a1) + b2[n];
    gate[(int64_t)b * C + n] = 1.0f / (1.0f + expf(-v));
  }
}

bool gca_gate_fused_ok(int C, int hid) {
  return C % 4 == 0 && C <= GCAG_MAXC && hid <= GCAG_MAXC / 2 && hid > 0;
}

static int launch_gca_partial(const float* x, const float* wk, const float* bk, float* scratch, int B, int HW, int C, int rows,
                              int chunks, hipStream_t s) {
  size_t smem = (size_t)(4 * C + 8) * sizeof(float);
  const int C4 = C / 4;
  dim3 grid(chunks, B), blk(256);
  if (C4 == 32) hipLaunchKernelGGL((gca_partial_kernel<1, 2>), grid, blk, smem, s, x, wk, bk, scratch, HW, C, rows);
  else if (C4 <= 64) hipLaunchKernelGGL((gca_partial_kernel<1, 1>), grid, blk, smem, s, x, wk, bk, scratch, HW, C, rows);
  else if (C4 <= 128) hipLaunchKernelGGL((gca_partial_kernel<2, 1>), grid, blk, smem, s, x, wk, bk, scratch, HW, C, rows);
  else if (C4 <= 256) hipLaunchKernelGGL((gca_partial_kernel<4, 1>), grid, blk, smem, s, x, wk, bk, scratch, HW, C, rows);
  else hipLaunchKernelGGL((gca_partial_kernel<8, 1>), grid, blk, smem, s, x, wk, bk, scratch, HW, C, rows);
  KD_HIP_CHECK(hipGetLastError());
  return 0;
}

int launch_gca_gate(const float* x, const float* wk, const float* bk, float* scratch, const float* w0, const float* b0, int hid,
                    const float* w2, const float* b2, float* gate, int B, int HW, int C, hipStream_t s) {
  KD_REQUIRE(gca_gate_fused_ok(C, hid), "fused GlobalContext gate needs C % 4 == 0, C <= 512, hidden <= 256");
  KD_REQUIRE((((uintptr_t)w0 | (uintptr_t)w2) & 15) == 0, "fused GlobalContext gate: 16-byte aligned weights");
  const int rows = gca_rows(HW, B), chunks = (HW + rows - 1) / rows;
  if (launch_gca_partial(x, wk, bk, scratch, B, HW, C, rows, chunks, s)) return 1;
  hipLaunchKernelGGL(gca_gate_kernel, dim3(B), dim3(256), 0, s, scratch, chunks, C, w0, b0, hid, w2, b2, gate);
  KD_HIP_CHECK(hipGetLastError());
  return 0;
}

size_t gca_scratch_floats(int B, int HW, int C) {
  int rows = gca_rows(HW, B), chunks = (HW + rows - 1) / rows;
  return (size_t)B * chunks * (C + 2);
}

int launch_gca_pool(const float* x, const float* wk, const float* bk, float* , float* pooled,
                    float* scratch, int B, int HW, int C, hipStream_t s) {
  KD_REQUIRE(C % 4 == 0 && C <= 64 * 4 * GCA_MAXT, "gca needs C % 4 == 0 and C <= 2048");
  const int rows = gca_rows(HW, B), chunks = (HW + rows - 1) / rows;
  if (launch_gca_partial(x, wk, bk, scratch, B, HW, C, rows, chunks, s)) return 1;
  hipLaunchKernelGGL(gca_combine_kernel, dim3(B, (C + 15) / 16), dim3(256), 0, s, scratch, pooled, chunks, C);
  KD_HIP_CHECK(hipGetLastError());
  return 0;
}

}
```

### kidney-diffusion_amd/csrc/kernels_wino4.hip

```cpp
#include "common.h"

namespace kd {

namespace {
__device__ __forceinline__ float w4_silu(float v) {
  return v * __builtin_amdgcn_rcpf(1.0f + __builtin_amdgcn_exp2f(-1.4426950408889634f * v));
}

typedef float f32x2 __attribute__((ext_vector_type(2)));

template <class F>
__device__ __forceinline__ void w4_bt(const F (&d)[6], F (&t)[6]) {
  t[0] = 4.0f * d[0] - 5.0f * d[2] + d[4];
  t[1] = (d[3] + d[4]) - 4.0f * (d[1] + d[2]);
  t[2] = (d[4] - d[3]) + 4.0f * (d[1] - d[2]);
  t[3] = (d[4] - d[2]) + 2.0f * (d[3] - d[1]);
  t[4] = (d[4] - d[2]) + 2.0f * (d[1] - d[3]);
  t[5] = 4.0f * d[1] - 5.0f * d[3] + d[5];
}
template <class F>
__device__ __forceinline__ void w4_at(const F (&m)[6], F (&y)[4]) {
  const F a = m[1] + m[2], b = m[1] - m[2], c = m[3] + m[4], d = m[3] - m[4];
  y[0] = m[0] + a + c;
  y[1] = b + 2.0f * d;
  y[2] = a + 4.0f * c;
  y[3] = b + 8.0f * d + m[5];
}
}

__global__ __launch_bounds__(256) void wino4_pack_kernel(const float* __restrict__ w, float* __restrict__ U, int O, int I) {
  const int64_t total = (int64_t)O * I;
  for (int64_t idx = (int64_t)blockIdx.x * blockDim.x + threadIdx.x; idx < total;
       idx += (int64_t)gridDim.x * blockDim.x) {
    const float* g = w + idx * 9;
    float t[6][3];
#pragma unroll
    for (int k = 0; k < 3; ++k) {
      const float g0 = g[k], g1 = g[3 + k], g2 = g[6 + k];
      t[0][k] = g0 * 0.25f;
      t[1][k] = -(g0 + g1 + g2) * (1.0f / 6.0f);
      t[2][k] = -(g0 - g1 + g2) * (1.0f / 6.0f);
      t[3][k] = g0 * (1.0f / 24.0f) + g1 * (1.0f / 12.0f) + g2 * (1.0f / 6.0f);
      t[4][k] = g0 * (1.0f / 24.0f) - g1 * (1.0f / 12.0f) + g2 * (1.0f / 6.0f);
      t[5][k] = g2;
    }
#pragma unroll
    for (int r = 0; r < 6; ++r) {
      const float a0 = t[r][0], a1 = t[r][1], a2 = t[r][2];
      const float u[6] = {a0 * 0.25f,
                          -(a0 + a1 + a2) * (1.0f / 6.0f),
                          -(a0 - a1 + a2) * (1.0f / 6.0f),
                          a0 * (1.0f / 24.0f) + a1 * (1.0f / 12.0f) + a2 * (1.0f / 6.0f),
                          a0 * (1.0f / 24.0f) - a1 * (1.0f / 12.0f) + a2 * (1.0f / 6.0f),
                          a2};
#pragma unroll
      for (int s = 0; s < 6; ++s) U[(int64_t)(r * 6 + s) * total + idx] = u[s];
    }
  }
}

int launch_wino4_pack(const float* w_oihw, float* U, int O, int I, hipStream_t s) {
  const int64_t total = (int64_t)O * I;
  const int blocks = (int)((total + 255) / 256 < 8192 ? (total + 255) / 256 : 8192);
  hipLaunchKernelGGL(wino4_pack_kernel, dim3(blocks), dim3(256), 0, s, w_oihw, U, O, I);
  KD_HIP_CHECK(hipGetLastError());
  return 0;
}

template <bool PLANES>
__global__ __launch_bounds__(256) void wino4_in_kernel(const float* __restrict__ x, int ldx, const float* __restrict__ stats,
                                                       const float* __restrict__ gamma, const float* __restrict__ beta,
                                                       const float* __restrict__ scale_shift, int ld_ss,
                                                       float* __restrict__ V, int B, int H, int W, int C, int G, int64_t nt,
                                                       int mul_c0, float mul) {
  const int Ht = H >> 2, Wt = W >> 2, C2 = C >> 1;
  const int64_t idx = (int64_t)blockIdx.x * blockDim.x + threadIdx.x;
  if (idx >= nt * C2) return;
  int c;
  int64_t t;
  if (PLANES) {
    const int64_t w = idx >> 6;
    const int lane = (int)(idx & 63), nkc = C / X3_BK;
    c = (int)(w % nkc) * X3_BK + (lane & 7) * 2;
    t = (w / nkc) * 8 + (lane >> 3);
  } else {
    c = (int)(idx % C2) * 2;
    t = idx / C2;
  }
  const int tx = (int)(t % Wt);
  const int ty = (int)((t / Wt) % Ht);
  const int b = (int)(t / ((int64_t)Wt * Ht));
  f32x2 A = {1.0f, 1.0f}, Bc = {0.0f, 0.0f};
  const bool norm = stats != nullptr;
  if (norm) {
#pragma unroll
    for (int e = 0; e < 2; ++e) {
      const int ce = c + e, g = ce / (C / G);
      const float mean = stats[(b * G + g) * 2], rstd = stats[(b * G + g) * 2 + 1];
      float a = rstd * gamma[ce];
      float bb = beta[ce] - mean * a;
      if (scale_shift) {
        const float sc = scale_shift[(int64_t)b * ld_ss + ce] + 1.0f;
        const float sh = scale_shift[(int64_t)b * ld_ss + C + ce];
        a *= sc;
        bb = bb * sc + sh;
      }
      A[e] = ce >= mul_c0 ? a * mul : a;
      Bc[e] = bb;
    }
  }
  f32x2 u[6][6];
  bool rok[6], cok[6];
  uint32_t rowp[6], colp[6];
#pragma unroll
  for (int r = 0; r < 6; ++r) {
    const int iy = 4 * ty - 1 + r;
    rok[r] = iy >= 0 && iy < H;
    rowp[r] = (uint32_t)((b * H + (iy < 0 ? 0 : iy >= H ? H - 1 : iy)) * W) * (uint32_t)(ldx * 4) + (uint32_t)(c * 4);
  }
#pragma unroll
  for (int s = 0; s < 6; ++s) {
    const int ix = 4 * tx - 1 + s;
    cok[s] = ix >= 0 && ix < W;
    colp[s] = (uint32_t)(ix < 0 ? 0 : ix >= W ? W - 1 : ix) * (uint32_t)(ldx * 4);
  }
  const __amdgpu_buffer_rsrc_t rsX = __builtin_amdgcn_make_buffer_rsrc((void*)x, 0, (int)(uint32_t)((int64_t)B * H * W * ldx * 4), 0x00020000);
  typedef unsigned int u32x2 __attribute__((ext_vector_type(2)));
#pragma unroll
  for (int r = 0; r < 6; ++r)
#pragma unroll
    for (int s = 0; s < 6; ++s) {
      const u32x2 q = __builtin_amdgcn_raw_buffer_load_b64(rsX, rowp[r] + colp[s], 0, 0);
      u[r][s] = f32x2{__uint_as_float(q[0]), __uint_as_float(q[1])};
    }
#pragma unroll
  for (int s = 0; s < 6; ++s) {
    f32x2 d[6];
#pragma unroll
    for (int r = 0; r < 6; ++r) {
      f32x2 v = u[r][s];
      if (norm) {
        v[0] = w4_silu(v[0] * A[0] + Bc[0]);
        v[1] = w4_silu(v[1] * A[1] + Bc[1]);
      }
      const f32x2 z = {0.0f, 0.0f};
      d[r] = (rok[r] && cok[s]) ? v : z;
    }
    f32x2 tcol[6];
    w4_bt(d, tcol);
#pragma unroll
    for (int r = 0; r < 6; ++r) u[r][s] = tcol[r];
  }
  if (PLANES) {
    const int64_t pstride = nt * C2, plane = 36 * pstride;
    uint32_t* out = (uint32_t*)V + ((int64_t)(c / X3_BK) * nt + t) * (X3_BK / 2) + (c % X3_BK) / 2;
#pragma unroll
    for (int r = 0; r < 6; ++r) {
      f32x2 trow[6];
      w4_bt(u[r], trow);
#pragma unroll
      for (int s = 0; s < 6; ++s) {
        uint32_t h, m, l;
        x3_split(trow[s], h, m, l);
        uint32_t* o = out + (int64_t)(r * 6 + s) * pstride;
        o[0] = h;
        o[plane] = m;
        o[2 * plane] = l;
      }
    }
    return;
  }
  float* out = V + t * C + c;
  const int64_t pstride = nt * C;
#pragma unroll
  for (int r = 0; r < 6; ++r) {
    f32x2 trow[6];
    w4_bt(u[r], trow);
#pragma unroll
    for (int s = 0; s < 6; ++s) *(f32x2*)(out + (int64_t)(r * 6 + s) * pstride) = trow[s];
  }
}

int launch_wino4_in(const float* x, int ldx, const float* stats, const float* gamma, const float* beta,
                    const float* scale_shift, int ld_ss, float* V, int B, int H, int W, int C, int G, hipStream_t s, int mul_c0,
                    float mul) {
  KD_REQUIRE(mul_c0 < 0 || stats, "Winograd F(4x4,3x3) input transform: a channel scale needs the GroupNorm form");
  if (mul_c0 < 0) mul_c0 = C;
  KD_REQUIRE(H % 4 == 0 && W % 4 == 0 && ldx >= C && C % 2 == 0 && ldx % 2 == 0 && ((uintptr_t)x & 7) == 0,
             "Winograd F(4x4,3x3) input transform needs H % 4 == 0, W % 4 == 0 and even C / row stride");
  KD_REQUIRE((int64_t)B * H * W * ldx * 4 < ((int64_t)1 << 32), "Winograd F(4x4,3x3) input transform: maps below 4 GB");
  const int64_t nt = (int64_t)B * (H / 4) * (W / 4), total = nt * (C / 2);
  hipLaunchKernelGGL(wino4_in_kernel<false>, dim3((unsigned)((total + 255) / 256)), dim3(256), 0, s, x, ldx, stats, gamma,
                     beta, scale_shift, ld_ss, V, B, H, W, C, G, nt, mul_c0, mul);
  KD_HIP_CHECK(hipGetLastError());
  return 0;
}

int launch_wino4_in3(const float* x, int ldx, const float* stats, const float* gamma, const float* beta,
                     const float* scale_shift, int ld_ss, void* V3, int B, int H, int W, int C, int G, hipStream_t s, int mul_c0,
                     float mul) {
  KD_REQUIRE(mul_c0 < 0 || stats, "Winograd F(4x4,3x3) input transform: a channel scale needs the GroupNorm form");
  if (mul_c0 < 0) mul_c0 = C;
  const int64_t nt = (int64_t)B * (H / 4) * (W / 4), total = nt * (C / 2);
  KD_REQUIRE((int64_t)B * H * W * ldx * 4 < ((int64_t)1 << 32), "Winograd F(4x4,3x3) input transform: maps below 4 GB");
  KD_REQUIRE(H % 4 == 0 && W % 4 == 0 && ldx >= C && C % X3_BK == 0 && ldx % 2 == 0 && ((uintptr_t)x & 7) == 0 && nt % 8 == 0 &&
                 ((uintptr_t)V3 & 3) == 0,
             "Winograd F(4x4,3x3) input transform to bf16x3 planes needs H % 4 == 0, W % 4 == 0, C % 16 == 0, tiles % 8 == 0");
  hipLaunchKernelGGL(wino4_in_kernel<true>, dim3((unsigned)((total + 255) / 256)), dim3(256), 0, s, x, ldx, stats, gamma, beta,
                     scale_shift, ld_ss, (float*)V3, B, H, W, C, G, nt, mul_c0, mul);
  KD_HIP_CHECK(hipGetLastError());
  return 0;
}

template <bool RES>
__global__ __launch_bounds__(256) void wino4_out_kernel(const float* __restrict__ D, const float* __restrict__ bias,
                                                        const float* __restrict__ res, int ldres, float* __restrict__ y,
                                                        int ldy, double* __restrict__ seg, int B, int H, int W, int C,
                                                        int64_t nt) {
  const int Ht = H >> 2, Wt = W >> 2, C2 = C >> 1;
  const int64_t idx = (int64_t)blockIdx.x * blockDim.x + threadIdx.x;
  if (idx >= nt * C2) return;
  const int c = (int)(idx % C2) * 2;
  const int64_t t = idx / C2;
  const int tx = (int)(t % Wt);
  const int ty = (int)((t / Wt) % Ht);
  const int b = (int)(t / ((int64_t)Wt * Ht));
  const float* in = D + t * C + c;
  const int64_t pstride = nt * C;
  f32x2 u[4][6];
#pragma unroll
  for (int s = 0; s < 6; ++s) {
    f32x2 m[6];
#pragma unroll
    for (int r = 0; r < 6; ++r) m[r] = *(const f32x2*)(in + (int64_t)(r * 6 + s) * pstride);
    f32x2 ycol[4];
    w4_at(m, ycol);
#pragma unroll
    for (int i = 0; i < 4; ++i) u[i][s] = ycol[i];
  }
  f32x2 bv = {0.0f, 0.0f};
  if (bias) bv = *(const f32x2*)(bias + c);
  f32x2 rnext[4];
#pragma unroll
  for (int j = 0; j < 4; ++j) rnext[j] = f32x2{0.0f, 0.0f};
  const int64_t pix0 = ((int64_t)b * H + 4 * ty) * W + 4 * tx;
  if (RES) {
#pragma unroll
    for (int j = 0; j < 4; ++j) rnext[j] = *(const f32x2*)(res + (pix0 + j) * ldres + c);
  }
  float s1 = 0.0f, s2 = 0.0f;
#pragma unroll
  for (int i = 0; i < 4; ++i) {
    f32x2 rcur[4];
#pragma unroll
    for (int j = 0; j < 4; ++j) rcur[j] = rnext[j];
    if (RES && i < 3) {
#pragma unroll
      for (int j = 0; j < 4; ++j) rnext[j] = *(const f32x2*)(res + (pix0 + (int64_t)(i + 1) * W + j) * ldres + c);
    }
    f32x2 o[4];
    w4_at(u[i], o);
#pragma unroll
    for (int j = 0; j < 4; ++j) {
      const int64_t pix = pix0 + (int64_t)i * W + j;
      f32x2 v = o[j] + bv;
      v += rcur[j];
      *(f32x2*)(y + pix * ldy + c) = v;
      s1 += v[0] + v[1];
      s2 = fmaf(v[0], v[0], fmaf(v[1], v[1], s2));
    }
  }
  if (seg) {
    double d1 = (double)s1, d2 = (double)s2;
#pragma unroll
    for (int off = 1; off <= 4; off <<= 1) {
      d1 += __shfl_xor(d1, off, 64);
      d2 += __shfl_xor(d2, off, 64);
    }
    if ((c & 15) == 0) {
      const int nchunk = Ht * Wt;
      double* op = seg + (((int64_t)b * (C >> 4) + (c >> 4)) * nchunk + (ty * Wt + tx)) * 2;
      op[0] = d1;
      op[1] = d2;
    }
  }
}

int launch_wino4_out(const float* D, const float* bias, const float* res, int ldres, float* y, int ldy, double* seg_partial,
                     int B, int H, int W, int C, hipStream_t s) {
  KD_REQUIRE(H % 4 == 0 && W % 4 == 0 && ldy >= C && C % 2 == 0 && ldy % 2 == 0 && ldres % 2 == 0 &&
                 (((uintptr_t)y | (uintptr_t)res | (uintptr_t)bias) & 7) == 0,
             "Winograd F(4x4,3x3) output transform needs H % 4 == 0, W % 4 == 0, even C / row strides, 8-byte aligned maps");
  KD_REQUIRE(!seg_partial || C % 128 == 0 || (C % 16 == 0 && ((int64_t)B * (H / 4) * (W / 4) * (C / 2)) % 64 == 0),
             "output statistics need whole waves of 16-channel segments");
  const int64_t nt = (int64_t)B * (H / 4) * (W / 4), total = nt * (C / 2);
  if (res)
    hipLaunchKernelGGL(wino4_out_kernel<true>, dim3((unsigned)((total + 255) / 256)), dim3(256), 0, s, D, bias, res, ldres, y, ldy,
                       seg_partial, B, H, W, C, nt);
  else
    hipLaunchKernelGGL(wino4_out_kernel<false>, dim3((unsigned)((total + 255) / 256)), dim3(256), 0, s, D, bias, res, ldres, y, ldy,
                       seg_partial, B, H, W, C, nt);
  KD_HIP_CHECK(hipGetLastError());
  return 0;
}

}
```

### kidney-diffusion_amd/imagen_pytorch/_engine.py

```python
from __future__ import annotations

import ctypes as C
import os
from pathlib import Path

KD_MAX_LEVELS = 8

_LIB_PATH = Path(__file__).resolve().parent.parent / "lib" / "libkd_engine.so"


class EngineUnavailable(RuntimeError):
    pass


class EngineError(RuntimeError):
    pass


class kd_unet_config_t(C.Structure):
    _fields_ = [
        ("dim", C.c_int),
        ("num_levels", C.c_int),
        ("dim_mults", C.c_int * KD_MAX_LEVELS),
        ("num_resnet_blocks", C.c_int * KD_MAX_LEVELS),
        ("layer_attns", C.c_int * KD_MAX_LEVELS),
        ("layer_cross_attns", C.c_int * KD_MAX_LEVELS),
        ("cond_dim", C.c_int),
        ("channels", C.c_int),
        ("cond_images_channels", C.c_int),
        ("lowres_cond", C.c_int),
        ("memory_efficient", C.c_int),
        ("init_conv_to_final_conv_residual", C.c_int),
        ("cond_on_text", C.c_int),
        ("text_tokens", C.c_int),
        ("attn_heads", C.c_int),
        ("attn_dim_head", C.c_int),
        ("ff_mult_x2", C.c_int),
        ("num_time_tokens", C.c_int),
        ("sinu_dim", C.c_int),
        ("resnet_groups", C.c_int),
        ("attend_at_middle", C.c_int),
        ("use_gca", C.c_int),
        ("batch", C.c_int),
        ("image_size", C.c_int),
        ("conv_algo", C.c_int),
        ("attn_qk_norm", C.c_int),
        ("downsample_conv4", C.c_int),
        ("mid_attn_plain", C.c_int),
        ("wino_slice_mb", C.c_int),
        ("wino43_min_cin", C.c_int),
        ("gemm_bf16x3", C.c_int),
        ("x3_linear", C.c_int),
        ("wino4_max_images", C.c_int),
    ]


class kd_param_t(C.Structure):
    _fields_ = [("name", C.c_char_p), ("d_data", C.c_void_p), ("numel", C.c_int64)]


class kd_schedule_t(C.Structure):
    _fields_ = [("T", C.c_int)] + [
        (n, C.POINTER(C.c_float))
        for n in ("log_snr", "alpha", "sigma", "alpha_next", "sigma_next", "c", "noise_scale", "rn_a", "rn_b")
    ]


class kd_sample_args_t(C.Structure):
    _fields_ = [
        ("objective", C.c_int),
        ("dynamic_threshold", C.c_int),
        ("percentile", C.c_float),
        ("resample_times", C.c_int),
        ("d_lowres", C.c_void_p),
        ("d_lowres_log_snr", C.c_void_p),
        ("d_cond_images", C.c_void_p),
        ("d_text_tokens", C.c_void_p),
        ("d_text_hiddens", C.c_void_p),
        ("d_inpaint_images", C.c_void_p),
        ("d_inpaint_masks", C.c_void_p),
        ("d_noise_step", C.c_void_p),
        ("d_noise_inpaint", C.c_void_p),
        ("d_noise_renoise", C.c_void_p),
        ("seed", C.c_uint64),
        ("use_graph", C.c_int),
        ("cond_scale", C.c_float),
        ("d_null_text_tokens", C.c_void_p),
        ("d_null_text_hiddens", C.c_void_p),
        ("lowres_log_snr_uniform", C.c_int),
        ("lowres_log_snr_value", C.c_float),
        ("cond_table", C.c_int),
        ("cond_table_max_mb", C.c_int),
    ]



class kd_edm_schedule_t(C.Structure):
    _fields_ = [("N", C.c_int), ("S_noise", C.c_float)] + [
        (n, C.POINTER(C.c_float))
        for n in ("sigma", "sigma_hat", "sigma_next", "churn", "euler_step", "heun_step", "renoise", "c_in_hat",
                  "c_skip_hat", "c_out_hat", "c_noise_hat", "c_in_next", "c_skip_next", "c_out_next", "c_noise_next")
    ]

class kd_unet_ext_t(C.Structure):
    _fields_ = [("self_cond", C.c_int), ("use_linear_attn", C.c_int * KD_MAX_LEVELS),
                ("use_linear_cross_attn", C.c_int * KD_MAX_LEVELS),
                ("cross_embed_downsample", C.c_int), ("upsample_nearest", C.c_int)]


class kd_unet_ext2_t(C.Structure):
    _fields_ = [("combine_upsample_fmaps", C.c_int)]


class kd_unet_ext3_t(C.Structure):
    _fields_ = [("layer_attns_depth", C.c_int * KD_MAX_LEVELS)]


SIGNATURES = {
    "kd_last_error": (C.c_char_p, []),
    "kd_version": (C.c_int, []),
    "kd_build_id": (C.c_char_p, []),
    "kd_unet_create": (C.c_int, [C.POINTER(kd_unet_config_t), C.POINTER(kd_param_t), C.c_int,
                                 C.POINTER(C.c_void_p)]),
    "kd_unet_destroy": (None, [C.c_void_p]),
    "kd_unet_hbm_bytes": (C.c_int64, [C.c_void_p]),
    "kd_unet_create_shared": (C.c_int, [C.POINTER(kd_unet_config_t), C.POINTER(kd_param_t), C.c_int, C.c_void_p,
                                        C.POINTER(C.c_void_p)]),
    "kd_unet_create_self_cond": (C.c_int, [C.POINTER(kd_unet_config_t), C.POINTER(kd_param_t), C.c_int, C.c_void_p,
                                           C.c_int, C.POINTER(C.c_void_p)]),
    "kd_unet_create_ext": (C.c_int, [C.POINTER(kd_unet_config_t), C.POINTER(kd_param_t), C.c_int, C.c_void_p,
                                     C.POINTER(kd_unet_ext_t), C.POINTER(C.c_void_p)]),
    "kd_unet_create_ext2": (C.c_int, [C.POINTER(kd_unet_config_t), C.POINTER(kd_param_t), C.c_int, C.c_void_p,
                                      C.POINTER(kd_unet_ext_t), C.POINTER(kd_unet_ext2_t), C.POINTER(C.c_void_p)]),
    "kd_unet_create_ext3": (C.c_int, [C.POINTER(kd_unet_config_t), C.POINTER(kd_param_t), C.c_int, C.c_void_p,
                                      C.POINTER(kd_unet_ext_t), C.POINTER(kd_unet_ext2_t), C.POINTER(kd_unet_ext3_t),
                                      C.POINTER(C.c_void_p)]),
    "kd_unet_weight_bytes": (C.c_int64, [C.c_void_p]),
    "kd_unet_macs": (C.c_int64, [C.c_void_p]),
    "kd_unet_mfma_macs": (C.c_int64, [C.c_void_p]),
    "kd_unet_mfma_bf16_macs": (C.c_int64, [C.c_void_p]),
    "kd_unet_num_launches": (C.c_int, [C.c_void_p]),
    "kd_unet_num_cond_launches": (C.c_int, [C.c_void_p]),
    "kd_unet_cond_table_build_ms": (C.c_float, [C.c_void_p, C.POINTER(C.c_int), C.POINTER(C.c_int)]),
    "kd_unet_cond_table_refused_bytes": (C.c_int64, [C.c_void_p]),
    "kd_unet_text_cond": (C.c_int, [C.c_void_p, C.c_void_p, C.c_void_p, C.c_int, C.c_int, C.c_void_p, C.c_void_p,
                                    C.c_void_p]),
    "kd_unet_profile": (C.c_int, [C.c_void_p, C.c_int, C.c_char_p, C.c_size_t, C.c_void_p]),
    "kd_unet_forward": (C.c_int, [C.c_void_p] + [C.c_void_p] * 8 + [C.c_void_p]),
    "kd_unet_forward_self_cond": (C.c_int, [C.c_void_p] + [C.c_void_p] * 9 + [C.c_void_p]),
    "kd_sample_loop": (C.c_int, [C.c_void_p, C.POINTER(kd_schedule_t), C.POINTER(kd_sample_args_t), C.c_void_p,
                                 C.c_void_p]),
    "kd_sample_steps": (C.c_int, [C.c_void_p, C.POINTER(kd_schedule_t), C.POINTER(kd_sample_args_t), C.c_void_p,
                                  C.c_int, C.c_int, C.c_void_p]),
    "kd_sample_build_cond_table": (C.c_int, [C.c_void_p, C.POINTER(kd_schedule_t), C.POINTER(kd_sample_args_t), C.c_int,
                                             C.c_int, C.c_int, C.POINTER(C.c_int), C.c_void_p]),
    "kd_sample_finalize": (C.c_int, [C.c_void_p, C.POINTER(kd_sample_args_t), C.c_void_p, C.c_void_p]),
    "kd_sample_last": (C.c_int, [C.c_void_p, C.c_int, C.c_void_p, C.c_void_p]),
    "kd_sample_set_self_cond": (C.c_int, [C.c_void_p, C.c_void_p, C.c_void_p]),
    "kd_edm_sample_loop": (C.c_int, [C.c_void_p, C.POINTER(kd_edm_schedule_t), C.POINTER(kd_sample_args_t), C.c_void_p,
                                     C.c_void_p]),
    "kd_edm_sample_steps": (C.c_int, [C.c_void_p, C.POINTER(kd_edm_schedule_t), C.POINTER(kd_sample_args_t), C.c_void_p,
                                      C.c_int, C.c_int, C.c_void_p]),
    "kd_conv2d_nhwc": (C.c_int, [C.c_void_p] * 4 + [C.c_int] * 10 + [C.c_void_p]),
    "kd_upsample_nearest_conv3x3_nhwc": (C.c_int, [C.c_void_p] * 4 + [C.c_int] * 7 + [C.c_void_p]),
    "kd_upsample_nearest_gn_conv3x3_nhwc": (C.c_int, [C.c_void_p, C.c_int] + [C.c_void_p] * 4 + [C.c_int] * 8 + [C.c_void_p]),
    "kd_conv3x3_winograd_nhwc": (C.c_int, [C.c_void_p] * 4 + [C.c_int] * 5 + [C.c_void_p]),
    "kd_conv3x3_winograd4_nhwc": (C.c_int, [C.c_void_p] * 5 + [C.c_int] * 6 + [C.c_float, C.c_void_p, C.c_int, C.c_void_p]),
    "kd_gemm_bf16x3": (C.c_int, [C.c_void_p] * 3 + [C.c_int] * 5 + [C.c_void_p]),
    "kd_linear_bf16x3": (C.c_int, [C.c_void_p, C.c_int, C.c_void_p, C.c_void_p, C.c_void_p, C.c_int, C.c_void_p, C.c_int,
                                   C.c_void_p, C.c_int, C.c_void_p, C.c_int, C.c_int, C.c_int, C.c_int, C.c_int, C.c_int, C.c_void_p,
                                   C.c_void_p]),
    "kd_linear_bf16x3_seg_rows": (C.c_int, [C.c_int, C.c_int, C.c_int]),
    "kd_downsample_bf16x3": (C.c_int, [C.c_void_p, C.c_int, C.c_void_p, C.c_void_p, C.c_void_p] + [C.c_int] * 5 + [C.c_void_p, C.c_void_p]),
    "kd_gn_conv3x3_winograd_fused_nhwc": (C.c_int, [C.c_void_p] * 8 + [C.c_int] * 6 + [C.c_float, C.c_void_p, C.c_int, C.c_void_p]),
    "kd_linattn_chunk_tokens": (C.c_int, []),
    "kd_linattn_dwconv_nhwc": (C.c_int, [C.c_void_p] * 6 + [C.c_int] * 4 + [C.c_void_p]),
    "kd_linattn_context": (C.c_int, [C.c_void_p, C.c_void_p, C.c_int, C.c_void_p, C.c_int, C.c_void_p, C.c_void_p, C.c_int,
                                     C.c_int, C.c_void_p, C.c_void_p, C.c_void_p, C.c_int, C.c_int, C.c_void_p]),
    "kd_linattn_apply": (C.c_int, [C.c_void_p, C.c_int, C.c_void_p, C.c_void_p, C.c_int, C.c_int, C.c_int, C.c_int,
                                   C.c_float, C.c_int, C.c_void_p]),
    "kd_linear_skinny": (C.c_int, [C.c_void_p, C.c_int, C.c_void_p, C.c_void_p, C.c_void_p] + [C.c_int] * 6 + [C.c_void_p]),
    "kd_global_context_gate": (C.c_int, [C.c_void_p] + [C.c_int] * 3 + [C.c_void_p] * 4 + [C.c_int] + [C.c_void_p] * 4 +
                               [C.c_int, C.c_void_p]),
    "kd_gate_add_nhwc": (C.c_int, [C.c_void_p] * 3 + [C.c_int, C.c_void_p, C.c_int, C.c_void_p] + [C.c_int] * 3 + [C.c_void_p]),
    "kd_gate_add_chunks": (C.c_int, [C.c_int, C.c_int]),
    "kd_gn_fold_seg": (C.c_int, [C.c_void_p, C.c_int, C.c_int, C.c_float, C.c_float, C.c_void_p, C.c_int, C.c_int, C.c_float,
                                 C.c_float] + [C.c_void_p] * 3 + [C.c_int] + [C.c_void_p] * 2 + [C.c_int] * 4 +
                       [C.c_float, C.c_void_p]),
    "kd_wf_ab_scale": (C.c_float, []),
    "kd_gn_conv3x3_winograd4_nhwc": (C.c_int, [C.c_void_p, C.c_int] + [C.c_void_p] * 4 + [C.c_int, C.c_int, C.c_float] +
                                     [C.c_void_p] * 3 + [C.c_int] + [C.c_void_p] * 2 + [C.c_int] * 8 + [C.c_void_p]),
    "kd_init_conv_nchw": (C.c_int, [C.c_void_p] * 6 + [C.c_int] * 5 + [C.c_void_p]),
    "kd_init_conv_planes_nchw": (C.c_int, [C.c_void_p] * 5 + [C.c_int] * 2 + [C.c_void_p] * 3 + [C.c_int] * 6 +
                                 [C.POINTER(C.c_float), C.c_void_p]),
    "kd_init_conv_planes_c_nchw": (C.c_int, [C.c_void_p] * 5 + [C.c_int] * 2 + [C.c_void_p] * 3 + [C.c_int] * 6 +
                                   [C.POINTER(C.c_float), C.c_int, C.c_void_p]),
    "kd_final_conv_nchw": (C.c_int, [C.c_void_p] * 5 + [C.c_int] * 5 + [C.c_void_p]),
    "kd_groupnorm_silu_nhwc": (C.c_int, [C.c_void_p] * 5 + [C.c_int] * 4 + [C.c_float, C.c_void_p]),
    "kd_layernorm": (C.c_int, [C.c_void_p] * 4 + [C.c_int, C.c_int, C.c_float, C.c_void_p]),
    "kd_layernorm_ex": (C.c_int, [C.c_void_p] * 5 + [C.c_int, C.c_int, C.c_float, C.c_int, C.c_void_p, C.c_void_p, C.c_void_p]),
    "kd_layernorm_linear_bf16x3": (C.c_int, [C.c_void_p] * 3 + [C.c_int, C.c_int, C.c_float, C.c_int] + [C.c_void_p] * 3 +
                                   [C.c_int, C.c_void_p, C.c_int, C.c_int, C.c_void_p, C.c_void_p]),
    "kd_attention_ex_d": (C.c_int, [C.c_void_p, C.c_int, C.c_void_p, C.c_void_p, C.c_void_p, C.c_int, C.c_int, C.c_void_p,
                                   C.c_void_p, C.c_int, C.c_int, C.c_void_p, C.c_int, C.c_int, C.c_int, C.c_int, C.c_int,
                                   C.c_int, C.c_float, C.c_void_p]),
    "kd_attention_key_tile": (C.c_int, [C.c_int]),
    "kd_l2norm_heads_d": (C.c_int, [C.c_void_p, C.c_int, C.c_int64, C.c_int, C.c_int, C.c_void_p, C.c_void_p]),
    "kd_attention": (C.c_int, [C.c_void_p] * 4 + [C.c_int] * 6 + [C.c_void_p]),
    "kd_attention_ex": (C.c_int, [C.c_void_p, C.c_int, C.c_void_p, C.c_void_p, C.c_void_p, C.c_int, C.c_int, C.c_void_p,
                                  C.c_void_p, C.c_int, C.c_int, C.c_void_p, C.c_int, C.c_int, C.c_int, C.c_int, C.c_int,
                                  C.c_float, C.c_void_p]),
    "kd_l2norm_heads": (C.c_int, [C.c_void_p, C.c_int, C.c_int64, C.c_int, C.c_void_p, C.c_void_p]),
    "kd_text_select": (C.c_int, [C.c_void_p] * 4 + [C.c_int] * 5 + [C.c_void_p]),
    "kd_add_rows_bcast": (C.c_int, [C.c_void_p] * 3 + [C.c_int] * 3 + [C.c_void_p]),
    "kd_mean_rows": (C.c_int, [C.c_void_p] * 2 + [C.c_int] * 3 + [C.c_void_p]),
    "kd_copy_rows": (C.c_int, [C.c_void_p, C.c_int64, C.c_int, C.c_void_p, C.c_int64, C.c_int, C.c_int, C.c_int, C.c_int,
                               C.c_void_p]),
    "kd_quantile_abs": (C.c_int, [C.c_void_p, C.c_void_p, C.c_int, C.c_int64, C.c_float, C.c_void_p, C.c_size_t,
                                  C.c_void_p]),
    "kd_quantile_workspace_bytes": (C.c_size_t, [C.c_int]),
    "kd_cfg_combine": (C.c_int, [C.c_void_p, C.c_void_p, C.c_void_p, C.c_float, C.c_int64, C.c_void_p]),
    "kd_philox_normal": (C.c_int, [C.c_void_p, C.c_int64, C.c_uint64, C.c_uint64, C.c_void_p]),
}

_lib = None
ABI_VERSION = 2


def lib_path() -> Path:
    return Path(os.environ.get("KD_ENGINE_LIB", _LIB_PATH))


def load() -> C.CDLL:
    global _lib
    if _lib is not None:
        return _lib
    path = lib_path()
    if not path.exists():
        raise EngineUnavailable(
            f"{path} not found — build it with `make -C kidney-diffusion_amd/csrc` "
            "(or `python -c 'import __graft_entry__ as g; g.build()'`). There is no CPU fallback.")
    lib = C.CDLL(str(path))
    for name, (restype, argtypes) in SIGNATURES.items():
        fn = getattr(lib, name)
        fn.restype = restype
        fn.argtypes = argtypes
    if lib.kd_version() != ABI_VERSION:
        raise EngineUnavailable(f"{path} speaks ABI version {lib.kd_version()}, this binding {ABI_VERSION} "
                                "(KD_ENGINE_ABI_VERSION of include/kd_engine.h)")
    _check_build_id(lib, path)
    _lib = lib
    return lib


def source_build_id():
    script = Path(__file__).resolve().parent.parent / "csrc" / "build_id.py"
    if not script.exists():
        return None
    import importlib.util

    spec = importlib.util.spec_from_file_location("_kd_build_id", script)
    mod = importlib.util.module_from_spec(spec)
    spec.loader.exec_module(mod)
    return mod.build_id()


def _check_build_id(lib, path):
    if "KD_ENGINE_LIB" in os.environ:
        return
    want = source_build_id()
    if want is None:
        return
    have = lib.kd_build_id().decode()
    if "+" in have:
        raise EngineUnavailable(
            f"{path} is an experiment build ({have}: its kernels and plans follow KD_* environment variables); the product "
            "path loads it only when KD_ENGINE_LIB names it explicitly. Rebuild with `make -C kidney-diffusion_amd/csrc`.")
    if have != want:
        raise EngineUnavailable(
            f"{path} was built from other sources (library build id {have}, sources {want}): "
            "rebuild with `make -C kidney-diffusion_amd/csrc`.")


def check(rc: int):
    if rc != 0:
        raise EngineError(load().kd_last_error().decode("utf-8", "replace"))


def require_gpu():
    import torch

    if not torch.cuda.is_available():
        raise EngineUnavailable("no HIP device visible: the MI355X engine has no CPU fallback")


def ptr(t):
    if t is None:
        return None
    import torch

    assert t.is_cuda and t.dtype == torch.float32 and t.is_contiguous(), "engine tensors: contiguous fp32 on device"
    return C.c_void_p(t.data_ptr())


def current_stream():
    import torch

    return C.c_void_p(torch.cuda.current_stream().cuda_stream)
```

Before: 40.69.

## Fuse GlobalContext attention pooling into Winograd F(4x4) output transform

Adds a Winograd output-transform kernel for Cout==128 that, while writing the conv output, also computes the GlobalContext to_k logits and an online-softmax weighted pooling, producing per-chunk partial records. The resnet block's GCA then merges these partials (fused gate or pool+MLP) and skips a separate full read of the block2 activation. This removes one pass over a large NHWC feature map per GCA block. In exchange the output kernel uses more registers and cross-lane shuffles, and it applies only when no residual is fused and Cout is 128.

Result: no change. 41.04 (median of 6 runs) (+0.9%).

```diff
diff --git a/include/kd_engine.h b/include/kd_engine.h
--- a/include/kd_engine.h
+++ b/include/kd_engine.h
@@ -239,6 +239,12 @@
                                  const float* d_scale_shift, int ld_ss, int skip_c0, float skip_scale, const float* d_w_oihw,
                                  const float* d_bias, const float* d_res, int ldres, float* d_y, double* d_out_seg, int B,
                                  int H, int W, int Cin, int Cout, int G, int gemm_mode, int images_per_set, void* stream);
+int kd_gn_conv3x3_winograd4_gca_nhwc(const float* d_x, int ldx, const float* d_stats, const float* d_gamma, const float* d_beta,
+                                     const float* d_scale_shift, int ld_ss, int skip_c0, float skip_scale,
+                                     const float* d_w_oihw, const float* d_bias, float* d_y, double* d_out_seg, int B, int H,
+                                     int W, int Cin, int Cout, int G, int gemm_mode, int images_per_set, const float* d_wk,
+                                     const float* d_bk, const float* d_w0, const float* d_b0, int hid, const float* d_w2,
+                                     const float* d_b2, float* d_gate, float* d_pooled, void* stream);
 
 int kd_init_conv_nchw(const float* d_x, const float* d_w3, const float* d_w7, const float* d_w15,
                       const float* d_bias, float* d_y, int B, int S, int n3, int n7, int n15, void* stream);
diff --git a/kidney-diffusion_amd/csrc/api.inc b/kidney-diffusion_amd/csrc/api.inc
--- a/kidney-diffusion_amd/csrc/api.inc
+++ b/kidney-diffusion_amd/csrc/api.inc
@@ -689,10 +689,45 @@
                       s);
 }
 
+namespace {
+struct W4GcaArgs {
+  const float *wk, *bk, *w0, *b0, *w2, *b2;
+  int hid;
+  float *gate, *pooled;
+};
+int gn_conv3x3_winograd4(const float* d_x, int ldx, const float* d_stats, const float* d_gamma, const float* d_beta,
+                         const float* d_scale_shift, int ld_ss, int skip_c0, float skip_scale, const float* d_w_oihw,
+                         const float* d_bias, const float* d_res, int ldres, float* d_y, double* d_out_seg, int B, int H, int W,
+                         int Cin, int Cout, int G, int gemm_mode, int images_per_set, const W4GcaArgs* gca, void* stream);
+}
+
 int kd_gn_conv3x3_winograd4_nhwc(const float* d_x, int ldx, const float* d_stats, const float* d_gamma, const float* d_beta,
                                  const float* d_scale_shift, int ld_ss, int skip_c0, float skip_scale, const float* d_w_oihw,
                                  const float* d_bias, const float* d_res, int ldres, float* d_y, double* d_out_seg, int B,
                                  int H, int W, int Cin, int Cout, int G, int gemm_mode, int images_per_set, void* stream) {
+  return gn_conv3x3_winograd4(d_x, ldx, d_stats, d_gamma, d_beta, d_scale_shift, ld_ss, skip_c0, skip_scale, d_w_oihw, d_bias,
+                              d_res, ldres, d_y, d_out_seg, B, H, W, Cin, Cout, G, gemm_mode, images_per_set, nullptr, stream);
+}
+
+int kd_gn_conv3x3_winograd4_gca_nhwc(const float* d_x, int ldx, const float* d_stats, const float* d_gamma, const float* d_beta,
+                                     const float* d_scale_shift, int ld_ss, int skip_c0, float skip_scale,
+                                     const float* d_w_oihw, const float* d_bias, float* d_y, double* d_out_seg, int B, int H,
+                                     int W, int Cin, int Cout, int G, int gemm_mode, int images_per_set, const float* d_wk,
+                                     const float* d_bk, const float* d_w0, const float* d_b0, int hid, const float* d_w2,
+                                     const float* d_b2, float* d_gate, float* d_pooled, void* stream) {
+  KD_REQUIRE(d_wk && d_bk && d_w0 && d_b0 && d_w2 && d_b2 && d_gate, "kd_gn_conv3x3_winograd4_gca_nhwc: null argument");
+  KD_REQUIRE(wino4_out_gca_ok(Cout), "kd_gn_conv3x3_winograd4_gca_nhwc: the pooling output transform needs Cout == 128");
+  KD_REQUIRE(hid > 0 && ((uintptr_t)d_wk & 7) == 0, "kd_gn_conv3x3_winograd4_gca_nhwc: hid > 0 and an 8-byte aligned to_k weight");
+  const W4GcaArgs gca{d_wk, d_bk, d_w0, d_b0, d_w2, d_b2, hid, d_gate, d_pooled};
+  return gn_conv3x3_winograd4(d_x, ldx, d_stats, d_gamma, d_beta, d_scale_shift, ld_ss, skip_c0, skip_scale, d_w_oihw, d_bias,
+                              nullptr, 0, d_y, d_out_seg, B, H, W, Cin, Cout, G, gemm_mode, images_per_set, &gca, stream);
+}
+
+namespace {
+int gn_conv3x3_winograd4(const float* d_x, int ldx, const float* d_stats, const float* d_gamma, const float* d_beta,
+                         const float* d_scale_shift, int ld_ss, int skip_c0, float skip_scale, const float* d_w_oihw,
+                         const float* d_bias, const float* d_res, int ldres, float* d_y, double* d_out_seg, int B, int H, int W,
+                         int Cin, int Cout, int G, int gemm_mode, int images_per_set, const W4GcaArgs* gca, void* stream) {
   hipStream_t s = (hipStream_t)stream;
   if (ldx <= 0) ldx = Cin;
   if (ldres <= 0) ldres = Cout;
@@ -725,6 +760,15 @@
   if (bufs.get((void**)&D, (size_t)36 * Mt * Cout * sizeof(float))) return 1;
   if (x3 && bufs.get(&U3, ((size_t)36 * Cout * Cin * 3 + 1) / 2 * sizeof(float))) return 1;
   if (x3 && bufs.get(&ws, gemm_bf16x3_workspace_bytes())) return 1;
+  const int gchunks = gca ? wino4_out_gca_chunks(Bx, H, W) : 0;
+  float* rec = nullptr;
+  if (gca && bufs.get((void**)&rec, (size_t)B * gchunks * (Cout + 2) * sizeof(float))) return 1;
+  const bool gate_fused = gca && gca_gate_fused_ok(Cout, gca->hid) && B > 1 && (((uintptr_t)gca->w0 | (uintptr_t)gca->w2) & 15) == 0;
+  float *pooled = gca ? gca->pooled : nullptr, *hidden = nullptr;
+  if (gca && !gate_fused) {
+    if (!pooled && bufs.get((void**)&pooled, (size_t)B * Cout * sizeof(float))) return 1;
+    if (bufs.get((void**)&hidden, (size_t)B * gca->hid * sizeof(float))) return 1;
+  }
   int rc = launch_wino4_pack(d_w_oihw, U, Cout, Cin, s);
   if (!rc && x3) rc = launch_split3(U, U3, 36, Cout, Cin, s);
   const int64_t HW = (int64_t)H * W, nchunk = (H / 4) * (W / 4);
@@ -749,11 +793,23 @@
       p.wz_rows = (int)Mt; p.wz_count = 36;
       rc = launch_conv_igemm(p, s);
     }
-    if (!rc)
+    double* segp = d_out_seg ? d_out_seg + (size_t)b0 * (Cout / 16) * nchunk * 2 : nullptr;
+    if (!rc && gca)
+      rc = launch_wino4_out_gca(D, d_bias, d_y + (size_t)b0 * HW * Cout, Cout, segp, gca->wk, gca->bk,
+                                rec + (size_t)b0 * gchunks * (Cout + 2), Bx, H, W, Cout, s);
+    else if (!rc)
       rc = launch_wino4_out(D, d_bias, d_res ? d_res + (size_t)b0 * HW * ldres : nullptr, ldres, d_y + (size_t)b0 * HW * Cout,
-                            Cout, d_out_seg ? d_out_seg + (size_t)b0 * (Cout / 16) * nchunk * 2 : nullptr, Bx, H, W, Cout, s);
-  }
-  return entry_finish(rc, s);
+                            Cout, segp, Bx, H, W, Cout, s);
+  }
+  if (!rc && gca) {
+    const bool fused = gate_fused;
+    if (fused) rc = launch_gca_gate_from_partials(rec, gchunks, gca->w0, gca->b0, gca->hid, gca->w2, gca->b2, gca->gate, B, Cout, s);
+    if (!rc && pooled) rc = launch_gca_pool_from_partials(rec, gchunks, pooled, B, Cout, s);
+    if (!rc && !fused) rc = launch_linear_skinny(pooled, Cout, gca->w0, gca->b0, hidden, gca->hid, B, Cout, gca->hid, ACT_NONE, ACT_SILU, s);
+    if (!rc && !fused) rc = launch_linear_skinny(hidden, gca->hid, gca->w2, gca->b2, gca->gate, Cout, B, gca->hid, Cout, ACT_NONE, ACT_SIGMOID, s);
+  }
+  return entry_finish(rc, s);
+}
 }
 
 int kd_init_conv_nchw(const float* d_x, const float* d_w3, const float* d_w7, const float* d_w15, const float* d_bias,
diff --git a/kidney-diffusion_amd/csrc/common.h b/kidney-diffusion_amd/csrc/common.h
--- a/kidney-diffusion_amd/csrc/common.h
+++ b/kidney-diffusion_amd/csrc/common.h
@@ -89,6 +89,10 @@
                     int mul_c0 = -1, float mul = 1.0f);
 int launch_wino4_out(const float* D, const float* bias, const float* res, int ldres, float* y, int ldy, double* seg_partial,
                      int B, int H, int W, int C, hipStream_t s);
+bool wino4_out_gca_ok(int C);
+int wino4_out_gca_chunks(int B, int H, int W);
+int launch_wino4_out_gca(const float* D, const float* bias, float* y, int ldy, double* seg_partial, const float* wk,
+                         const float* bk, float* part, int B, int H, int W, int C, hipStream_t s);
 
 constexpr int X3_BK = 16;
 __device__ __forceinline__ void x3_split(const float __attribute__((ext_vector_type(2))) a, uint32_t& h, uint32_t& m,
@@ -205,9 +209,13 @@
 int launch_gca_pool(const float* x, const float* wk, const float* bk, float* logits, float* pooled,
                     float* scratch, int B, int HW, int C, hipStream_t s);
 size_t gca_scratch_floats(int B, int HW, int C);
+int gca_chunk_rows(int HW, int B);
+int launch_gca_pool_from_partials(const float* part, int chunks, float* pooled, int B, int C, hipStream_t s);
 bool gca_gate_fused_ok(int C, int hid);
 int launch_gca_gate(const float* x, const float* wk, const float* bk, float* scratch, const float* w0, const float* b0, int hid,
                     const float* w2, const float* b2, float* gate, int B, int HW, int C, hipStream_t s);
+int launch_gca_gate_from_partials(const float* part, int chunks, const float* w0, const float* b0, int hid, const float* w2,
+                                  const float* b2, float* gate, int B, int C, hipStream_t s);
 int launch_sinu_emb(const float* t, const float* w, float* out, int B, int half, hipStream_t s);
 
 bool init_conv_fused_ok(int S, int n3, int n7, int n15, int np);
diff --git a/kidney-diffusion_amd/csrc/engine.hip b/kidney-diffusion_amd/csrc/engine.hip
--- a/kidney-diffusion_amd/csrc/engine.hip
+++ b/kidney-diffusion_amd/csrc/engine.hip
@@ -1013,8 +1013,17 @@
     return y;
   }
 
-  T gca(const T& h, const std::string& pre) {
+  struct GcaTap {
+    const float* wk = nullptr;
+    const float* bk = nullptr;
+    T rec;
+    int chunks = 0;
+  };
+
+  T gca(const T& h, const std::string& pre, const GcaTap* tap = nullptr) {
     int C = h.C, hid = std::max(3, C / 2);
+    const bool tapped = tap && tap->chunks > 0;
+    const int chunks = tapped ? tap->chunks : 0;
     const float* wk = P(pre + ".to_k.weight", C);
     const float* bk = P(pre + ".to_k.bias", 1);
     const float* w0 = P(pre + ".net.0.weight", (int64_t)hid * C);
@@ -1024,10 +1033,11 @@
     int Bx = h.B, HW = h.HW();
     const Ref hr = at(h);
     if (gca_gate_fused_ok(C, hid) && h.B > 1 && kd_switch("KD_GCA_FUSED", 1)) {
-      T scratch = alloc_bytes(gca_scratch_floats(h.B, h.HW(), C) * sizeof(float));
+      T scratch = tapped ? tap->rec : alloc_bytes(gca_scratch_floats(h.B, h.HW(), C) * sizeof(float));
       T gate = alloc(h.B, 1, 1, C);
       const Ref sr = at(scratch), gr = at(gate);
       emit([=](hipStream_t s) {
+        if (tapped) return launch_gca_gate_from_partials(sr.f(), chunks, w0, b0, hid, w2, b2, gr.f(), Bx, C, s);
         return launch_gca_gate(hr.f(), wk, bk, sr.f(), w0, b0, hid, w2, b2, gr.f(), Bx, HW, C, s);
       }, "gca_gate HW" + std::to_string(HW) + " C" + std::to_string(C));
       u->macs += (int64_t)Bx * HW * C * 2 + (int64_t)Bx * C * hid * 2;
@@ -1036,9 +1046,10 @@
     }
     T logits = alloc(h.B, h.H, h.W, 1);
     T pooled = alloc(h.B, 1, 1, C);
-    T scratch = alloc_bytes(gca_scratch_floats(h.B, h.HW(), C) * sizeof(float));
+    T scratch = tapped ? tap->rec : alloc_bytes(gca_scratch_floats(h.B, h.HW(), C) * sizeof(float));
     const Ref lr = at(logits), pr = at(pooled), sr = at(scratch);
     emit([=](hipStream_t s) {
+      if (tapped) return launch_gca_pool_from_partials(sr.f(), chunks, pr.f(), Bx, C, s);
       return launch_gca_pool(hr.f(), wk, bk, lr.f(), pr.f(), sr.f(), Bx, HW, C, s);
     }, "gca_pool HW" + std::to_string(HW) + " C" + std::to_string(C));
     u->macs += (int64_t)Bx * HW * C * 2;
@@ -1060,7 +1071,7 @@
     if (images > 0) return {Conv3x3::Wino4, images};
     const bool fused = fwino_ok(x, cout);
     auto gemm_ok = [&] {
-      if (cfg.conv_algo == 1 || cfg.conv_algo == 4) return false;
+      if (cfg.conv_algo == 1 || cfg.conv_algo == 4 || cfg.conv_algo == 5) return false;
       const int min_cin = cfg.conv_algo >= 32 ? cfg.conv_algo : 256;
       if (cfg.conv_algo < 32 && fused) return false;
       if ((x.H & 1) || (x.W & 1) || x.C < min_cin || x.C % 32 || cout <= 32 || cout % 4) return false;
@@ -1095,19 +1106,19 @@
     return 0;
   }
   bool wino4_whole_ok(const T& x, int cout) const {
-    if (cfg.conv_algo != 0 && cfg.conv_algo != 4) return false;
+    if (cfg.conv_algo != 0 && cfg.conv_algo != 4 && cfg.conv_algo != 5) return false;
     if (cfg.wino43_min_cin < 0 && cfg.conv_algo == 0) return false;
     if ((x.H & 3) || (x.W & 3) || x.C % 32 || cout % 64 || cout < 64) return false;
     const int64_t Mt = (int64_t)x.B * (x.H / 4) * (x.W / 4);
     if (Mt % 128 || 36 * Mt >= 0x7fffffff || (int64_t)36 * cout * x.C * 4 >= 0x7fffffff) return false;
-    if (cfg.conv_algo == 4) return true;
+    if (cfg.conv_algo == 4 || cfg.conv_algo == 5) return true;
     if ((36 * Mt / 128) * (cout / 64) < 512) return false;
     int thr = cfg.wino43_min_cin > 0 ? cfg.wino43_min_cin : 512;
     if (cfg.wino43_min_cin == 0 && cfg.gemm_bf16x3 >= 0 && gemm_bf16x3_ok(36, Mt, cout, x.C)) thr = 128;
     return x.C >= thr;
   }
   T wino4_block(const T& x, int Bx, const std::string& gn_prefix, int ss_col, const std::string& conv_prefix, int Cout,
-                const T* res, int skip_c0, float skip_scale) {
+                const T* res, int skip_c0, float skip_scale, GcaTap* tap = nullptr) {
     const int Cin = x.C, G = cfg.resnet_groups, H = x.H, W = x.W, HW = x.HW(), nset = x.B / Bx;
     const int64_t Mt = (int64_t)Bx * (H / 4) * (W / 4);
     const float* gamma = P(gn_prefix + ".weight", Cin);
@@ -1129,6 +1140,14 @@
     const int seg_nchunk = (H / 4) * (W / 4);
     const size_t sgo_all = sg ? add_seg(y, 0, Cout / 16, seg_nchunk) : 0;
     const Ref vr = at(V), dr = at(D);
+    const bool pool = tap && !res && wino4_out_gca_ok(Cout) && ((uintptr_t)tap->wk & 7) == 0;
+    const int gchunks = pool ? wino4_out_gca_chunks(Bx, H, W) : 0;
+    if (pool) {
+      tap->rec = alloc_bytes((size_t)x.B * gchunks * (Cout + 2) * sizeof(float));
+      tap->chunks = gchunks;
+    }
+    const Ref recr = pool ? at(tap->rec) : Ref();
+    const float *gwk = pool ? tap->wk : nullptr, *gbk = pool ? tap->bk : nullptr;
     for (int st = 0; st < nset; ++st) {
       const int b0 = st * Bx;
       {
@@ -1157,9 +1176,11 @@
       {
         const Ref seg = sg ? seg_at(sgo_all, Cout / 16, seg_nchunk, b0) : Ref(), yr = image(y, b0), rr = image(res, b0);
         const int ldres = res ? res->LD() : 0;
+        const Ref pr = recr.floats((int64_t)b0 * gchunks * (Cout + 2));
         emit([=](hipStream_t s) {
+          if (pool) return launch_wino4_out_gca(dr.f(), bias, yr.f(), Cout, seg.d(), gwk, gbk, pr.f(), Bx, H, W, Cout, s);
           return launch_wino4_out(dr.f(), bias, rr.f(), ldres, yr.f(), Cout, seg.d(), Bx, H, W, Cout, s);
-        }, "wino4_out" + shape);
+        }, "wino4_out" + shape + (pool ? " gca" : ""));
       }
     }
     free(V);
@@ -1254,14 +1275,14 @@
   }
 
   T gn_conv3x3(const T& x, bool free_x, const std::string& pre, int ss_col, int Cout, const T* res, int skip_c0 = -1,
-               float skip_scale = 1.0f) {
+               float skip_scale = 1.0f, GcaTap* tap = nullptr) {
     const Conv3x3Choice c = conv3x3_choice(x, Cout);
     if (skip_c0 >= 0 && c.algo != Conv3x3::Wino4 && c.algo != Conv3x3::WinoFused)
       throw std::runtime_error("plan: folded skip scale on a conv path that cannot apply it: " + pre);
     const std::string gn = pre + ".groupnorm", cv = pre + ".project";
     T y;
     switch (c.algo) {
-      case Conv3x3::Wino4: y = wino4_block(x, c.images, gn, ss_col, cv, Cout, res, skip_c0, skip_scale); break;
+      case Conv3x3::Wino4: y = wino4_block(x, c.images, gn, ss_col, cv, Cout, res, skip_c0, skip_scale, tap); break;
       case Conv3x3::WinoGemm: y = wino_block(x, gn, ss_col, cv, Cout, res); break;
       case Conv3x3::WinoFused: y = fwino_gn_conv(x, gn, ss_col, cv, Cout, res); break;
       case Conv3x3::Direct: {
@@ -1293,7 +1314,14 @@
     auto it = tmlp_off.find(pre);
     int ss_col = it != tmlp_off.end() ? it->second : -1;
     bool has_res_conv = has(pre + ".res_conv.weight");
-    T h2 = gn_conv3x3(h, true, pre + ".block2", ss_col, dim_out, (!use_gca && !has_res_conv) ? &x : nullptr);
+    GcaTap tap;
+    const bool offer = use_gca && !has_cross && kd_switch("KD_WINO4_GCA", 1) != 0 && cfg.conv_algo != 5;
+    if (offer) {
+      tap.wk = P(pre + ".gca.to_k.weight", dim_out);
+      tap.bk = P(pre + ".gca.to_k.bias", 1);
+    }
+    T h2 = gn_conv3x3(h, true, pre + ".block2", ss_col, dim_out, (!use_gca && !has_res_conv) ? &x : nullptr, -1, 1.0f,
+                      offer ? &tap : nullptr);
     if (!use_gca && !has_res_conv) return h2;
     if (skip_c0 >= 0 && !has_res_conv) throw std::runtime_error("plan: folded skip scale without a skip conv: " + pre);
     const float* w_res = nullptr;
@@ -1310,7 +1338,7 @@
     }
     T out;
     if (use_gca) {
-      T gate = gca(h2, pre + ".gca");
+      T gate = gca(h2, pre + ".gca", &tap);
       if (has_res_conv) {
         ConvOpt o;
         o.gate_src = &h2;
diff --git a/kidney-diffusion_amd/csrc/kernels_small.hip b/kidney-diffusion_amd/csrc/kernels_small.hip
--- a/kidney-diffusion_amd/csrc/kernels_small.hip
+++ b/kidney-diffusion_amd/csrc/kernels_small.hip
@@ -116,6 +116,7 @@
   while (r > 32 && (int64_t)((HW + r - 1) / r) * B < 1024 && (HW + r / 2 - 1) / (r / 2) <= 1024) r /= 2;
   return r;
 }
+int gca_chunk_rows(int HW, int B) { return gca_rows(HW, B); }
 constexpr int GCA_MAXT = 8;
 constexpr int GCA_U = 4;
 
@@ -359,7 +360,15 @@
   KD_REQUIRE((((uintptr_t)w0 | (uintptr_t)w2) & 15) == 0, "fused GlobalContext gate: 16-byte aligned weights");
   const int rows = gca_rows(HW, B), chunks = (HW + rows - 1) / rows;
   if (launch_gca_partial(x, wk, bk, scratch, B, HW, C, rows, chunks, s)) return 1;
-  hipLaunchKernelGGL(gca_gate_kernel, dim3(B), dim3(256), 0, s, scratch, chunks, C, w0, b0, hid, w2, b2, gate);
+  return launch_gca_gate_from_partials(scratch, chunks, w0, b0, hid, w2, b2, gate, B, C, s);
+}
+
+int launch_gca_gate_from_partials(const float* part, int chunks, const float* w0, const float* b0, int hid, const float* w2,
+                                  const float* b2, float* gate, int B, int C, hipStream_t s) {
+  KD_REQUIRE(gca_gate_fused_ok(C, hid), "fused GlobalContext gate needs C % 4 == 0, C <= 512, hidden <= 256");
+  KD_REQUIRE((((uintptr_t)w0 | (uintptr_t)w2) & 15) == 0, "fused GlobalContext gate: 16-byte aligned weights");
+  KD_REQUIRE(part && B > 0 && chunks > 0 && chunks <= 1024, "GlobalContext merge: 1 .. 1024 records per image");
+  hipLaunchKernelGGL(gca_gate_kernel, dim3(B), dim3(256), 0, s, part, chunks, C, w0, b0, hid, w2, b2, gate);
   KD_HIP_CHECK(hipGetLastError());
   return 0;
 }
@@ -374,7 +383,12 @@
   KD_REQUIRE(C % 4 == 0 && C <= 64 * 4 * GCA_MAXT, "gca needs C % 4 == 0 and C <= 2048");
   const int rows = gca_rows(HW, B), chunks = (HW + rows - 1) / rows;
   if (launch_gca_partial(x, wk, bk, scratch, B, HW, C, rows, chunks, s)) return 1;
-  hipLaunchKernelGGL(gca_combine_kernel, dim3(B, (C + 15) / 16), dim3(256), 0, s, scratch, pooled, chunks, C);
+  return launch_gca_pool_from_partials(scratch, chunks, pooled, B, C, s);
+}
+
+int launch_gca_pool_from_partials(const float* part, int chunks, float* pooled, int B, int C, hipStream_t s) {
+  KD_REQUIRE(part && pooled && B > 0 && C > 0 && chunks > 0 && chunks <= 1024, "GlobalContext merge: 1 .. 1024 records per image");
+  hipLaunchKernelGGL(gca_combine_kernel, dim3(B, (C + 15) / 16), dim3(256), 0, s, part, pooled, chunks, C);
   KD_HIP_CHECK(hipGetLastError());
   return 0;
 }
diff --git a/kidney-diffusion_amd/csrc/kernels_wino4.hip b/kidney-diffusion_amd/csrc/kernels_wino4.hip
--- a/kidney-diffusion_amd/csrc/kernels_wino4.hip
+++ b/kidney-diffusion_amd/csrc/kernels_wino4.hip
@@ -304,4 +304,155 @@
   return 0;
 }
 
-}
+constexpr int W4G_C = 128;
+__global__ __launch_bounds__(256) __attribute__((amdgpu_waves_per_eu(4, 4))) void wino4_out_gca_kernel(const float* __restrict__ D, const float* __restrict__ bias,
+                                                            float* __restrict__ y, int ldy, double* __restrict__ seg,
+                                                            const float* __restrict__ wk, const float* __restrict__ bk,
+                                                            float* __restrict__ part, int H, int W, int64_t nt, int tpc) {
+  constexpr int C = W4G_C;
+  __shared__ __attribute__((aligned(8))) float sacc[4 * C];
+  __shared__ float sml[8];
+  const int Ht = H >> 2, Wt = W >> 2, nimg = Ht * Wt;
+  const int b = blockIdx.y, chunk = blockIdx.x, nchunks = gridDim.x;
+  const int lane = threadIdx.x & 63, wave = __builtin_amdgcn_readfirstlane(threadIdx.x >> 6);
+  const int c = lane * 2;
+  const int t0 = chunk * tpc, t1 = min(nimg, t0 + tpc);
+  const int64_t pstride = nt * C;
+  f32x2 bv = {0.0f, 0.0f};
+  if (bias) bv = *(const f32x2*)(bias + c);
+  const f32x2 wv = *(const f32x2*)(wk + c);
+  const float kb = bk[0];
+  const bool b5 = (lane & 32) != 0, b4 = (lane & 16) != 0, b3 = (lane & 8) != 0, b2 = (lane & 4) != 0;
+  float mrun = -INFINITY, lrun = 0.0f;
+  f32x2 acc = {0.0f, 0.0f};
+  const int nit = (tpc + 3) >> 2;
+  for (int ti = t0 + wave * nit, te = min(t1, ti + nit); ti < te; ++ti) {
+    const int tx = ti % Wt, ty = ti / Wt;
+    const float* in = D + ((int64_t)b * nimg + ti) * C + c;
+    f32x2 u[4][6];
+#pragma unroll
+    for (int s = 0; s < 6; ++s) {
+      f32x2 m[6];
+#pragma unroll
+      for (int r = 0; r < 6; ++r) m[r] = *(const f32x2*)(in + (int64_t)(r * 6 + s) * pstride);
+      f32x2 ycol[4];
+      w4_at(m, ycol);
+#pragma unroll
+      for (int i = 0; i < 4; ++i) u[i][s] = ycol[i];
+    }
+    const int64_t pix0 = ((int64_t)b * H + 4 * ty) * W + 4 * tx;
+    float s1 = 0.0f, s2 = 0.0f;
+    f32x2 v[16];
+    float d[16];
+#pragma unroll
+    for (int i = 0; i < 4; ++i) {
+      f32x2 o[4];
+      w4_at(u[i], o);
+#pragma unroll
+      for (int j = 0; j < 4; ++j) {
+        const int64_t pix = pix0 + (int64_t)i * W + j;
+        f32x2 vv = o[j] + bv;
+        vv += f32x2{0.0f, 0.0f};
+        *(f32x2*)(y + pix * ldy + c) = vv;
+        s1 += vv[0] + vv[1];
+        s2 = fmaf(vv[0], vv[0], fmaf(vv[1], vv[1], s2));
+        v[i * 4 + j] = vv;
+        d[i * 4 + j] = vv[0] * wv[0] + vv[1] * wv[1];
+      }
+    }
+    float e8[8], e4[4], e2[2];
+#pragma unroll
+    for (int q = 0; q < 8; ++q) e8[q] = (b5 ? d[q + 8] : d[q]) + __shfl_xor(b5 ? d[q] : d[q + 8], 32, 64);
+#pragma unroll
+    for (int q = 0; q < 4; ++q) e4[q] = (b4 ? e8[q + 4] : e8[q]) + __shfl_xor(b4 ? e8[q] : e8[q + 4], 16, 64);
+#pragma unroll
+    for (int q = 0; q < 2; ++q) e2[q] = (b3 ? e4[q + 2] : e4[q]) + __shfl_xor(b3 ? e4[q] : e4[q + 2], 8, 64);
+    float k = (b2 ? e2[1] : e2[0]) + __shfl_xor(b2 ? e2[0] : e2[1], 4, 64);
+    k += __shfl_xor(k, 2, 64);
+    k += __shfl_xor(k, 1, 64);
+    const float lgl = k + kb;
+    float mnew = mrun;
+#pragma unroll
+    for (int q = 0; q < 16; ++q)
+      mnew = fmaxf(mnew, __builtin_bit_cast(float, __builtin_amdgcn_readlane(__builtin_bit_cast(int, lgl), 4 * q)));
+    const float corr = expf(mrun - mnew);
+    const float pl = expf(lgl - mnew);
+    float p[16];
+#pragma unroll
+    for (int q = 0; q < 16; ++q) p[q] = __builtin_bit_cast(float, __builtin_amdgcn_readlane(__builtin_bit_cast(int, pl), 4 * q));
+    float ps[4];
+    f32x2 as[4];
+#pragma unroll
+    for (int i = 0; i < 4; ++i) {
+      ps[i] = (p[4 * i] + p[4 * i + 1]) + (p[4 * i + 2] + p[4 * i + 3]);
+      as[i] = (v[4 * i] * p[4 * i] + v[4 * i + 1] * p[4 * i + 1]) + (v[4 * i + 2] * p[4 * i + 2] + v[4 * i + 3] * p[4 * i + 3]);
+    }
+    lrun = lrun * corr + ((ps[0] + ps[1]) + (ps[2] + ps[3]));
+    acc = acc * corr + ((as[0] + as[1]) + (as[2] + as[3]));
+    mrun = mnew;
+    if (seg) {
+      double d1 = (double)s1, d2 = (double)s2;
+#pragma unroll
+      for (int off = 1; off <= 4; off <<= 1) {
+        d1 += __shfl_xor(d1, off, 64);
+        d2 += __shfl_xor(d2, off, 64);
+      }
+      if ((c & 15) == 0) {
+        double* op = seg + (((int64_t)b * (C >> 4) + (c >> 4)) * nimg + ti) * 2;
+        op[0] = d1;
+        op[1] = d2;
+      }
+    }
+  }
+  if (lane == 0) {
+    sml[wave * 2] = mrun;
+    sml[wave * 2 + 1] = lrun;
+  }
+  *(f32x2*)(sacc + wave * C + c) = acc;
+  __syncthreads();
+  const float mb = fmaxf(fmaxf(sml[0], sml[2]), fmaxf(sml[4], sml[6]));
+  float sc[4], lb = 0.f;
+#pragma unroll
+  for (int w = 0; w < 4; ++w) {
+    sc[w] = sml[w * 2] == -INFINITY ? 0.f : expf(sml[w * 2] - mb);
+    lb += sml[w * 2 + 1] * sc[w];
+  }
+  float* out = part + ((int64_t)b * nchunks + chunk) * (C + 2);
+  for (int cc = threadIdx.x; cc < C; cc += 256)
+    out[2 + cc] = (sacc[cc] * sc[0] + sacc[C + cc] * sc[1]) + (sacc[2 * C + cc] * sc[2] + sacc[3 * C + cc] * sc[3]);
+  if (threadIdx.x == 0) {
+    out[0] = mb;
+    out[1] = lb;
+  }
+}
+
+bool wino4_out_gca_ok(int C) { return C == W4G_C; }
+
+static int w4g_rows(int B, int H, int W) {
+  if (kd_switch("KD_W4G_ROWS", 0) > 0) return kd_switch("KD_W4G_ROWS", 0);
+  const int HW = H * W;
+  int rows = gca_chunk_rows(HW, B);
+  while (rows < 1024 && (int64_t)B * ((HW + 2 * rows - 1) / (2 * rows)) >= 2048) rows *= 2;
+  return rows;
+}
+int wino4_out_gca_chunks(int B, int H, int W) {
+  const int rows = w4g_rows(B, H, W);
+  return (H * W + rows - 1) / rows;
+}
+
+int launch_wino4_out_gca(const float* D, const float* bias, float* y, int ldy, double* seg_partial, const float* wk,
+                         const float* bk, float* part, int B, int H, int W, int C, hipStream_t s) {
+  KD_REQUIRE(wino4_out_gca_ok(C), "Winograd F(4x4,3x3) output transform with GlobalContext pooling: Cout == 128 only");
+  KD_REQUIRE(wk && bk && part, "Winograd F(4x4,3x3) output transform with GlobalContext pooling: null to_k weight, bias or records");
+  KD_REQUIRE(B > 0 && B <= 65535 && H > 0 && W > 0 && H % 4 == 0 && W % 4 == 0 && ldy >= C && ldy % 2 == 0 &&
+                 (((uintptr_t)y | (uintptr_t)bias | (uintptr_t)wk) & 7) == 0,
+             "Winograd F(4x4,3x3) output transform needs H % 4 == 0, W % 4 == 0, even C / row strides, 8-byte aligned maps");
+  const int rows = w4g_rows(B, H, W);
+  const int nimg = (H / 4) * (W / 4), tpc = rows / 16, chunks = (nimg + tpc - 1) / tpc;
+  hipLaunchKernelGGL(wino4_out_gca_kernel, dim3((unsigned)chunks, (unsigned)B), dim3(256), 0, s, D, bias, y, ldy, seg_partial, wk,
+                     bk, part, H, W, (int64_t)B * nimg, tpc);
+  KD_HIP_CHECK(hipGetLastError());
+  return 0;
+}
+
+}
diff --git a/kidney-diffusion_amd/imagen_pytorch/_engine.py b/kidney-diffusion_amd/imagen_pytorch/_engine.py
--- a/kidney-diffusion_amd/imagen_pytorch/_engine.py
+++ b/kidney-diffusion_amd/imagen_pytorch/_engine.py
@@ -190,6 +190,8 @@
     "kd_wf_ab_scale": (C.c_float, []),
     "kd_gn_conv3x3_winograd4_nhwc": (C.c_int, [C.c_void_p, C.c_int] + [C.c_void_p] * 4 + [C.c_int, C.c_int, C.c_float] +
                                      [C.c_void_p] * 3 + [C.c_int] + [C.c_void_p] * 2 + [C.c_int] * 8 + [C.c_void_p]),
+    "kd_gn_conv3x3_winograd4_gca_nhwc": (C.c_int, [C.c_void_p, C.c_int] + [C.c_void_p] * 4 + [C.c_int, C.c_int, C.c_float] +
+                                         [C.c_void_p] * 4 + [C.c_int] * 8 + [C.c_void_p] * 4 + [C.c_int] + [C.c_void_p] * 5),
     "kd_init_conv_nchw": (C.c_int, [C.c_void_p] * 6 + [C.c_int] * 5 + [C.c_void_p]),
     "kd_init_conv_planes_nchw": (C.c_int, [C.c_void_p] * 5 + [C.c_int] * 2 + [C.c_void_p] * 3 + [C.c_int] * 6 +
                                  [C.POINTER(C.c_float), C.c_void_p]),
```
